# skywoodsz/qm_control

Measured on NVIDIA H100. Metric: mpc_wbc_iters_per_s, higher is better.
Workload: dtype f64

## Files before the change

include/qmb200.h:

```cpp
#ifndef QMB200_H
#define QMB200_H
#include <stdint.h>

#ifdef __cplusplus
extern "C" {
#endif

#define QMB200_NX 30
#define QMB200_NU 30
#define QMB200_RBD 55
#define QMB200_CMD 54
#define QMB200_TARGET 37
#define QMB200_EMAX 32
#define QMB200_KMAX 4

#define QMB200_WBC_HIERARCHICAL 0
#define QMB200_WBC_HIERARCHICAL_MPC 1

#define QMB200_ST_ITER_CAP 1
#define QMB200_ST_OVERFLOW 2
#define QMB200_ST_NAN 4
#define QMB200_ST_NOT_PD 8
#define QMB200_ST_NO_STEP 16
#define QMB200_ST_CONVERGED 32
// ... 15 lines not shown
  int32_t wbc_variant;
} qmb200_config;

int qmb200_create(const qmb200_config* cfg, qmb200_handle** out);
void qmb200_destroy(qmb200_handle* h);
const char* qmb200_last_error(const qmb200_handle* h);

int qmb200_get_dims(const qmb200_handle* h, int32_t* batch, int32_t* nmax, int32_t* emax, int32_t* kmax);
int qmb200_get_model_info(const qmb200_handle* h, double* robot_mass, double* initial_state30, double* default_joint_state18, double* time_horizon, double* dt);
int qmb200_get_joint_name(const qmb200_handle* h, int32_t joint, char* out, int32_t capacity);

int qmb200_wbc_update(qmb200_handle* h, const double* x_des , const double* u_des , const double* rbd ,
                      const int32_t* mode , const double* period , const double* time , double* cmd , int32_t* status );
int qmb200_wbc_update_dev(qmb200_handle* h, const double* x_des, const double* u_des, const double* rbd, const int32_t* mode, const double* period,
                          const double* time, double* cmd, int32_t* status, void* cuda_stream);
int qmb200_wbc_set_input_last(qmb200_handle* h, const double* input_last );
int qmb200_wbc_get_input_last(qmb200_handle* h, double* input_last );

typedef struct {
  double kp_swing, kd_swing, base_height_kp, base_height_kd, kp_base_linear, kd_base_linear, kp_base_angular, kd_base_angular;
  double kp_arm_joint[6], kd_arm_joint[6], kp_ee_linear[3], kd_ee_linear[3], kp_ee_angular[3], kd_ee_angular[3];
} qmb200_wbc_gains;
int qmb200_wbc_get_gains(const qmb200_handle* h, qmb200_wbc_gains* out);
int qmb200_wbc_set_gains(qmb200_handle* h, const qmb200_wbc_gains* gains);
int qmb200_wbc_get_diagnostics(qmb200_handle* h, int32_t* diag );
int qmb200_wbc_set_iteration_caps(qmb200_handle* h, int32_t level0_passes, int32_t active_set_iterations);

int qmb200_mpc_solve(qmb200_handle* h, const double* t0 , const double* x0 ,
                     const int32_t* n_events , const double* event_times , const int32_t* mode_sequence ,
                     const int32_t* n_target , const double* target_times , const double* target_states ,
                     int32_t* n_nodes , double* node_times , int32_t* node_events ,
                     double* x_traj , double* u_traj , int32_t* status , double* step_info );
int qmb200_mpc_solve_dev(qmb200_handle* h, const double* t0, const double* x0, const int32_t* n_events, const double* event_times, const int32_t* mode_sequence,
                         const int32_t* n_target, const double* target_times, const double* target_states, void* cuda_stream);
int qmb200_mpc_set_iterations(qmb200_handle* h, int32_t sqp_iterations, double cost_tol);
int qmb200_mpc_reset(qmb200_handle* h);
int qmb200_mpc_set_solution(qmb200_handle* h, const int32_t* n_nodes, const double* node_times, const int32_t* node_events, const double* x_traj, const double* u_traj);
int qmb200_mpc_get_solution(qmb200_handle* h, int32_t* n_nodes, double* node_times, int32_t* node_events, double* x_traj, double* u_traj, int32_t* status, double* step_info);

int qmb200_policy_eval(qmb200_handle* h, const double* t , double* x_des , double* u_des , int32_t* mode );
int qmb200_policy_eval_dev(qmb200_handle* h, const double* t, double* x_des, double* u_des, int32_t* mode, void* cuda_stream);

int qmb200_tick(qmb200_handle* h, const double* t0, const double* x0, const int32_t* n_events, const double* event_times, const int32_t* mode_sequence,
                const int32_t* n_target, const double* target_times, const double* target_states, const double* t_eval, const double* rbd,
                const double* period, double* cmd , int32_t* status );
int qmb200_tick_dev(qmb200_handle* h, const double* t0, const double* x0, const int32_t* n_events, const double* event_times, const int32_t* mode_sequence,
                    const int32_t* n_target, const double* target_times, const double* target_states, const double* t_eval, const double* rbd,
                    const double* period, double* cmd, int32_t* status, void* cuda_stream);

int qmb200_centroidal_state_from_rbd(const qmb200_handle* h, int32_t n, const double* rbd , double* x );

#define QMB200_SRBD 24
int qmb200_set_model_payload(qmb200_handle* h, const double* payload );
int qmb200_get_model_payload(const qmb200_handle* h, double* payload , int32_t* is_set);

#define QMB200_TUNING 40
int qmb200_set_robot_tuning(qmb200_handle* h, const double* rows );
int qmb200_get_robot_tuning(const qmb200_handle* h, double* rows , int32_t* is_set);
int qmb200_get_handle_tuning(const qmb200_handle* h, double* row );

typedef struct qmb200_payload_est_params {
  double forgetting, p0_mass, p0_first_moment, p0_inertia, trace_max, mass_min, mass_max, offset_max;
} qmb200_payload_est_params;
int qmb200_payload_est_get_params(const qmb200_handle* h, qmb200_payload_est_params* out);
int qmb200_payload_est_set_params(qmb200_handle* h, const qmb200_payload_est_params* p);
int qmb200_payload_est_reset(qmb200_handle* h, const double* prior );
int qmb200_payload_est_step(qmb200_handle* h, double dt, const double* effort , const double* rbd , int32_t* status );
int qmb200_payload_est_step_dev(qmb200_handle* h, double dt, const double* effort, const double* rbd, int32_t* status, void* cuda_stream);
int qmb200_payload_est_commit_dev(qmb200_handle* h, void* cuda_stream);
int qmb200_payload_est_get(qmb200_handle* h, double* theta , double* p_diag , int32_t* samples );
int qmb200_payload_est_stop(qmb200_handle* h);
int qmb200_get_model_payload_dev(const qmb200_handle* h, double* payload , void* cuda_stream);

int qmb200_gait_schedule(const char* gait_file, const char* gait_name, double t_start, double lo, double hi,
                         double* event_times , int32_t* mode_sequence );

typedef struct qmb200_gait qmb200_gait;
int qmb200_gait_create(const char* task_file, const char* reference_file, qmb200_gait** out);
void qmb200_gait_destroy(qmb200_gait* g);
int qmb200_gait_insert_template(qmb200_gait* g, const char* gait_file, const char* gait_name, double start_time, double final_time);
int qmb200_gait_get_mode_schedule(qmb200_gait* g, double lower_bound_time, double upper_bound_time, double* event_times , int32_t* mode_sequence );

#define QMB200_GAIT_CAP 64
#define QMB200_GAIT_MAXM 16
int qmb200_gait_dev_set_templates(qmb200_handle* h, const char* gait_file, const char* const* names, int32_t n);
int qmb200_gait_dev_reset(qmb200_handle* h, const int32_t* tmpl , const double* t_start );
int qmb200_gait_dev_set_commands(qmb200_handle* h, int32_t n_cmd, const double* t , const int32_t* tmpl , const double* cmd_vel );
int qmb200_gait_dev_set_commands_ee(qmb200_handle* h, int32_t n_cmd, const double* t , const int32_t* tmpl , const double* cmd_vel ,
                                    const int32_t* ee_kind , const double* ee_cmd );
int qmb200_gait_dev_step(qmb200_handle* h, const double* t_obs , int32_t* n_events , double* event_times ,
                         int32_t* mode_sequence , double* cmd , int32_t* tmpl , int32_t* mode ,
                         int32_t* status );
int qmb200_gait_dev_step_dev(qmb200_handle* h, const double* t_obs, int32_t* n_events, double* event_times, int32_t* mode_sequence, double* cmd, int32_t* tmpl,
                             int32_t* mode, int32_t* status, void* cuda_stream);
int qmb200_gait_dev_step_ee(qmb200_handle* h, const double* t_obs , int32_t* n_events , double* event_times ,
                            int32_t* mode_sequence , double* cmd , int32_t* tmpl , int32_t* mode ,
                            int32_t* status , int32_t* target_kind );
int qmb200_gait_dev_step_ee_dev(qmb200_handle* h, const double* t_obs, int32_t* n_events, double* event_times, int32_t* mode_sequence, double* cmd, int32_t* tmpl,
                                int32_t* mode, int32_t* status, int32_t* target_kind, void* cuda_stream);
int qmb200_gait_dev_get(qmb200_handle* h, int32_t* n_events , double* event_times , int32_t* mode_sequence ,
                        int32_t* tmpl , int32_t* cursor );
int qmb200_gait_dev_get_commands(qmb200_handle* h, int32_t* n_cmd, double* t , int32_t* tmpl , double* cmd_vel ,
                                 int32_t* ee_kind , double* ee_cmd );
int qmb200_gait_dev_stop(qmb200_handle* h);

#define QMB200_TARGET_CMD_VEL 0
#define QMB200_TARGET_EE_CMD_VEL 1
#define QMB200_TARGET_EE_GOAL 2
#define QMB200_JOINT_CMD 5
#define QMB200_ST_SAFETY 0x10000
#define QMB200_ST_HW_RING_FULL 2

int qmb200_observation_update(qmb200_handle* h, const double* rbd , const double* period , double* t_obs , double* x_obs );
int qmb200_observation_update_dev(qmb200_handle* h, const double* rbd, const double* period, double* t_obs, double* x_obs, void* cuda_stream);

int qmb200_target_trajectories(qmb200_handle* h, int32_t kind, const double* cmd , const double* t_obs , const double* x_obs , const double* ee_state ,
                               double* last_ee_target , int32_t* n_target , double* target_times , double* target_states );
int qmb200_target_trajectories_dev(qmb200_handle* h, int32_t kind, const double* cmd, const double* t_obs, const double* x_obs, const double* ee_state, double* last_ee_target,
                                   int32_t* n_target, double* target_times, double* target_states, void* cuda_stream);
int qmb200_target_trajectories_per_robot(qmb200_handle* h, const int32_t* kind , const double* cmd , const double* t_obs , const double* x_obs ,
                                         const double* ee_state , double* last_ee_target , int32_t* n_target ,
                                         double* target_times , double* target_states );
int qmb200_target_trajectories_per_robot_dev(qmb200_handle* h, const int32_t* kind, const double* cmd, const double* t_obs, const double* x_obs, const double* ee_state,
                                             double* last_ee_target, int32_t* n_target, double* target_times, double* target_states, void* cuda_stream);
void qmb200_initial_ee_target(double* last_ee_target7);

int qmb200_control_law(qmb200_handle* h, const double* x_des , const double* u_des , const double* wbc_cmd , const double* t_obs , const double* x_obs ,
                       double* joint_cmd , double* arm_pos_cmd , double* last_time , int32_t* status );
int qmb200_control_law_dev(qmb200_handle* h, const double* x_des, const double* u_des, const double* wbc_cmd, const double* t_obs, const double* x_obs, double* joint_cmd, double* arm_pos_cmd,
                           double* last_time, int32_t* status, void* cuda_stream);
int qmb200_set_arm_gains(qmb200_handle* h, double kp_arm_wbc, double kd_arm_wbc);

int qmb200_hw_write(qmb200_handle* h, const double* time , const double* period , const double* joint_cmd , const double* joint_pos , const double* joint_vel ,
                    double* effort , int32_t* status );
int qmb200_hw_write_dev(qmb200_handle* h, const double* time, const double* period, const double* joint_cmd, const double* joint_pos, const double* joint_vel, double* effort, int32_t* status, void* cuda_stream);
int qmb200_hw_set_delay(qmb200_handle* h, double delay);

typedef struct {
  double ground_height;
  double foot_radius;
  double stiffness;
  double damping;
  double tangential_damping;
  double friction_mu;
  double joint_damping[18];
  int32_t substeps_per_ms;
} qmb200_sim_params;
int qmb200_sim_get_params(const qmb200_handle* h, qmb200_sim_params* out);
int qmb200_sim_set_params(qmb200_handle* h, const qmb200_sim_params* p);
int qmb200_sim_step(qmb200_handle* h, double duration, const double* effort , double* q , double* v ,
                    double* rbd , int32_t* contact , int32_t* status );
int qmb200_sim_step_dev(qmb200_handle* h, double duration, const double* effort, double* q, double* v, double* rbd, int32_t* contact, int32_t* status, void* cuda_stream);
int qmb200_sim_set_robot_params(qmb200_handle* h, const double* friction_mu , const double* payload );
int qmb200_sim_get_robot_params(const qmb200_handle* h, double* friction_mu , double* payload , int32_t* set_mask);
int qmb200_sim_step_ext(qmb200_handle* h, double duration, const double* effort , const double* wrench , double* q ,
                        double* v , double* rbd , int32_t* contact , int32_t* status );
int qmb200_sim_step_ext_dev(qmb200_handle* h, double duration, const double* effort, const double* wrench, double* q, double* v, double* rbd, int32_t* contact,
                            int32_t* status, void* cuda_stream);
int qmb200_sim_set_terrain(qmb200_handle* h, int32_t n_tiles, int32_t nx, int32_t ny, double cell, const double* heights );
int qmb200_sim_get_terrain(const qmb200_handle* h, int32_t* n_tiles, int32_t* nx, int32_t* ny, double* cell, double* heights );
int qmb200_sim_set_robot_terrain(qmb200_handle* h, const int32_t* tile , const double* origin );
int qmb200_sim_get_robot_terrain(const qmb200_handle* h, int32_t* tile , double* origin , int32_t* is_set);
int qmb200_sim_standing_state(const qmb200_handle* h, int32_t n, const double* xy_yaw , double* q , double* v );

#define QMB200_SENSORS 46
typedef struct qmb200_sensor_params {
  uint64_t seed;
  double sigma_orientation, sigma_gyro, sigma_accel, sigma_joint_pos, sigma_joint_vel;
} qmb200_sensor_params;
int qmb200_sim_get_sensor_params(const qmb200_handle* h, qmb200_sensor_params* out);
int qmb200_sim_set_sensor_params(qmb200_handle* h, const qmb200_sensor_params* p);
int qmb200_sim_read_sensors(qmb200_handle* h, double dt, int64_t sample, const double* q , const double* v , const double* v_prev ,
                            double* sensors );
int qmb200_sim_read_sensors_dev(qmb200_handle* h, double dt, int64_t sample, const double* q, const double* v, const double* v_prev, double* sensors, void* cuda_stream);

typedef struct qmb200_state_est_params {
  double process_base_pos, process_base_vel, process_foot, meas_foot_pos, meas_foot_vel, meas_foot_height, swing_scale, foot_height, p0_base_pos, p0_base_vel, p0_foot;
} qmb200_state_est_params;
int qmb200_state_est_get_params(const qmb200_handle* h, qmb200_state_est_params* out);
int qmb200_state_est_set_params(qmb200_handle* h, const qmb200_state_est_params* p);
int qmb200_state_est_reset(qmb200_handle* h, const double* base_pos );
int qmb200_state_est_step(qmb200_handle* h, double dt, const double* sensors , const int32_t* contact , double* rbd_est , int32_t* status );
int qmb200_state_est_step_dev(qmb200_handle* h, double dt, const double* sensors, const int32_t* contact, double* rbd_est, int32_t* status, void* cuda_stream);
int qmb200_state_est_get(qmb200_handle* h, double* x , double* p_diag , int32_t* samples );
int qmb200_state_est_stop(qmb200_handle* h);
int qmb200_state_est_set_ground(qmb200_handle* h, const int32_t* tile , const double* origin );
int qmb200_state_est_get_ground(const qmb200_handle* h, int32_t* tile , double* origin , int32_t* is_set);

typedef struct qmb200_attitude_params {
  double process_attitude, process_gyro_bias, meas_orientation, p0_attitude, p0_gyro_bias;
} qmb200_attitude_params;
int qmb200_attitude_get_params(const qmb200_handle* h, qmb200_attitude_params* out);
int qmb200_attitude_set_params(qmb200_handle* h, const qmb200_attitude_params* p);
int qmb200_attitude_reset(qmb200_handle* h);
int qmb200_attitude_step(qmb200_handle* h, double dt, double* sensors , int32_t* status );
int qmb200_attitude_step_dev(qmb200_handle* h, double dt, double* sensors, int32_t* status, void* cuda_stream);
int qmb200_attitude_get(qmb200_handle* h, double* quat , double* gyro_bias , double* p_diag , int32_t* samples );
int qmb200_attitude_stop(qmb200_handle* h);

typedef struct qmb200_slip_params {
  double gate, release, meas_slip;
  int32_t hold;
} qmb200_slip_params;
int qmb200_slip_get_params(const qmb200_handle* h, qmb200_slip_params* out);
int qmb200_slip_set_params(qmb200_handle* h, const qmb200_slip_params* p);
int qmb200_slip_reset(qmb200_handle* h);
int qmb200_slip_step(qmb200_handle* h, double dt, const double* sensors , const int32_t* contact_in , int32_t* stance_out ,
                     int32_t* slip_out , int32_t* status );
int qmb200_slip_step_dev(qmb200_handle* h, double dt, const double* sensors, const int32_t* contact_in, int32_t* stance_out, int32_t* slip_out, int32_t* status,
                         void* cuda_stream);
int qmb200_slip_get(qmb200_handle* h, int32_t* mask , int32_t* hold , int32_t* onsets );
int qmb200_slip_stop(qmb200_handle* h);

int qmb200_robot_image_save(qmb200_handle* h);
int qmb200_robot_image_clear(qmb200_handle* h);
int qmb200_robot_image_restore(qmb200_handle* h, const int32_t* mask );
int qmb200_robot_image_restore_dev(qmb200_handle* h, const int32_t* mask , void* cuda_stream);
int qmb200_fall_detect(qmb200_handle* h, const double* rbd , double z_min, double tilt_max, int32_t* count , int32_t* fallen );
int qmb200_fall_detect_dev(qmb200_handle* h, const double* rbd, double z_min, double tilt_max, int32_t* count, int32_t* fallen, void* cuda_stream);

#define QMB200_EPISODE 27
#define QMB200_EPISODE_MODEL_PAYLOAD 1
#define QMB200_EPISODE_MPC_FRICTION 2
#define QMB200_EPISODE_WBC_FRICTION 4
int qmb200_episode_set_ranges(qmb200_handle* h, const double* lo , const double* hi , int64_t seed);
int qmb200_episode_get_ranges(const qmb200_handle* h, double* lo , double* hi , int64_t* seed, int32_t* is_set);
int qmb200_episode_sample(qmb200_handle* h, const int32_t* mask , const int32_t* episode , int32_t link, double* rows );
int qmb200_episode_sample_dev(qmb200_handle* h, const int32_t* mask, const int32_t* episode, int32_t link, double* rows, void* cuda_stream);
int qmb200_episode_draw(const qmb200_handle* h, int32_t n, const int32_t* robot , const int32_t* episode , double* rows );

#define QMB200_SPAWN 4
#define QMB200_SPAWN_GROUND_MAP 1
int qmb200_spawn_set_ranges(qmb200_handle* h, const double* lo , const double* hi , int64_t seed);
int qmb200_spawn_get_ranges(const qmb200_handle* h, double* lo , double* hi , int64_t* seed, int32_t* is_set);
int qmb200_spawn_sample(qmb200_handle* h, const int32_t* mask , const int32_t* episode , int32_t link, double* rows ,
                        double* q , double* v , double* rbd , int32_t* contact ,
                        double* x_obs , double* last_ee , double* rbd_est );
int qmb200_spawn_sample_dev(qmb200_handle* h, const int32_t* mask, const int32_t* episode, int32_t link, double* rows, double* q, double* v, double* rbd, int32_t* contact,
                            double* x_obs, double* last_ee, double* rbd_est, void* cuda_stream);
int qmb200_spawn_draw(const qmb200_handle* h, int32_t n, const int32_t* robot , const int32_t* episode , double* rows );

#define QMB200_METRICS 18
#define QMB200_METRICS_ACC 32
int qmb200_metrics_step(qmb200_handle* h, double dt, const double* rbd , const int32_t* contact , const double* effort ,
                        const double* cmd , const int32_t* kind , const int32_t* n_target , const double* target_times,
                        const double* target_states, const double* time , const int32_t* status , const double* rbd_est ,
                        double* acc );
int qmb200_metrics_step_dev(qmb200_handle* h, double dt, const double* rbd, const int32_t* contact, const double* effort, const double* cmd, const int32_t* kind,
                            const int32_t* n_target, const double* target_times, const double* target_states, const double* time, const int32_t* status,
                            const double* rbd_est, double* acc, void* cuda_stream);
int qmb200_metrics_close(qmb200_handle* h, const int32_t* mask , const int32_t* end , const int32_t* episode , int32_t n_episodes,
                         double* acc , double* out , int32_t* status );
int qmb200_metrics_close_dev(qmb200_handle* h, const int32_t* mask, const int32_t* end, const int32_t* episode, int32_t n_episodes, double* acc, double* out,
                             int32_t* status, void* cuda_stream);

#define QMB200_TIMELINE 22
#define QMB200_TIMELINE_CMD 14
int qmb200_timeline_set_ranges(qmb200_handle* h, int32_t n_cmd, const double* lo , const double* hi ,
                               int64_t seed);
int qmb200_timeline_get_ranges(const qmb200_handle* h, int32_t* n_cmd, double* lo , double* hi , int64_t* seed,
                               int32_t* is_set);
int qmb200_timeline_sample(qmb200_handle* h, const int32_t* mask , const int32_t* episode , double* rows );
int qmb200_timeline_sample_dev(qmb200_handle* h, const int32_t* mask, const int32_t* episode, double* rows, void* cuda_stream);
int qmb200_timeline_draw(const qmb200_handle* h, int32_t n, const int32_t* robot , const int32_t* episode , double* rows );

#define QMB200_CURRICULUM 7
#define QMB200_CURRICULUM_STATE 4
#define QMB200_CURRICULUM_MAX_COND 4
#define QMB200_CURRICULUM_EPISODE 0
#define QMB200_CURRICULUM_SPAWN 1
#define QMB200_CURRICULUM_TIMELINE 2
#define QMB200_CURRICULUM_GE 0
#define QMB200_CURRICULUM_LE 1
#define QMB200_CURRICULUM_PASS 0
#define QMB200_CURRICULUM_FAIL 1
typedef struct qmb200_curriculum_rule {
  int32_t n_levels, n_cond;
  int32_t column[QMB200_CURRICULUM_MAX_COND], op[QMB200_CURRICULUM_MAX_COND], role[QMB200_CURRICULUM_MAX_COND];
} qmb200_curriculum_rule;
int qmb200_curriculum_set(qmb200_handle* h, const qmb200_curriculum_rule* rule, const double* rows );
int qmb200_curriculum_attach(qmb200_handle* h, int32_t kind, const double* lo_top , const double* hi_top );
int qmb200_curriculum_update(qmb200_handle* h, const int32_t* mask , const int32_t* end , const int32_t* episode ,
                             const double* rows , int32_t n_episodes, int32_t* level ,
                             int32_t* status );
int qmb200_curriculum_update_dev(qmb200_handle* h, const int32_t* mask, const int32_t* end, const int32_t* episode, const double* rows, int32_t n_episodes,
                                 int32_t* level, int32_t* status, void* cuda_stream);
int qmb200_curriculum_get(const qmb200_handle* h, int32_t* state , int32_t* is_set);
int qmb200_curriculum_draw(const qmb200_handle* h, int32_t kind, int32_t n, const int32_t* robot , const int32_t* episode ,
                           const int32_t* level , double* rows);

int qmb200_update(qmb200_handle* h, const double* rbd , const double* period , double* t_obs , double* x_obs , double* joint_cmd ,
                  double* arm_pos_cmd , double* last_time , double* cmd , int32_t* status );
int qmb200_update_dev(qmb200_handle* h, const double* rbd, const double* period, double* t_obs, double* x_obs, double* joint_cmd, double* arm_pos_cmd, double* last_time, double* cmd, int32_t* status, void* cuda_stream);

int qmb200_set_pipeline(qmb200_handle* h, int chunks);

int qmb200_set_profiling(qmb200_handle* h, int on);
int qmb200_collect_kernel_times(qmb200_handle* h);
int qmb200_get_kernel_times(qmb200_handle* h, double* ms6);
int qmb200_get_flow_kernel_time(qmb200_handle* h, double* ms);
int qmb200_measure_fp64_peak(qmb200_handle* h, double* tflops);

int qmb200_debug_get_step(qmb200_handle* h, double* dx , double* du , double* robot );
#define QMB200_SOLVER_SQP 0
#define QMB200_SOLVER_IPM 1
#define QMB200_SOLVER_DDP 2
int qmb200_mpc_set_solver(qmb200_handle* h, int32_t solver);
int qmb200_mpc_get_solver(const qmb200_handle* h, int32_t* solver, int32_t* iterations, double* delta_tol, double* g_max, double* g_min);

#define QMB200_COMM_ID_BYTES 128
int qmb200_comm_get_unique_id(void* id128);
int qmb200_comm_init(qmb200_handle* h, int32_t nranks, int32_t rank, const void* id128);
int qmb200_comm_destroy(qmb200_handle* h);
int qmb200_comm_info(const qmb200_handle* h, int32_t* nranks, int32_t* rank, int32_t* nccl_version);
int qmb200_allgather_torque(qmb200_handle* h, void* nccl_comm, const double* cmd_local , const int32_t* perm ,
                            double* torque_all , void* cuda_stream);
int qmb200_gait_bin_permutation(int32_t n, const double* t0, const int32_t* n_events, const double* event_times , const int32_t* modes , int32_t* perm );

int64_t qmb200_debug_model_blob(const qmb200_config* cfg, void* out, int64_t capacity);
int qmb200_debug_srbd_constants(const qmb200_config* cfg, int32_t n, const double* payload , double* out );

int64_t qmb200_launch_count(const qmb200_handle* h);
void* qmb200_stream(const qmb200_handle* h);

#ifdef __cplusplus
}
#endif
#endif
```

qm_control_b200/_lib.py:

```python
import ctypes as C
import os

HERE = os.path.dirname(os.path.abspath(__file__))
ROOT = os.path.dirname(HERE)
LIB_PATH = os.environ.get("QMB200_LIB", os.path.join(HERE, "libqmb200.so"))
ASSETS = os.path.join(ROOT, "assets")

NX, NU, RBD, CMD, TARGET, EMAX, KMAX = 30, 30, 55, 54, 37, 32, 4
GAIT_CAP, GAIT_MAXM = 64, 16
TARGET_CMD_VEL, TARGET_EE_CMD_VEL, TARGET_EE_GOAL = 0, 1, 2

dp = C.POINTER(C.c_double)
ip = C.POINTER(C.c_int32)


class QmbError(RuntimeError):
    pass


class Config(C.Structure):
    _fields_ = [("task_file", C.c_char_p), ("urdf_file", C.c_char_p), ("reference_file", C.c_char_p), ("wbc_gains_file", C.c_char_p),
                ("batch", C.c_int32), ("device", C.c_int32), ("time_horizon", C.c_double), ("dt", C.c_double), ("max_nodes", C.c_int32), ("wbc_variant", C.c_int32)]


class WbcGains(C.Structure):
    _fields_ = [(n, C.c_double) for n in ("kp_swing", "kd_swing", "base_height_kp", "base_height_kd", "kp_base_linear", "kd_base_linear", "kp_base_angular", "kd_base_angular")] + \
               [("kp_arm_joint", C.c_double * 6), ("kd_arm_joint", C.c_double * 6), ("kp_ee_linear", C.c_double * 3), ("kd_ee_linear", C.c_double * 3), ("kp_ee_angular", C.c_double * 3), ("kd_ee_angular", C.c_double * 3)]


class SimParams(C.Structure):
    _fields_ = [(n, C.c_double) for n in ("ground_height", "foot_radius", "stiffness", "damping", "tangential_damping", "friction_mu")] + \
               [("joint_damping", C.c_double * 18), ("substeps_per_ms", C.c_int32)]


class PayloadEstParams(C.Structure):
    _fields_ = [(n, C.c_double) for n in ("forgetting", "p0_mass", "p0_first_moment", "p0_inertia", "trace_max", "mass_min", "mass_max", "offset_max")]


SENSORS = 46


class SensorParams(C.Structure):
    _fields_ = [("seed", C.c_uint64)] + [(n, C.c_double) for n in ("sigma_orientation", "sigma_gyro", "sigma_accel", "sigma_joint_pos", "sigma_joint_vel")]


class StateEstParams(C.Structure):
    _fields_ = [(n, C.c_double) for n in ("process_base_pos", "process_base_vel", "process_foot", "meas_foot_pos", "meas_foot_vel", "meas_foot_height", "swing_scale",
                                          "foot_height", "p0_base_pos", "p0_base_vel", "p0_foot")]


class AttitudeParams(C.Structure):
    _fields_ = [(n, C.c_double) for n in ("process_attitude", "process_gyro_bias", "meas_orientation", "p0_attitude", "p0_gyro_bias")]


class SlipParams(C.Structure):
    _fields_ = [("gate", C.c_double), ("release", C.c_double), ("meas_slip", C.c_double), ("hold", C.c_int32)]


SENSOR_LAYOUT = ("quat_x", "quat_y", "quat_z", "quat_w", "gyro_x", "gyro_y", "gyro_z", "accel_x", "accel_y", "accel_z") + \
                tuple("joint_pos_%d" % j for j in range(18)) + tuple("joint_vel_%d" % j for j in range(18))
STATE_EST_LAYOUT = ("p_x", "p_y", "p_z", "v_x", "v_y", "v_z") + tuple("foot_%s_%s" % (f, a) for f in ("LF", "RF", "LH", "RH") for a in "xyz")
SENSOR_NOISE_REFERENCE = dict(sigma_orientation=0.0012 ** 0.5, sigma_gyro=0.0004 ** 0.5, sigma_accel=0.01 ** 0.5)

THETA_LAYOUT = ("m", "mc_x", "mc_y", "mc_z", "I_xx", "I_xy", "I_xz", "I_yy", "I_yz", "I_zz")

PAYLOAD_LAYOUT = ("m_ee", "o_ee_x", "o_ee_y", "o_ee_z", "m_base", "o_base_x", "o_base_y", "o_base_z")
SRBD_LAYOUT = ("m",) + tuple("I_nom_%d%d" % (i, j) for i in range(3) for j in range(3)) + tuple("I_nom_inv_%d%d" % (i, j) for i in range(3) for j in range(3)) + \
              ("c_nom_x", "c_nom_y", "c_nom_z", "pad0", "pad1")
TUNING_LAYOUT = {}
for _n, _w in [("friction_mu", 1), ("wbc_friction", 1), ("mu_ee_pos", 1), ("mu_ee_ori", 1), ("mu_final_ee_pos", 1), ("mu_final_ee_ori", 1)] + \
              [(_f, getattr(_t, "_length_", 1)) for _f, _t in WbcGains._fields_] + [("kp_arm_wbc", 1), ("kd_arm_wbc", 1)]:
    TUNING_LAYOUT[_n] = (sum(w for _, w in TUNING_LAYOUT.values()), _w)
TUNING = sum(w for _, w in TUNING_LAYOUT.values())
del _n, _w
WRENCH_LAYOUT = ("f_base_x", "f_base_y", "f_base_z", "n_base_x", "n_base_y", "n_base_z", "f_ee_x", "f_ee_y", "f_ee_z", "n_ee_x", "n_ee_y", "n_ee_z")
EPISODE_LAYOUT = ("friction_mu",) + PAYLOAD_LAYOUT + ("push_t_on", "push_duration") + WRENCH_LAYOUT + ("cmd_vel_x", "cmd_vel_y", "cmd_vel_z", "cmd_yaw_rate")
EPISODE = len(EPISODE_LAYOUT)
EPISODE_MODEL_PAYLOAD, EPISODE_MPC_FRICTION, EPISODE_WBC_FRICTION = 1, 2, 4
SPAWN_LAYOUT = ("tile", "dx", "dy", "yaw")
SPAWN = len(SPAWN_LAYOUT)
SPAWN_GROUND_MAP = 1
METRICS_LAYOUT = ("duration", "end", "status", "distance", "path_length", "min_height", "max_tilt", "vel_err_rms", "yaw_rate_err_rms", "ee_pos_err_rms",
                  "ee_pos_err_max", "ee_ori_err_rms", "energy", "torque_rms", "slip", "touchdowns", "est_pos_err_rms", "est_vel_err_rms")
METRICS = len(METRICS_LAYOUT)
METRICS_ACC = 32
TIMELINE_LAYOUT = ("t_first", "gap", "p_gait", "gait_set", "w_none", "w_cmd_vel", "w_ee_cmd_vel", "w_ee_goal", "cmd_vel_x", "cmd_vel_y", "cmd_vel_z", "cmd_yaw_rate",
                   "ee_vx", "ee_vy", "ee_vz", "ee_x", "ee_y", "ee_z", "ee_qx", "ee_qy", "ee_qz", "ee_qw")
TIMELINE = len(TIMELINE_LAYOUT)
TIMELINE_CMD_LAYOUT = ("t", "tmpl", "cmd_vel_x", "cmd_vel_y", "cmd_vel_z", "cmd_yaw_rate", "ee_kind") + tuple("ee_%d" % i for i in range(7))
TIMELINE_CMD = len(TIMELINE_CMD_LAYOUT)
CURRICULUM_LAYOUT = ("start_level", "up_after", "down_after", "threshold_0", "threshold_1", "threshold_2", "threshold_3")
CURRICULUM = len(CURRICULUM_LAYOUT)
CURRICULUM_STATE_LAYOUT = ("level", "pass_run", "fail_run", "n_updates")
CURRICULUM_STATE = len(CURRICULUM_STATE_LAYOUT)
CURRICULUM_MAX_COND = 4
CURRICULUM_KINDS = ("episode", "spawn", "timeline")
CURRICULUM_OPS = (">=", "<=")
CURRICULUM_ROLES = ("pass", "fail")


class CurriculumRule(C.Structure):
    _fields_ = [("n_levels", C.c_int32), ("n_cond", C.c_int32), ("column", C.c_int32 * 4), ("op", C.c_int32 * 4), ("role", C.c_int32 * 4)]


P, I32, I64, D, S, CFG = C.c_void_p, C.c_int32, C.c_int64, C.c_double, C.c_char_p, C.POINTER(Config)
PROTOTYPES = {
    "qmb200_create": (I32, [CFG, P]),
    "qmb200_destroy": (None, [P]),
    "qmb200_last_error": (S, [P]),
    "qmb200_get_dims": (I32, [P] * 5),
    "qmb200_get_model_info": (I32, [P] * 6),
    "qmb200_get_joint_name": (I32, [P, I32, P, I32]),
    "qmb200_wbc_update": (I32, [P] * 9),
    "qmb200_wbc_update_dev": (I32, [P] * 10),
    "qmb200_wbc_set_input_last": (I32, [P] * 2),
    "qmb200_wbc_get_input_last": (I32, [P] * 2),
    "qmb200_wbc_get_gains": (I32, [P] * 2),
    "qmb200_wbc_set_gains": (I32, [P] * 2),
    "qmb200_wbc_get_diagnostics": (I32, [P] * 2),
    "qmb200_wbc_set_iteration_caps": (I32, [P, I32, I32]),
    "qmb200_mpc_solve": (I32, [P] * 16),
    "qmb200_mpc_solve_dev": (I32, [P] * 10),
    "qmb200_mpc_set_iterations": (I32, [P, I32, D]),
    "qmb200_mpc_reset": (I32, [P]),
    "qmb200_mpc_set_solution": (I32, [P] * 6),
    "qmb200_mpc_get_solution": (I32, [P] * 8),
    "qmb200_policy_eval": (I32, [P] * 5),
    "qmb200_policy_eval_dev": (I32, [P] * 6),
    "qmb200_tick": (I32, [P] * 14),
    "qmb200_tick_dev": (I32, [P] * 15),
    "qmb200_centroidal_state_from_rbd": (I32, [P, I32, P, P]),
    "qmb200_set_model_payload": (I32, [P] * 2),
    "qmb200_get_model_payload": (I32, [P] * 3),
    "qmb200_set_robot_tuning": (I32, [P] * 2),
    "qmb200_get_robot_tuning": (I32, [P] * 3),
    "qmb200_get_handle_tuning": (I32, [P] * 2),
    "qmb200_payload_est_get_params": (I32, [P] * 2),
    "qmb200_payload_est_set_params": (I32, [P] * 2),
    "qmb200_payload_est_reset": (I32, [P] * 2),
    "qmb200_payload_est_step": (I32, [P, D] + [P] * 3),
    "qmb200_payload_est_step_dev": (I32, [P, D] + [P] * 4),
    "qmb200_payload_est_commit_dev": (I32, [P] * 2),
    "qmb200_payload_est_get": (I32, [P] * 4),
    "qmb200_payload_est_stop": (I32, [P]),
    "qmb200_get_model_payload_dev": (I32, [P] * 3),
    "qmb200_gait_schedule": (I32, [S, S, D, D, D, P, P]),
    "qmb200_gait_create": (I32, [S, S, P]),
    "qmb200_gait_destroy": (None, [P]),
    "qmb200_gait_insert_template": (I32, [P, S, S, D, D]),
    "qmb200_gait_get_mode_schedule": (I32, [P, D, D, P, P]),
    "qmb200_gait_dev_set_templates": (I32, [P, S, P, I32]),
    "qmb200_gait_dev_reset": (I32, [P] * 3),
    "qmb200_gait_dev_set_commands": (I32, [P, I32] + [P] * 3),
    "qmb200_gait_dev_set_commands_ee": (I32, [P, I32] + [P] * 5),
    "qmb200_gait_dev_step": (I32, [P] * 9),
    "qmb200_gait_dev_step_dev": (I32, [P] * 10),
    "qmb200_gait_dev_step_ee": (I32, [P] * 10),
    "qmb200_gait_dev_step_ee_dev": (I32, [P] * 11),
    "qmb200_gait_dev_get": (I32, [P] * 6),
    "qmb200_gait_dev_get_commands": (I32, [P] * 7),
    "qmb200_gait_dev_stop": (I32, [P]),
    "qmb200_observation_update": (I32, [P] * 5),
    "qmb200_observation_update_dev": (I32, [P] * 6),
    "qmb200_target_trajectories": (I32, [P, I32] + [P] * 8),
    "qmb200_target_trajectories_dev": (I32, [P, I32] + [P] * 9),
    "qmb200_target_trajectories_per_robot": (I32, [P] * 10),
    "qmb200_target_trajectories_per_robot_dev": (I32, [P] * 11),
    "qmb200_initial_ee_target": (None, [P]),
    "qmb200_control_law": (I32, [P] * 10),
    "qmb200_control_law_dev": (I32, [P] * 11),
    "qmb200_set_arm_gains": (I32, [P, D, D]),
    "qmb200_hw_write": (I32, [P] * 8),
    "qmb200_hw_write_dev": (I32, [P] * 9),
    "qmb200_hw_set_delay": (I32, [P, D]),
    "qmb200_sim_get_params": (I32, [P] * 2),
    "qmb200_sim_set_params": (I32, [P] * 2),
    "qmb200_sim_step": (I32, [P, D] + [P] * 6),
    "qmb200_sim_step_dev": (I32, [P, D] + [P] * 7),
    "qmb200_sim_set_robot_params": (I32, [P] * 3),
    "qmb200_sim_get_robot_params": (I32, [P] * 4),
    "qmb200_sim_step_ext": (I32, [P, D] + [P] * 7),
    "qmb200_sim_step_ext_dev": (I32, [P, D] + [P] * 8),
    "qmb200_sim_set_terrain": (I32, [P, I32, I32, I32, D, P]),
    "qmb200_sim_get_terrain": (I32, [P] * 6),
    "qmb200_sim_set_robot_terrain": (I32, [P] * 3),
    "qmb200_sim_get_robot_terrain": (I32, [P] * 4),
    "qmb200_sim_standing_state": (I32, [P, I32, P, P, P]),
    "qmb200_sim_get_sensor_params": (I32, [P] * 2),
    "qmb200_sim_set_sensor_params": (I32, [P] * 2),
    "qmb200_sim_read_sensors": (I32, [P, D, I64] + [P] * 4),
    "qmb200_sim_read_sensors_dev": (I32, [P, D, I64] + [P] * 5),
    "qmb200_state_est_get_params": (I32, [P] * 2),
    "qmb200_state_est_set_params": (I32, [P] * 2),
    "qmb200_state_est_reset": (I32, [P] * 2),
    "qmb200_state_est_step": (I32, [P, D] + [P] * 4),
    "qmb200_state_est_step_dev": (I32, [P, D] + [P] * 5),
    "qmb200_state_est_get": (I32, [P] * 4),
    "qmb200_state_est_stop": (I32, [P]),
    "qmb200_state_est_set_ground": (I32, [P] * 3),
    "qmb200_state_est_get_ground": (I32, [P] * 4),
    "qmb200_attitude_get_params": (I32, [P] * 2),
    "qmb200_attitude_set_params": (I32, [P] * 2),
    "qmb200_attitude_reset": (I32, [P]),
    "qmb200_attitude_step": (I32, [P, D] + [P] * 2),
    "qmb200_attitude_step_dev": (I32, [P, D] + [P] * 3),
    "qmb200_attitude_get": (I32, [P] * 5),
    "qmb200_attitude_stop": (I32, [P]),
    "qmb200_slip_get_params": (I32, [P] * 2),
    "qmb200_slip_set_params": (I32, [P] * 2),
    "qmb200_slip_reset": (I32, [P]),
    "qmb200_slip_step": (I32, [P, D] + [P] * 5),
    "qmb200_slip_step_dev": (I32, [P, D] + [P] * 6),
    "qmb200_slip_get": (I32, [P] * 4),
    "qmb200_slip_stop": (I32, [P]),
    "qmb200_robot_image_save": (I32, [P]),
    "qmb200_robot_image_clear": (I32, [P]),
    "qmb200_robot_image_restore": (I32, [P] * 2),
    "qmb200_robot_image_restore_dev": (I32, [P] * 3),
    "qmb200_fall_detect": (I32, [P, P, D, D, P, P]),
    "qmb200_fall_detect_dev": (I32, [P, P, D, D, P, P, P]),
    "qmb200_episode_set_ranges": (I32, [P, P, P, I64]),
    "qmb200_episode_get_ranges": (I32, [P] * 5),
    "qmb200_episode_sample": (I32, [P, P, P, I32, P]),
    "qmb200_episode_sample_dev": (I32, [P, P, P, I32, P, P]),
    "qmb200_episode_draw": (I32, [P, I32, P, P, P]),
    "qmb200_spawn_set_ranges": (I32, [P, P, P, I64]),
    "qmb200_spawn_get_ranges": (I32, [P] * 5),
    "qmb200_spawn_sample": (I32, [P, P, P, I32] + [P] * 8),
    "qmb200_spawn_sample_dev": (I32, [P, P, P, I32] + [P] * 9),
    "qmb200_spawn_draw": (I32, [P, I32, P, P, P]),
    "qmb200_metrics_step": (I32, [P, D] + [P] * 12),
    "qmb200_metrics_step_dev": (I32, [P, D] + [P] * 13),
    "qmb200_metrics_close": (I32, [P] * 4 + [I32] + [P] * 3),
    "qmb200_metrics_close_dev": (I32, [P] * 4 + [I32] + [P] * 4),
    "qmb200_timeline_set_ranges": (I32, [P, I32, P, P, I64]),
    "qmb200_timeline_get_ranges": (I32, [P] * 6),
    "qmb200_timeline_sample": (I32, [P] * 4),
    "qmb200_timeline_sample_dev": (I32, [P] * 5),
    "qmb200_timeline_draw": (I32, [P, I32, P, P, P]),
    "qmb200_curriculum_set": (I32, [P] * 3),
    "qmb200_curriculum_attach": (I32, [P, I32, P, P]),
    "qmb200_curriculum_update": (I32, [P] * 5 + [I32] + [P] * 2),
    "qmb200_curriculum_update_dev": (I32, [P] * 5 + [I32] + [P] * 3),
    "qmb200_curriculum_get": (I32, [P] * 3),
    "qmb200_curriculum_draw": (I32, [P, I32, I32] + [P] * 4),
    "qmb200_update": (I32, [P] * 10),
    "qmb200_update_dev": (I32, [P] * 11),
    "qmb200_set_pipeline": (I32, [P, I32]),
    "qmb200_set_profiling": (I32, [P, I32]),
    "qmb200_collect_kernel_times": (I32, [P]),
    "qmb200_get_kernel_times": (I32, [P] * 2),
    "qmb200_get_flow_kernel_time": (I32, [P] * 2),
    "qmb200_measure_fp64_peak": (I32, [P] * 2),
    "qmb200_debug_get_step": (I32, [P] * 4),
    "qmb200_mpc_set_solver": (I32, [P, I32]),
    "qmb200_mpc_get_solver": (I32, [P] * 6),
    "qmb200_comm_get_unique_id": (I32, [P]),
    "qmb200_comm_init": (I32, [P, I32, I32, P]),
    "qmb200_comm_destroy": (I32, [P]),
    "qmb200_comm_info": (I32, [P] * 4),
    "qmb200_allgather_torque": (I32, [P] * 6),
    "qmb200_gait_bin_permutation": (I32, [I32] + [P] * 5),
    "qmb200_debug_model_blob": (I64, [CFG, P, I64]),
    "qmb200_debug_srbd_constants": (I32, [CFG, I32, P, P]),
    "qmb200_launch_count": (I64, [P]),
    "qmb200_stream": (P, [P]),
}
SYMBOLS = list(PROTOTYPES)

_lib = None


def load_library():
    global _lib
    if _lib is not None:
        return _lib
    if not os.path.exists(LIB_PATH):
        raise QmbError("libqmb200.so not built (%s): run `python -c 'import __graft_entry__ as g; g.build()'` — there is no CPU fallback" % LIB_PATH)
    lib = C.CDLL(LIB_PATH)
    for name, (restype, argtypes) in PROTOTYPES.items():
        fn = getattr(lib, name)
        fn.restype, fn.argtypes = restype, argtypes
    _lib = lib
    return lib


def asset(name):
    return os.path.join(ASSETS, name)
```

qm_control_b200/csrc/capi_mpc.inc:

```

extern "C" {

int qmb200_centroidal_state_from_rbd(const qmb200_handle* h, int32_t n, const double* rbd, double* x) {
  if (!h || !rbd || !x) return -1; const DevModel& d = h->hm.dev;
  if (int rc = model_rows_sync(h)) return rc;
  const double* srbd = h->srbd.host.empty() ? nullptr : h->srbd.host.data();
  if (srbd && n != h->B) return fail(const_cast<qmb200_handle*>(h), "qmb200_centroidal_state_from_rbd: with a model payload set, n must equal the batch size");
  for (int r = 0; r < n; ++r) centroidal_from_rbd(*srbd_of(&d, srbd, r), rbd + (size_t)r * QMB200_RBD, x + (size_t)r * NX);
  return 0;
}

int qmb200_gait_schedule(const char* gait_file, const char* gait_name, double t_start, double lo, double hi, double* event_times, int32_t* mode_sequence) {
  try {
    InfoFile f(gait_file); ModeTemplate t = read_mode_template(f, gait_name);
    std::vector<double> ev; std::vector<int> md; md.push_back(15); ev.push_back(t_start);
    while (ev.back() < hi) { for (size_t i = 0; i < t.modes.size(); ++i) { md.push_back(t.modes[i]); ev.push_back(ev.back() + (t.switching_times[i + 1] - t.switching_times[i])); } }
    md.push_back(15);
    const size_t idx = std::lower_bound(ev.begin(), ev.end(), lo) - ev.begin();
    if (idx > 0) { ev.erase(ev.begin(), ev.begin() + (idx - 1)); md.erase(md.begin(), md.begin() + (idx - 1)); md.front() = 15; }
    if (ev.size() > QMB200_EMAX) { g_create_error = "qmb200_gait_schedule: more than EMAX events in the window"; return -2; }
    for (size_t i = 0; i < ev.size(); ++i) event_times[i] = ev[i]; for (size_t i = 0; i < md.size(); ++i) mode_sequence[i] = md[i];
    return (int)ev.size();
  } catch (const std::exception& e) { g_create_error = e.what(); return -1; }
}


struct qmb200_gait { std::vector<double> ev; std::vector<int> md; ModeTemplate tmpl; double phase_transition_stance_time = 0.0; };
namespace {
int gait_tile(qmb200_gait* g, double start_time, double final_time) {
  if (g->tmpl.modes.empty()) return 0;
  if (!g->ev.empty() && start_time <= g->ev.back()) { g_create_error = "GaitSchedule: the initial time for template-tiling is not greater than the last event time"; return -2; }
  g->ev.push_back(start_time);
  while (g->ev.back() < final_time) for (size_t i = 0; i < g->tmpl.modes.size(); ++i) { g->md.push_back(g->tmpl.modes[i]); g->ev.push_back(g->ev.back() + (g->tmpl.switching_times[i + 1] - g->tmpl.switching_times[i])); }
  g->md.push_back(15); return 0;
}
}

int qmb200_gait_create(const char* task_file, const char* reference_file, qmb200_gait** out) {
  if (!task_file || !reference_file || !out) { g_create_error = "qmb200_gait_create: null argument"; return -1; }
  try {
    InfoFile task(task_file), ref(reference_file); qmb200_gait* g = new qmb200_gait();
    for (auto& s : ref.list("initialModeSchedule.modeSequence")) g->md.push_back(mode_from_name(s));
    for (auto& s : ref.list("initialModeSchedule.eventTimes")) g->ev.push_back(std::stod(s));
    if (g->md.size() != g->ev.size() + 1) { delete g; g_create_error = "qmb200_gait_create: initialModeSchedule needs one more mode than event times"; return -2; }
    g->tmpl = read_mode_template(ref, "defaultModeSequenceTemplate"); g->phase_transition_stance_time = task.number("model_settings.phaseTransitionStanceTime", 0.4);
    *out = g; return 0;
  } catch (const std::exception& e) { g_create_error = e.what(); return -2; }
}
void qmb200_gait_destroy(qmb200_gait* g) { delete g; }

int qmb200_gait_insert_template(qmb200_gait* g, const char* gait_file, const char* gait_name, double start_time, double final_time) {
  if (!g || !gait_file || !gait_name) return -1;
  try {
    InfoFile f(gait_file); g->tmpl = read_mode_template(f, gait_name);
    const size_t index = std::lower_bound(g->ev.begin(), g->ev.end(), start_time) - g->ev.begin();
    if (index < g->ev.size()) { g->ev.erase(g->ev.begin() + index, g->ev.end()); g->md.erase(g->md.begin() + index + 1, g->md.end()); }
    double stance = g->phase_transition_stance_time; if (!g->md.empty() && g->md.back() == 15) stance = 0.0;
    if (stance > 0.0) { g->ev.push_back(start_time); g->md.push_back(15); }
    return gait_tile(g, start_time + stance, final_time);
  } catch (const std::exception& e) { g_create_error = e.what(); return -2; }
}

int qmb200_gait_get_mode_schedule(qmb200_gait* g, double lower, double upper, double* event_times, int32_t* mode_sequence) {
  if (!g || !event_times || !mode_sequence) return -1;
  const size_t index = std::lower_bound(g->ev.begin(), g->ev.end(), lower) - g->ev.begin();
  if (index > 0) { g->ev.erase(g->ev.begin(), g->ev.begin() + index - 1); g->md.erase(g->md.begin(), g->md.begin() + index - 1); g->md.front() = 15; }
  const double tiling_start = g->ev.empty() ? upper : g->ev.back();
  if (!g->ev.empty()) g->ev.pop_back(); g->md.pop_back();
  if (int rc = gait_tile(g, tiling_start, upper)) return rc;
  if (g->ev.size() > QMB200_EMAX) { g_create_error = "qmb200_gait_get_mode_schedule: more than EMAX events in the window"; return -2; }
  for (size_t i = 0; i < g->ev.size(); ++i) event_times[i] = g->ev[i]; for (size_t i = 0; i < g->md.size(); ++i) mode_sequence[i] = g->md[i];
  return (int)g->ev.size();
}

namespace {
__global__ void combine_status_kernel(int b0, int B, const int32_t* mpc_status, int32_t* status) { const int b = b0 + blockIdx.x * blockDim.x + threadIdx.x; if (b < B) status[b] = status[b] | (mpc_status[b] << 8); }

int stage_problem(qmb200_handle* h, const double* t0, const double* x0, const int32_t* n_events, const double* event_times, const int32_t* modes, const int32_t* n_target, const double* target_times, const double* target_states, cudaMemcpyKind kind, cudaStream_t s) {
  MpcBuffers& m = h->mpc; const size_t B = (size_t)h->B;
  QMB_CUDA(h, cudaMemcpyAsync(m.t0, t0, B * 8, kind, s)); QMB_CUDA(h, cudaMemcpyAsync(m.x0, x0, B * NX * 8, kind, s));
  QMB_CUDA(h, cudaMemcpyAsync(m.n_events, n_events, B * 4, kind, s)); QMB_CUDA(h, cudaMemcpyAsync(m.event_times, event_times, B * EMAX * 8, kind, s));
  QMB_CUDA(h, cudaMemcpyAsync(m.modes, modes, B * (EMAX + 1) * 4, kind, s)); QMB_CUDA(h, cudaMemcpyAsync(m.n_target, n_target, B * 4, kind, s));
  QMB_CUDA(h, cudaMemcpyAsync(m.target_times, target_times, B * KMAX * 8, kind, s)); QMB_CUDA(h, cudaMemcpyAsync(m.target_states, target_states, B * KMAX * TARGET_DIM * 8, kind, s));
  return 0;
}
int launch_solve(qmb200_handle* h, cudaStream_t s) {
  MpcBuffers& m = h->mpc; MpcProblemDev p{m.t0, m.x0, m.n_events, m.event_times, m.modes, m.n_target, m.target_times, m.target_states, h->srbd.dev(), h->tuning.dev()};
  h->launches += mpc_solve_launch(h->d_model, h->hm.dev, m, p, 0, m.B, s, h->profiling ? h->ev : nullptr); m.cur = 1 - m.cur;
  QMB_CUDA(h, cudaGetLastError()); return 0;
}
int launch_tick(qmb200_handle* h, const double* t_eval, const double* rbd, const double* period, double* cmd, int32_t* status, cudaStream_t s) {
  MpcBuffers& m = h->mpc; MpcProblemDev p{m.t0, m.x0, m.n_events, m.event_times, m.modes, m.n_target, m.target_times, m.target_states, h->srbd.dev(), h->tuning.dev()};
  const int B = h->B; const int C = (h->profiling || h->chunks <= 1) ? 1 : h->chunks;
  auto lo = [&](int c) { return (int)((long long)B * c / C); };
  auto stream = [&](int c) { return C == 1 ? s : h->cs[c]; };
  if (C > 1) QMB_CUDA(h, cudaEventRecord(h->fork_ev, s));
  for (int c = 0; c < C; ++c) {
    if (C > 1) QMB_CUDA(h, cudaStreamWaitEvent(h->cs[c], h->fork_ev, 0));
    h->launches += mpc_solve_launch(h->d_model, h->hm.dev, m, p, lo(c), lo(c + 1), stream(c), h->profiling ? h->ev : nullptr);
  }
  m.cur = 1 - m.cur;
  for (int c = 0; c < C; ++c) {
    const int b0 = lo(c), b1 = lo(c + 1); cudaStream_t cs = stream(c);
    h->launches += mpc_policy_eval_launch(m, t_eval, h->d_xdes, h->d_udes, h->d_mode, cs, b0, b1);
    if (h->profiling) cudaEventRecord(h->ev[5], cs);
    wbc_launch(h, h->d_xdes, h->d_udes, rbd, h->d_mode, period, t_eval, cmd, status, cs, b0, b1);
    if (h->profiling) { cudaEventRecord(h->ev[6], cs); h->ev_pending = true; }
    combine_status_kernel<<<(b1 - b0 + 127) / 128, 128, 0, cs>>>(b0, b1, m.status, status); h->launches += 1;
    if (C > 1) { QMB_CUDA(h, cudaEventRecord(h->join_ev[c], cs)); QMB_CUDA(h, cudaStreamWaitEvent(s, h->join_ev[c], 0)); }
  }
  QMB_CUDA(h, cudaGetLastError()); return 0;
}
bool null_problem(const void* a, const void* b, const void* c, const void* d, const void* e, const void* f, const void* g, const void* i) { return !a || !b || !c || !d || !e || !f || !g || !i; }
int check_counts(qmb200_handle* h, const int32_t* n_events, const int32_t* n_target, const char* who) {
  for (int b = 0; b < h->B; ++b) {
    if (n_events[b] < 0 || n_events[b] > EMAX) return fail(h, std::string(who) + ": n_events[" + std::to_string(b) + "] = " + std::to_string(n_events[b]) + " outside [0, QMB200_EMAX]");
    if (n_target[b] < 1 || n_target[b] > KMAX) return fail(h, std::string(who) + ": n_target[" + std::to_string(b) + "] = " + std::to_string(n_target[b]) + " outside [1, QMB200_KMAX]");
  }
  return 0;
}
}

int qmb200_mpc_solve_dev(qmb200_handle* h, const double* t0, const double* x0, const int32_t* n_events, const double* event_times, const int32_t* modes, const int32_t* n_target, const double* target_times, const double* target_states, void* cuda_stream) {
  if (!h) return -1; if (null_problem(t0, x0, n_events, event_times, modes, n_target, target_times, target_states)) return fail(h, "qmb200_mpc_solve_dev: null buffer");
  QMB_CUDA(h, cudaSetDevice(h->device)); cudaStream_t s = cuda_stream ? (cudaStream_t)cuda_stream : h->stream;
  if (int rc = stage_problem(h, t0, x0, n_events, event_times, modes, n_target, target_times, target_states, cudaMemcpyDeviceToDevice, s)) return rc;
  return launch_solve(h, s);
}

int qmb200_mpc_get_solution(qmb200_handle* h, int32_t* n_nodes, double* node_times, int32_t* node_events, double* x_traj, double* u_traj, int32_t* status, double* step_info) {
  if (!h) return -1; QMB_CUDA(h, cudaSetDevice(h->device)); MpcBuffers& m = h->mpc; const MpcSolutionDev& sol = m.sol[m.cur]; const size_t B = (size_t)h->B, Bn = B * h->nmax; cudaStream_t s = h->stream;
  if (n_nodes) QMB_CUDA(h, cudaMemcpyAsync(n_nodes, sol.n_nodes, B * 4, cudaMemcpyDeviceToHost, s)); if (node_times) QMB_CUDA(h, cudaMemcpyAsync(node_times, sol.t, Bn * 8, cudaMemcpyDeviceToHost, s));
  if (node_events) QMB_CUDA(h, cudaMemcpyAsync(node_events, sol.event, Bn * 4, cudaMemcpyDeviceToHost, s)); if (x_traj) QMB_CUDA(h, cudaMemcpyAsync(x_traj, sol.x, Bn * NX * 8, cudaMemcpyDeviceToHost, s));
  if (u_traj) QMB_CUDA(h, cudaMemcpyAsync(u_traj, sol.u, Bn * NU * 8, cudaMemcpyDeviceToHost, s)); if (status) QMB_CUDA(h, cudaMemcpyAsync(status, m.status, B * 4, cudaMemcpyDeviceToHost, s));
  if (step_info) QMB_CUDA(h, cudaMemcpyAsync(step_info, m.step_info, B * 4 * 8, cudaMemcpyDeviceToHost, s));
  QMB_CUDA(h, cudaStreamSynchronize(s)); return 0;
}

int qmb200_mpc_solve(qmb200_handle* h, const double* t0, const double* x0, const int32_t* n_events, const double* event_times, const int32_t* modes, const int32_t* n_target, const double* target_times, const double* target_states,
                     int32_t* n_nodes, double* node_times, int32_t* node_events, double* x_traj, double* u_traj, int32_t* status, double* step_info) {
  if (!h) return -1; if (null_problem(t0, x0, n_events, event_times, modes, n_target, target_times, target_states)) return fail(h, "qmb200_mpc_solve: null buffer");
  if (int rc = check_counts(h, n_events, n_target, "qmb200_mpc_solve")) return rc;
  QMB_CUDA(h, cudaSetDevice(h->device));
  if (int rc = stage_problem(h, t0, x0, n_events, event_times, modes, n_target, target_times, target_states, cudaMemcpyHostToDevice, h->stream)) return rc;
  if (int rc = launch_solve(h, h->stream)) return rc;
  return qmb200_mpc_get_solution(h, n_nodes, node_times, node_events, x_traj, u_traj, status, step_info);
}

int qmb200_mpc_set_solver(qmb200_handle* h, int32_t solver) {
  if (!h) return -1; if (solver < QMB200_SOLVER_SQP || solver > QMB200_SOLVER_DDP) return fail(h, "qmb200_mpc_set_solver: unknown solver");
  QMB_CUDA(h, cudaSetDevice(h->device)); DevModel& d = h->hm.dev;
  try {
    InfoFile task(h->task_file);
    if (solver == QMB200_SOLVER_SQP) { d.sqp_iterations = std::max(1, (int)task.number("sqp.sqpIteration", 1.0)); d.delta_tol = task.number("sqp.deltaTol", 1e-4); d.g_max = task.number("sqp.g_max", 1e-2); d.g_min = task.number("sqp.g_min", 1e-6); }
    else if (solver == QMB200_SOLVER_IPM) {
      d.sqp_iterations = std::max(1, (int)task.number("ipm.ipmIteration", 1.0)); d.delta_tol = task.number("ipm.deltaTol", 1e-4); d.g_max = task.number("ipm.g_max", 1e-2); d.g_min = task.number("ipm.g_min", 1e-6); }
    else { d.sqp_iterations = std::max(1, (int)task.number("ddp.maxNumIterations", 1.0)); d.ddp_penalty = task.number("ddp.constraintPenaltyInitialValue", 20.0);
      d.ddp_min_step = task.number("ddp.lineSearch.minStepLength", 1e-2); d.ddp_max_step = task.number("ddp.lineSearch.maxStepLength", 1.0);
      d.ddp_armijo = 1e-4; d.ddp_contraction = 0.5; }
  } catch (const std::exception& e) { return fail(h, std::string("qmb200_mpc_set_solver: ") + e.what()); }
  d.solver = solver;
  return push_model(h);
}
int qmb200_mpc_get_solver(const qmb200_handle* h, int32_t* solver, int32_t* iterations, double* delta_tol, double* g_max, double* g_min) {
  if (!h) return -1; const DevModel& d = h->hm.dev; if (solver) *solver = d.solver; if (iterations) *iterations = d.sqp_iterations; if (delta_tol) *delta_tol = d.delta_tol; if (g_max) *g_max = d.g_max; if (g_min) *g_min = d.g_min; return 0;
}

int qmb200_mpc_set_iterations(qmb200_handle* h, int32_t sqp_iterations, double cost_tol) {
  if (!h) return -1; QMB_CUDA(h, cudaSetDevice(h->device));
  if (sqp_iterations > 0) h->hm.dev.sqp_iterations = sqp_iterations; if (cost_tol > 0.0) h->hm.dev.cost_tol = cost_tol;
  return push_model(h);
}

int qmb200_mpc_reset(qmb200_handle* h) {
  if (!h) return -1; QMB_CUDA(h, cudaSetDevice(h->device));
  for (int s = 0; s < 2; ++s) QMB_CUDA(h, cudaMemsetAsync(h->mpc.sol[s].n_nodes, 0, (size_t)h->B * 4, h->stream));
  QMB_CUDA(h, cudaStreamSynchronize(h->stream)); return 0;
}

int qmb200_mpc_set_solution(qmb200_handle* h, const int32_t* n_nodes, const double* node_times, const int32_t* node_events, const double* x_traj, const double* u_traj) {
  if (!h) return -1; if (!n_nodes || !node_times || !node_events || !x_traj || !u_traj) return fail(h, "qmb200_mpc_set_solution: null buffer");
  QMB_CUDA(h, cudaSetDevice(h->device)); MpcBuffers& m = h->mpc; const MpcSolutionDev& sol = m.sol[m.cur]; const size_t B = (size_t)h->B, Bn = B * h->nmax; cudaStream_t s = h->stream;
  QMB_CUDA(h, cudaMemcpyAsync(sol.n_nodes, n_nodes, B * 4, cudaMemcpyHostToDevice, s)); QMB_CUDA(h, cudaMemcpyAsync(sol.t, node_times, Bn * 8, cudaMemcpyHostToDevice, s));
  QMB_CUDA(h, cudaMemcpyAsync(sol.event, node_events, Bn * 4, cudaMemcpyHostToDevice, s)); QMB_CUDA(h, cudaMemcpyAsync(sol.x, x_traj, Bn * NX * 8, cudaMemcpyHostToDevice, s));
  QMB_CUDA(h, cudaMemcpyAsync(sol.u, u_traj, Bn * NU * 8, cudaMemcpyHostToDevice, s));
  h->launches += mpc_fixup_launch(m, s); QMB_CUDA(h, cudaGetLastError()); QMB_CUDA(h, cudaStreamSynchronize(s)); return 0;
}

int qmb200_policy_eval_dev(qmb200_handle* h, const double* t, double* x_des, double* u_des, int32_t* mode, void* cuda_stream) {
  if (!h) return -1; if (!t || !x_des || !u_des || !mode) return fail(h, "qmb200_policy_eval_dev: null buffer");
  QMB_CUDA(h, cudaSetDevice(h->device));
  h->launches += mpc_policy_eval_launch(h->mpc, t, x_des, u_des, mode, cuda_stream ? (cudaStream_t)cuda_stream : h->stream); QMB_CUDA(h, cudaGetLastError()); return 0;
}
int qmb200_policy_eval(qmb200_handle* h, const double* t, double* x_des, double* u_des, int32_t* mode) {
  if (!h) return -1; if (!t || !x_des || !u_des || !mode) return fail(h, "qmb200_policy_eval: null buffer");
  Staging st(h); if (int rc = st.open()) return rc; const size_t B = (size_t)h->B;
  return st.done(qmb200_policy_eval_dev(h, st.in(t, B), st.out(x_des, B * NX), st.out(u_des, B * NU), st.out(mode, B), h->stream));
}

int qmb200_tick_dev(qmb200_handle* h, const double* t0, const double* x0, const int32_t* n_events, const double* event_times, const int32_t* modes, const int32_t* n_target, const double* target_times, const double* target_states,
                    const double* t_eval, const double* rbd, const double* period, double* cmd, int32_t* status, void* cuda_stream) {
  if (!h) return -1; if (!t_eval || !rbd || !period || !cmd || !status) return fail(h, "qmb200_tick_dev: null buffer");
  cudaStream_t s = cuda_stream ? (cudaStream_t)cuda_stream : h->stream;
  if (null_problem(t0, x0, n_events, event_times, modes, n_target, target_times, target_states)) return fail(h, "qmb200_tick_dev: null buffer");
  QMB_CUDA(h, cudaSetDevice(h->device));
  if (int rc = stage_problem(h, t0, x0, n_events, event_times, modes, n_target, target_times, target_states, cudaMemcpyDeviceToDevice, s)) return rc;
  return launch_tick(h, t_eval, rbd, period, cmd, status, s);
}
int qmb200_tick(qmb200_handle* h, const double* t0, const double* x0, const int32_t* n_events, const double* event_times, const int32_t* modes, const int32_t* n_target, const double* target_times, const double* target_states,
                const double* t_eval, const double* rbd, const double* period, double* cmd, int32_t* status) {
  if (!h) return -1; if (null_problem(t0, x0, n_events, event_times, modes, n_target, target_times, target_states) || !t_eval || !rbd || !period || !cmd || !status) return fail(h, "qmb200_tick: null buffer");
  if (int rc = check_counts(h, n_events, n_target, "qmb200_tick")) return rc;
  Staging st(h); if (int rc = st.open()) return rc; const size_t B = (size_t)h->B;
  if (int rc = stage_problem(h, t0, x0, n_events, event_times, modes, n_target, target_times, target_states, cudaMemcpyHostToDevice, h->stream)) return rc;
  return st.done(launch_tick(h, st.in(t_eval, B), st.in(rbd, B * QMB200_RBD), st.in(period, B), st.out(cmd, B * QMB200_CMD), st.out(status, B), h->stream));
}

int qmb200_set_pipeline(qmb200_handle* h, int chunks) {
  if (!h) return -1; QMB_CUDA(h, cudaSetDevice(h->device));
  if (chunks < 1 || chunks > qmb200_handle::MAX_CHUNKS) return fail(h, "qmb200_set_pipeline: chunks must be in [1, 8]");
  if (chunks > h->B) chunks = h->B;
  if (!h->fork_ev) QMB_CUDA(h, cudaEventCreateWithFlags(&h->fork_ev, cudaEventDisableTiming));
  for (int c = 0; c < chunks; ++c) { if (!h->cs[c]) QMB_CUDA(h, cudaStreamCreateWithFlags(&h->cs[c], cudaStreamNonBlocking)); if (!h->join_ev[c]) QMB_CUDA(h, cudaEventCreateWithFlags(&h->join_ev[c], cudaEventDisableTiming)); }
  h->chunks = chunks; return 0;
}
int qmb200_set_profiling(qmb200_handle* h, int on) {
  if (!h) return -1; QMB_CUDA(h, cudaSetDevice(h->device));
  if (on && !h->ev[0]) for (int i = 0; i < 8; ++i) QMB_CUDA(h, cudaEventCreate(&h->ev[i]));
  h->profiling = on != 0; for (double& v : h->kernel_ms) v = 0.0; h->kernel_calls = 0; h->ev_pending = false; return 0;
}
int qmb200_collect_kernel_times(qmb200_handle* h) {
  if (!h || !h->profiling || !h->ev_pending) return -1; QMB_CUDA(h, cudaSetDevice(h->device)); QMB_CUDA(h, cudaEventSynchronize(h->ev[6]));
  const int a[6] = {0, 1, 2, 3, 4, 5}, b[6] = {1, 2, 3, 4, 5, 6};
  for (int i = 0; i < 6; ++i) { float ms = 0; QMB_CUDA(h, cudaEventElapsedTime(&ms, h->ev[a[i]], h->ev[b[i]])); h->kernel_ms[i] += ms; }
  { float ms = 0; QMB_CUDA(h, cudaEventElapsedTime(&ms, h->ev[1], h->ev[7])); h->kernel_ms[6] += ms; }
  h->kernel_calls += 1; h->ev_pending = false; return 0;
}
int qmb200_get_kernel_times(qmb200_handle* h, double* ms6) { if (!h || !ms6) return -1; for (int i = 0; i < 6; ++i) ms6[i] = h->kernel_calls ? h->kernel_ms[i] / h->kernel_calls : 0.0; return 0; }
int qmb200_get_flow_kernel_time(qmb200_handle* h, double* ms) { if (!h || !ms) return -1; *ms = h->kernel_calls ? h->kernel_ms[6] / h->kernel_calls : 0.0; return 0; }
int qmb200_measure_fp64_peak(qmb200_handle* h, double* tflops) { if (!h || !tflops) return -1; QMB_CUDA(h, cudaSetDevice(h->device)); *tflops = measure_fp64_peak(h->stream); QMB_CUDA(h, cudaGetLastError()); return 0; }

int qmb200_debug_get_step(qmb200_handle* h, double* dx , double* du , double* robot ) {
  if (!h) return -1; QMB_CUDA(h, cudaSetDevice(h->device)); const size_t Bn = (size_t)h->B * h->nmax;
  if (dx) QMB_CUDA(h, cudaMemcpy(dx, h->mpc.dx, Bn * NX * 8, cudaMemcpyDeviceToHost)); if (du) QMB_CUDA(h, cudaMemcpy(du, h->mpc.du, Bn * NU * 8, cudaMemcpyDeviceToHost));
  if (robot) QMB_CUDA(h, cudaMemcpy(robot, h->mpc.robot, (size_t)h->B * ROBOT_DBL * 8, cudaMemcpyDeviceToHost)); return 0;
}

}
```

qm_control_b200/csrc/kernels/mpc_api.cuh:

```cuda
#pragma once
#include <cuda_runtime.h>

#include <string>
#include <vector>

#include "dev_common.cuh"

namespace qmb {

constexpr int EMAX = 32, KMAX = 4, TARGET_DIM = 37;
constexpr int LDX = 36, LDB = 28, LDG = 34, LDH = 24;
constexpr int ST_AR = 0;
constexpr int ST_BR = ST_AR + 9 * LDX;
constexpr int ST_Q = ST_BR + 9 * LDB;
constexpr int Q_PACKED = 480;
__host__ __device__ constexpr int q_row_offset(int r) { return (r & 1) ? 2 * ((r >> 1) + 1) * ((r >> 1) + 1) : 2 * (r >> 1) * ((r >> 1) + 1); }
__host__ __device__ constexpr int q_row_padded(int r) { return (r + 2) & ~1; }
static_assert(q_row_offset(29) + q_row_padded(29) == Q_PACKED && q_row_offset(1) == 2 && q_row_offset(2) == 4 && q_row_offset(3) == 8, "packed lower triangle with even rows");
constexpr int ST_TAIL = ST_Q + Q_PACKED;
constexpr int T_PXJ = 0;
constexpr int T_b = 144, T_q = 174, T_r = 204;
constexpr int T_RT = 222;
constexpr int T_SJ = 276;
constexpr int T_PU2 = 372, T_PED = 380;
constexpr int T_MISC = 396;
constexpr int T_INT = 400;
constexpr int TAIL_DBL = 428, STAGE_DBL = ST_TAIL + TAIL_DBL;
constexpr int SI_TYPE = 0, SI_M = 1, SI_NDEP = 2, SI_DEP = 3, SI_FREE = 19, SI_PIV = 37, SI_PCOL = 41;
static_assert(STAGE_DBL == 1484 && (ST_BR % 2 == 0) && (ST_Q % 2 == 0) && (ST_TAIL % 2 == 0) && (TAIL_DBL % 2 == 0), "16-byte aligned pieces");
constexpr int GAIN_DBL = 18 * LDG;
constexpr int ROBOT_DBL = 8;

struct MpcSolutionDev { int32_t* n_nodes = nullptr; double* t = nullptr; int32_t* event = nullptr; double* x = nullptr; double* u = nullptr; };

struct MpcBuffers {
  int B = 0, nmax = 0, cur = 0;
  double *t0 = nullptr, *x0 = nullptr, *event_times = nullptr, *target_times = nullptr, *target_states = nullptr;
  int32_t *n_events = nullptr, *modes = nullptr, *n_target = nullptr;
  MpcSolutionDev sol[2];
  double *ddp_trial = nullptr;
  double *node_rec = nullptr;
  double *stage = nullptr, *gains = nullptr, *dx = nullptr, *du = nullptr, *robot = nullptr, *step_info = nullptr;
  int32_t *stage_i = nullptr, *status = nullptr;
};
bool mpc_alloc(MpcBuffers& m, int B, int nmax, std::string& err, std::vector<void*>& allocs, cudaStream_t stream);
int mpc_configure_device();

struct MpcProblemDev { const double* t0; const double* x0; const int32_t* n_events; const double* event_times; const int32_t* modes; const int32_t* n_target; const double* target_times; const double* target_states;
                       const double* srbd; const double* tuning; };

int mpc_solve_launch(const DevModel* mdl, const DevModel& host_mdl, MpcBuffers& m, const MpcProblemDev& p, int b0, int b1, cudaStream_t stream, cudaEvent_t* ev = nullptr);
double measure_fp64_peak(cudaStream_t stream);
int mpc_policy_eval_launch(const MpcBuffers& m, const double* t, double* x_des, double* u_des, int32_t* mode, cudaStream_t stream, int b0 = 0, int b1 = -1);
int mpc_fixup_launch(const MpcBuffers& m, cudaStream_t stream);

}
```

qm_control_b200/csrc/kernels/mpc_kernels.cu:

```cuda
#include <cstdlib>
#include "mpc_api.cuh"
#include "mpc_device.cuh"
#include "node_eval.cuh"
#include "wlinalg.cuh"

namespace qmb {

#ifndef QMB_LQ_WARPS
#define QMB_LQ_WARPS 4
#endif
#ifndef QMB_LQ_MINB
#define QMB_LQ_MINB 4
#endif
constexpr int LQ_WARPS = QMB_LQ_WARPS, LS_WARPS = 4, SETUP_WARPS = 4;
enum { MST_ITER_CAP = 1, MST_OVERFLOW = 2, MST_NAN = 4, MST_NOT_PD = 8, MST_NO_STEP = 16, MST_CONVERGED = 32, MST_NEG_DT = 64 };

__device__ __forceinline__ double interval_start(double t, int ev) { return ev == 2 ? t + WEAK_EPS : t; }
__device__ __forceinline__ double interval_end(double t, int ev) { return ev == 1 ? t - WEAK_EPS : t; }
__device__ __forceinline__ int clamp_events(int ne) { return ne < 0 ? 0 : (ne > EMAX ? EMAX : ne); }
__device__ __forceinline__ int clamp_targets(int nk) { return nk < 1 ? 1 : (nk > KMAX ? KMAX : nk); }
__device__ __forceinline__ int flag_mask(int mode) { int m = 0; for (int i = 0; i < 4; ++i) if (contact_flag(mode, i)) m |= 1 << i; return m; }

struct SetupIdx { int iu, ix; double au, ax; };
__host__ __device__ inline size_t setup_smem_per_warp(int nmax) { return (size_t)nmax * (8 + 8 + 4 + sizeof(SetupIdx) + 4) + 8 * EMAX + 64; }
// ... 114 lines not shown
  double f1[12];
  if (work) { ne::FlowBlk* fl = reinterpret_cast<ne::FlowBlk*>(row); ne::flow_finish<true>(mdl, x, bk, acc, fl->f, fl, sc);
#pragma unroll
    for (int i = 0; i < 12; ++i) f1[i] = fl->f[i]; }
  flush(4 * ne::FOOT_DBL, ne::FLOW_DBL);
  if (work) { ne::EeRec* ee = reinterpret_cast<ne::EeRec*>(row);
    const int nk = clamp_targets(p.n_target[b]); const ne::TargetSeg sg = ne::target_segment(p.target_times + (size_t)b * KMAX, p.target_states + (size_t)b * KMAX * TARGET_DIM, nk, t);
    double pref[3], qref[4]; ne::target_pose(sg, nk, pref, qref); ne::ee_eval<true>(mdl, x, bk, pref, qref, ee->e, ee->Je); }
  flush(4 * ne::FOOT_DBL + ne::FLOW_DBL, ne::EE_DBL);
  const bool stage2 = work && !terminal;
  if (stage2) {
    const double cdt = mdl->rk_c * dt;
#pragma unroll
    for (int i = 0; i < NX; ++i) x[i] += cdt * (i < 12 ? f1[i < 12 ? i : 0] : u[i]);
    ne::base_eval<true>(mdl, x, bk, sc); ne::flow_acc_init(acc);
#pragma unroll 1
    for (int i = 0; i < 4; ++i) { ne::Foot2Blk* f2 = reinterpret_cast<ne::Foot2Blk*>(row) + i; ne::foot_eval<true>(mdl, x, u, bk, i, acc, f2->d, nullptr, nullptr, nullptr, f2->JxF, sc); }
  }
  flush(4 * ne::FOOT_DBL + ne::FLOW_DBL + ne::EE_DBL, 4 * ne::FOOT2_DBL);
  if (stage2) { ne::FlowBlk* fl = reinterpret_cast<ne::FlowBlk*>(row); ne::flow_finish<true>(mdl, x, bk, acc, fl->f, fl, sc); }
  flush(4 * ne::FOOT_DBL + ne::FLOW_DBL + ne::EE_DBL + 4 * ne::FOOT2_DBL, ne::FLOW_DBL);
}

__device__ __forceinline__ void flow_column(const ne::FlowBlk& fb, const double* jxf0, int fstride , int lfp, int col, double (&a)[9]) {
#pragma unroll
  for (int q = 0; q < 9; ++q) a[q] = (q >= 3 && q < 6 && col == q - 3) ? 1.0 : 0.0;
  if (col >= 3 && col < 6) {
#pragma unroll
    for (int r = 0; r < 3; ++r) { a[3 + r] = fb.Mpc[3 * r + col - 3]; a[6 + r] = fb.Mtw[3 * r + col - 3]; } }
  else if (col >= 9 && col < 12) {
#pragma unroll
    for (int r = 0; r < 3; ++r) { a[r] = fb.hth[col - 9][r]; a[3 + r] = fb.vp[col - 9][r]; a[6 + r] = fb.vt[col - 9][r]; } }
  else if (col >= 12 && col < 24) { const int j12 = col - 12; const double* jf = jxf0 + foot_of_leg_joint(lfp, j12) * fstride + 3 * (j12 % 3);
#pragma unroll
    for (int r = 0; r < 3; ++r) a[r] = jf[r]; }
}
__device__ __forceinline__ double flow_inner(const ne::FlowBlk& fb, int r, int q) {
  if (q < 3) return r < 3 ? 0.0 : (r < 6 ? fb.Mpc[3 * (r - 3) + q] : fb.Mtw[3 * (r - 6) + q]);
  if (q < 6) return 0.0;
  return r < 3 ? fb.hth[q - 6][r] : (r < 6 ? fb.vp[q - 6][r - 3] : fb.vt[q - 6][r - 6]);
}
template <bool TUNED>
__global__ void __launch_bounds__(32 * LQ_WARPS, QMB_LQ_MINB) mpc_lq_kernel(const DevModel* __restrict__ mdl, int b0, int B, int nmax, MpcProblemDev p, MpcSolutionDev sol, const double* __restrict__ rec, double* __restrict__ stage, int32_t* __restrict__ status) {
  extern __shared__ __align__(16) unsigned char smem_raw[];
  const int warp = threadIdx.x >> 5, lane = threadIdx.x & 31; const long long gid = (long long)blockIdx.x * LQ_WARPS + warp;
  const int b = b0 + (int)(gid / nmax), k = (int)(gid % nmax);
  if (b >= B) return;
  LqSmem& sm = reinterpret_cast<LqSmem*>(smem_raw)[warp]; LqLate& lt = *reinterpret_cast<LqLate*>(&sm.rec.foot[0]);
  const size_t node = (size_t)b * nmax + k; const bool has_next = k + 1 < nmax;
  const double2* rg = reinterpret_cast<const double2*>(rec + node * ne::NODE_REC_DBL); double2 rr[(ne::NODE_REC_DBL / 2 + 31) / 32];
#pragma unroll
  for (int q = 0; q < (ne::NODE_REC_DBL / 2 + 31) / 32; ++q) { const int e = lane + 32 * q; rr[q] = (e < ne::NODE_REC_DBL / 2) ? __ldg(rg + e) : make_double2(0.0, 0.0); }
  const double* xk = sol.x + node * NX; const double* uk = sol.u + node * NU;
  const double xv = (lane < NX) ? xk[lane] : 0.0, uv = (lane < NU) ? uk[lane] : 0.0, xnv = (lane < NX && has_next) ? xk[NX + lane] : 0.0;
  const double* gt = sol.t + (size_t)b * nmax; const int32_t* ge = sol.event + (size_t)b * nmax;
  const double tk = gt[k], tk1 = has_next ? gt[k + 1] : 0.0; const int ek = ge[k], ek1 = has_next ? ge[k + 1] : 0;
  const int ne = clamp_events(p.n_events[b]); double* s_ev = sm.ev; unsigned char* s_modes = sm.modes; const double* ev = s_ev; const unsigned char* modes = s_modes;
  { const double* gev = p.event_times + (size_t)b * EMAX; const int32_t* gmodes = p.modes + (size_t)b * (EMAX + 1); s_ev[lane] = (lane < ne) ? gev[lane] : 0.0; s_modes[lane] = (unsigned char)((lane <= ne) ? gmodes[lane] : 15); if (lane == 0) s_modes[EMAX] = (unsigned char)((EMAX <= ne) ? gmodes[EMAX] : 15); }
  const int n = sol.n_nodes[b];
  const bool work = k < n && !(status[b] & MST_CONVERGED);
  if (!work) return;
  double* sg = stage + node * STAGE_DBL;
  const bool terminal = (k == n - 1);
  const SrbdConst* sc = srbd_of(mdl, p.srbd, b);
  if (lane < NX) { sm.x[lane] = xv; sm.u[lane] = terminal ? 0.0 : uv; }
  __syncwarp();
  if (!terminal && ek == 1) {
    double* tl = sg + ST_TAIL; int32_t* si = reinterpret_cast<int32_t*>(tl + T_INT);
    double d = 0.0; if (lane < NX) { d = xv - xnv; tl[T_b + lane] = d; }
    const double ss = warp_sum(d * d);
    if (lane == 0) { si[SI_TYPE] = 1; si[SI_M] = 0; si[SI_NDEP] = 0; tl[T_MISC] = 0.0; tl[T_MISC + 1] = 0.0; tl[T_MISC + 2] = ss; tl[T_MISC + 3] = 0.0; }
    return;
  }
  { double2* rs = reinterpret_cast<double2*>(&sm.rec);
#pragma unroll
    for (int q = 0; q < (ne::NODE_REC_DBL / 2 + 31) / 32; ++q) { const int e = lane + 32 * q; if (e < ne::NODE_REC_DBL / 2) rs[e] = rr[q]; } }
  __syncwarp();
  const int lfp = pack_leg_foot(mdl);
  const int nk = clamp_targets(p.n_target[b]); const double* tt = p.target_times + (size_t)b * KMAX; const double* ts = p.target_states + (size_t)b * KMAX * TARGET_DIM;
  const double t = interval_start(tk, ek);
  const double dt = terminal ? 0.0 : interval_end(tk1, ek1) - t;
  const int mode = mode_at_time(ev, modes, ne, t); const int fm = terminal ? 0 : flag_mask(mode);
  if (!terminal && !(dt > 0.0) && lane == 0) atomicOr(&status[b], MST_NEG_DT);
  double cost_val = 0.0, eq_ss = 0.0; int ndep = 0, m = 0; double b1v[3] = {0.0, 0.0, 0.0}, b2v[3] = {0.0, 0.0, 0.0}, a1[9], a2[9];
  {
  struct XU { double x[NX], u[NU]; }; static_assert(offsetof(LqSmem, u) == offsetof(LqSmem, x) + NX * 8, "x then u");
  cost_val = stage_cost_quad(mdl, sc, tuning_of(mdl, TUNED ? p.tuning : nullptr, b), reinterpret_cast<const XU*>(sm.x), &sm.rec.ee, &sm.quad, target_xnom(tt, ts, nk, t, lane), fm, terminal, lane);
  if (terminal) {
    double* tl = sg + ST_TAIL; int32_t* si = reinterpret_cast<int32_t*>(tl + T_INT);
    for (int r = 0; r < NX; ++r) { const int a = ee_pos(r); if (lane < q_row_padded(r)) { const int cc = (lane <= r) ? ee_pos(lane) : -1; sg[ST_Q + q_row_offset(r) + lane] = (a >= 0 && cc >= 0) ? sm.quad.E[a * 12 + cc] : 0.0; } }
    if (lane < NX) tl[T_q + lane] = sm.quad.qf[lane];
    if (lane == 0) { si[SI_TYPE] = 2; si[SI_M] = 0; si[SI_NDEP] = 0; tl[T_MISC] = 0.0; tl[T_MISC + 1] = cost_val; tl[T_MISC + 2] = 0.0; tl[T_MISC + 3] = 0.0; }
    return;
  }
  int nd_before = 0; for (int i = 0; i < 4; ++i) if (i < lane) nd_before += ((fm >> i) & 1) ? 3 : 4;
  ndep = 0; for (int i = 0; i < 4; ++i) ndep += ((fm >> i) & 1) ? 3 : 4;
  m = NU - ndep;
  for (int e = lane; e < NU * 3; e += 32) { const int i = e / 3, c = e - 3 * i; sm.Rw[i][c] = (i < 24) ? quad_R(mdl, &sm.quad, i, 3 * (i / 3) + c) : (c == 0 ? quad_R(mdl, &sm.quad, i, i) : 0.0); }
  bool swing_ok = true; int pivot = -1;
  if (lane < 4) {
    const int i = lane; const int first = mdl->foot_leg[i]; LegWs& L = sm.leg[i]; L.first = first; L.stance = (fm >> i) & 1;
    if (L.stance) { for (int j = 0; j < 3; ++j) { sm.dep_idx[nd_before + j] = 12 + first + j; L.dep[j] = 1; } L.pivot = -1; for (int a = 0; a < 3; ++a) eq_ss += sm.rec.foot[i].e[a] * sm.rec.foot[i].e[a]; }
    else {
      double zp, zv; swing_ok = swing_reference(mdl, ev, modes, ne, i, t, zp, zv);
      double ez = sm.rec.foot[i].e[2] - zv; if (mdl->position_error_gain != 0.0) ez += mdl->position_error_gain * (sm.rec.foot[i].pf[2] - zp);
      sm.rec.foot[i].e[2] = ez;
      for (int a = 0; a < 3; ++a) { sm.dep_idx[nd_before + a] = 3 * i + a; eq_ss += sm.u[3 * i + a] * sm.u[3 * i + a]; }
      eq_ss += ez * ez;
      double best = -1.0; for (int j = 0; j < 3; ++j) { const double a = fabs(sm.rec.foot[i].Jl[3 * j + 2]); if (a > best) { best = a; pivot = j; } }
      sm.dep_idx[nd_before + 3] = 12 + first + pivot; L.pivot = pivot; for (int j = 0; j < 3; ++j) L.dep[j] = (j == pivot);
    }
  }
  eq_ss = warp_sum(eq_ss);
  if (!__all_sync(FULL, swing_ok)) { if (lane == 0) atomicOr(&status[b], MST_OVERFLOW); }
  __syncwarp();
  bool is_dep = false; if (lane < NU) for (int d = 0; d < ndep; ++d) is_dep |= (sm.dep_idx[d] == lane);
  const unsigned free_mask = __ballot_sync(FULL, lane < NU && !is_dep);
  if (lane < NU) { const int rank = __popc(free_mask & ((1u << lane) - 1u)); sm.col_of_input[lane] = is_dep ? -1 : rank; if (!is_dep) sm.free_idx[rank] = lane; }
  if (lane < 4) {
    const int i = lane; LegWs& L = sm.leg[i]; const ne::FootBlk& fb = sm.rec.foot[i];
    L.Pu2[0] = L.Pu2[1] = 0.0;
    if (L.stance) {
      double Jm[9], Ji[9]; for (int a = 0; a < 3; ++a) for (int j = 0; j < 3; ++j) Jm[3 * a + j] = fb.Jl[3 * j + a]; inv3(Jm, Ji);
      for (int e = 0; e < 9; ++e) L.G[e] = -Ji[e];
    } else {
      const double nip = -1.0 / fb.Jl[3 * pivot + 2];
      for (int e = 0; e < 9; ++e) L.G[e] = (e == 3 * pivot + 2) ? nip : 0.0;
      int nf = 0; for (int j = 0; j < 3; ++j) if (j != pivot) L.Pu2[nf++] = fb.Jl[3 * j + 2] * nip;
    }
  }
  __syncwarp();
  if (lane < 16) { const int i = lane >> 2, j = lane & 3; if (j < 3) sm.leg[i].free_col[j] = sm.col_of_input[12 + sm.leg[i].first + j]; }
  for (int e = lane; e < 144; e += 32) {
    const int i = e / 36, jc = e - 36 * i, j = jc / 12, c = jc - 12 * j; LegWs& L = sm.leg[i]; const ne::FootBlk& fb = sm.rec.foot[i];
    double sv = 0.0;
#pragma unroll
    for (int a = 0; a < 3; ++a) sv = fma(L.G[3 * j + a], fb.C[a][c], sv);
    L.Px[j][c] = sv;
  }
  if (lane < NU) {
    double pe = 0.0;
    if (lane < 12) { if (!sm.leg[lane / 3].stance) pe = -sm.u[lane]; }
    else if (lane < 24) { const int jl = lane - 12; const int i = foot_of_leg_joint(lfp, jl), j = jl % 3; const LegWs& L = sm.leg[i]; const double* e = sm.rec.foot[i].e;
#pragma unroll
      for (int a = 0; a < 3; ++a) pe = fma(L.G[3 * j + a], e[a], pe); }
    sm.Pe_full[lane] = pe;
  }
  __syncwarp();
  if (lane < NU) {
    double sv = sm.quad.rf[lane];
    if (lane < 24) { const int f = lane / 3; for (int a = 0; a < 3; ++a) sv += sm.Rw[lane][a] * sm.Pe_full[3 * f + a]; }
    sm.rs[lane] = sv;
  }
  const double imr = 1.0 / sc->m;
  if (lane < 12) { const int i = lane / 3, a = lane - 3 * i; const double* d1 = sm.rec.foot[i].d; const double* d2 = sm.rec.foot2[i].d;
#pragma unroll
    for (int r = 0; r < 3; ++r) if (r != a) { const double sgn = ((a - r + 3) % 3 == 1) ? -imr : imr; b1v[r] = sgn * d1[3 - r - a]; b2v[r] = sgn * d2[3 - r - a]; } }
  if (lane < NX) { flow_column(sm.rec.s1, sm.rec.foot[0].JxF, ne::FOOT_DBL, lfp, lane, a1); flow_column(sm.rec.s2, sm.rec.foot2[0].JxF, ne::FOOT2_DBL, lfp, lane, a2); }
  __syncwarp();
  }
  const double w1 = mdl->rk_w1, w2 = mdl->rk_w2, cdt = mdl->rk_c * dt, mass = sc->m, dtw = dt * (w1 + w2), imass = 1.0 / mass;
  double bb = 0.0; if (lane < NX) { const double fa = lane < 12 ? sm.rec.s1.f[lane < 12 ? lane : 0] : sm.u[lane], fb = lane < 12 ? sm.rec.s2.f[lane < 12 ? lane : 0] : sm.u[lane];
    bb = xv + dt * (w1 * fa + w2 * fb) - xnv; lt.bvec[lane] = bb; }
  const double dyn_ss = warp_sum(bb * bb);
  double out[9];
  if (lane < NX) {
    const int c = lane; const ne::FlowBlk& f2 = sm.rec.s2;
#pragma unroll
    for (int r = 0; r < 9; ++r) { double aa = 0.0;
#pragma unroll
      for (int q = 0; q < 9; ++q) if (!(q >= 3 && q < 6) && !(q < 3 && r < 3)) aa = fma(flow_inner(f2, r, q), a1[q], aa);
      out[r] = dt * (w1 * a1[r] + w2 * (a2[r] + cdt * aa));
      if (c < 12) { double b1 = 0.0, b2 = 0.0; if (r < 3) { b1 = b1v[r < 3 ? r : 0]; b2 = b2v[r < 3 ? r : 0]; } double ab = (r == 3 + c % 3) ? imass : 0.0;
        if (r >= 3) {
#pragma unroll
          for (int q = 0; q < 3; ++q) ab += flow_inner(f2, r, q) * b1v[q]; }
        lt.BrdF[r * 12 + c] = dt * (w1 * b1 + w2 * (b2 + cdt * ab)); }
      else if (r < 3) lt.BrdJ[r * NJ + c - 12] = dt * w2 * cdt * a2[r]; }
  }
  __syncwarp();
  double* tl = sg + ST_TAIL; int32_t* si = reinterpret_cast<int32_t*>(tl + T_INT);
  if (lane < NX) {
    const int r = lane; double bt = lt.bvec[r];
    if (r >= 3 && r < 6) for (int i = 0; i < 4; ++i) { const LegWs& L = sm.leg[i]; for (int j = 0; j < 3; ++j) if (L.dep[j]) bt += lt.BrdJ[(r - 3) * NJ + L.first + j] * sm.Pe_full[12 + L.first + j]; }
    if (r >= 12 && r < 24) {
      const LegWs& L = sm.leg[foot_of_leg_joint(lfp, r - 12)];
      if (L.dep[(r - 12) % 3]) bt += dtw * sm.Pe_full[r];
    }
    if (r < 3) for (int f = 0; f < 4; ++f) bt += (dtw * imass) * sm.Pe_full[3 * f + r];
    if (r >= 3 && r < 12) for (int f = 0; f < 4; ++f) if (!sm.leg[f].stance) for (int a = 0; a < 3; ++a) bt += lt.BrdF[(r - 3) * 12 + 3 * f + a] * sm.Pe_full[3 * f + a];
    tl[T_b + r] = bt;
    if (r >= 3 && r < 12) sg[ST_AR + (r - 3) * LDX + NX] = bt;
    const int c = lane; const int pos_all = c < 6 ? c : ((c >= 9 && c < 12) ? c - 3 : -1);
#pragma unroll
    for (int rr = 0; rr < 3; ++rr) {
      double v = out[rr];
#pragma unroll
      for (int i = 0; i < 4; ++i) { const LegWs& L = sm.leg[i]; const int first = L.first;
        const int pos = pos_all >= 0 ? pos_all : ((c >= 12 + first && c < 15 + first) ? 9 + c - 12 - first : -1);
        if (pos >= 0) { double acc = 0.0;
          for (int j = 0; j < 3; ++j) if (L.dep[j]) acc = fma(lt.BrdJ[rr * NJ + first + j], L.Px[j][pos], acc);
          v += acc; } }
      out[rr] = v;
    }
#pragma unroll
    for (int rr = 0; rr < 9; ++rr) { if (c == rr + 3) out[rr] += 1.0; sg[ST_AR + rr * LDX + c] = out[rr]; }
  } else if (lane == 31) {
#pragma unroll
    for (int rr = 0; rr < 9; ++rr) sg[ST_AR + rr * LDX + 31] = 0.0;
  }
  for (int e = lane; e < 36; e += 32) sg[ST_AR + (e >> 2) * LDX + 32 + (e & 3)] = 0.0;
  for (int e = lane; e < 144; e += 32) { const int j12 = e / 12, c = e - 12 * j12; const LegWs& L = sm.leg[foot_of_leg_joint(lfp, j12)]; const int j = j12 % 3; tl[T_PXJ + e] = L.dep[j] ? L.Px[j][c] : 0.0; }
  for (int e = lane; e < 9 * LDB; e += 32) {
    const int rr = e / LDB, a = e - rr * LDB; const int r = 3 + rr; double v = 0.0;
    if (a < m) { const int fa = sm.free_idx[a];
      if (fa < 12) v = lt.BrdF[rr * 12 + fa];
      else if (r < 6) { v = lt.BrdJ[rr * NJ + fa - 12];
        if (fa < 24) { const LegWs& L = sm.leg[foot_of_leg_joint(lfp, fa - 12)]; if (!L.stance) { const int jf = (fa - 12) % 3; v += lt.BrdJ[rr * NJ + L.first + L.pivot] * L.Pu2[jf > L.pivot ? jf - 1 : jf]; } } }
    }
    sg[ST_BR + e] = v;
  }
  if (lane < NX) {
    const int r = lane; double acc[NX];
    if (mdl->q_is_diag) { const double qrr = mdl->Qdiag[r];
#pragma unroll
      for (int c = 0; c < NX; ++c) acc[c] = (c == r) ? qrr : 0.0; }
    else {
#pragma unroll
      for (int c = 0; c < NX; ++c) acc[c] = mdl->Q[r * NX + c]; }
    double qv = sm.quad.qf[r];
    const int ea = ee_pos(r);
    if (ea >= 0) {
#pragma unroll
      for (int c = 0; c < 6; ++c) { acc[6 + c] += sm.quad.E[ea * 12 + c]; acc[24 + c] += sm.quad.E[ea * 12 + 6 + c]; }
    }
#pragma unroll
    for (int i = 0; i < 4; ++i) {
      const LegWs& L = sm.leg[i]; const int first = L.first;
      const int pr = (r < 6) ? r : ((r >= 9 && r < 12) ? r - 3 : ((r >= 12 + first && r < 15 + first) ? 9 + r - 12 - first : -1));
      if (pr >= 0) {
        double blk[12];
#pragma unroll
        for (int c = 0; c < 12; ++c) blk[c] = 0.0;
        double w3[3] = {0.0, 0.0, 0.0};
        for (int j = 0; j < 3; ++j) if (L.dep[j]) { const double pj = L.Px[j][pr]; qv = fma(pj, sm.rs[12 + first + j], qv);
#pragma unroll
          for (int a = 0; a < 3; ++a) w3[a] = fma(pj, sm.Rw[12 + first + j][a], w3[a]); }
        for (int a = 0; a < 3; ++a) if (L.dep[a]) { const double wa = w3[a];
#pragma unroll
          for (int c = 0; c < 12; ++c) blk[c] = fma(wa, L.Px[a][c], blk[c]); }
#pragma unroll
        for (int c = 0; c < 6; ++c) acc[c] += blk[c];
#pragma unroll
        for (int c = 0; c < 3; ++c) acc[9 + c] += blk[6 + c];
#pragma unroll
        for (int l = 0; l < 4; ++l) if (first == 3 * l) {
#pragma unroll
          for (int c = 0; c < 3; ++c) acc[12 + 3 * l + c] += blk[9 + c]; }
      }
    }
    const double dq = sm.quad.qdiag[r];
#pragma unroll
    for (int c = 0; c < NX; ++c) if (r <= c) sg[ST_Q + q_row_offset(c) + r] = dt * (acc[c] + ((c == r) ? dq : 0.0));
    if (!(r & 1)) sg[ST_Q + q_row_offset(r) + r + 1] = 0.0;
    tl[T_q + r] = dt * qv;
  }
  for (int e = lane; e < 8 * 12; e += 32) tl[T_SJ + e] = 0.0;
  __syncwarp();
  if (lane < MU) {
    const int a = lane; double rt[3] = {0.0, 0.0, 0.0}; double rtil = 0.0;
    if (a < m) {
      const int fa = sm.free_idx[a]; double rv = sm.rs[fa]; int li = -1, jf = -1;
      if (fa >= 12 && fa < 24) { li = foot_of_leg_joint(lfp, fa - 12); jf = (fa - 12) % 3; }
      const bool swing_joint = li >= 0 && !sm.leg[li].stance;
      const double* Rl = sm.Rw[jf >= 0 ? fa - jf : 0];
      if (swing_joint) {
        const LegWs& L = sm.leg[li]; const int pv = L.pivot; const int jfi = jf > pv ? jf - 1 : jf; const double pu = L.Pu2[jfi];
        rv += pu * sm.rs[fa - jf + pv];
        const double coef = Rl[3 * jf + pv]; double* Srow = tl + T_SJ + (2 * li + jfi) * 12;
        const double cf = dt * (coef + pu * Rl[3 * pv + pv]);
        for (int c = 0; c < 12; ++c) Srow[c] = cf * L.Px[pv][c];
      }
      rtil = dt * rv;
      if (fa >= 24) rt[0] = dt * sm.Rw[fa][0];
      else { const int bi = fa / 3;
        for (int jc = 0; jc < 3; ++jc) { const int fc = 3 * bi + jc; if (sm.col_of_input[fc] < 0) continue;
          double v = sm.Rw[fa][jc];
          if (swing_joint) { const LegWs& L = sm.leg[li]; const int pv = L.pivot; const double pa = L.Pu2[jf > pv ? jf - 1 : jf], pc = L.Pu2[jc > pv ? jc - 1 : jc];
            v += pa * Rl[3 * pv + jc] + Rl[3 * jf + pv] * pc + pa * Rl[3 * pv + pv] * pc; }
          rt[jc] = dt * v; } }
    }
    tl[T_r + a] = rtil; tl[T_RT + 3 * a] = rt[0]; tl[T_RT + 3 * a + 1] = rt[1]; tl[T_RT + 3 * a + 2] = rt[2];
  }
  if (lane < 4) { const LegWs& L = sm.leg[lane]; tl[T_PU2 + 2 * lane] = L.Pu2[0]; tl[T_PU2 + 2 * lane + 1] = L.Pu2[1]; si[SI_PIV + lane] = L.stance ? -1 : L.pivot;
    int nf = 0; for (int jj = 0; jj < 3; ++jj) if (!L.stance && jj != L.pivot) si[SI_PCOL + 2 * lane + nf++] = L.free_col[jj]; if (L.stance) { si[SI_PCOL + 2 * lane] = -1; si[SI_PCOL + 2 * lane + 1] = -1; } }
  if (lane < MAXDEP) { const int d = lane; double pe = 0.0; int di = -1; if (d < ndep) { di = sm.dep_idx[d]; pe = sm.Pe_full[di]; } tl[T_PED + d] = pe; si[SI_DEP + d] = di; }
  if (lane < MU) si[SI_FREE + lane] = (lane < m) ? sm.free_idx[lane] : -1;
  if (lane == 0) { si[SI_TYPE] = 0; si[SI_M] = m; si[SI_NDEP] = ndep; tl[T_MISC] = dtw; tl[T_MISC + 1] = dt * cost_val; tl[T_MISC + 2] = dt * dyn_ss; tl[T_MISC + 3] = dt * eq_ss; }
}

#ifndef QMB_TMA
#define QMB_TMA 1
#endif
constexpr int RIC_THREADS = 128, RIC_NTYPE = 512;
struct RicSmem {
  double P[NX * LDX];
  double A[NX * LDX];
  double W[NX * LDX];
  double Bm[NX * LDB], PB[NX * LDB];
  double G[MU * LDG];
  double H[MU * LDH];
  double Lt[MU * MU];
  alignas(16) double tail[TAIL_DBL];
  double dx[32], dut[32], tmp[32];
  double red[RIC_THREADS / 32][4];
  alignas(8) unsigned long long bar[4];
  int flag; int pad_;
  signed char srow[MU + 2], sfirst[MU + 2];
  unsigned char ntype[RIC_NTYPE];
};
static_assert(sizeof(RicSmem) <= 57344 - 64, "Riccati kernel must keep four CTAs per SM");

__device__ __forceinline__ unsigned smem_u32(const void* p) { return (unsigned)__cvta_generic_to_shared(p); }
__device__ __forceinline__ void mbar_init(unsigned long long* b, unsigned count) { asm volatile("mbarrier.init.shared::cta.b64 [%0], %1;\n" ::"r"(smem_u32(b)), "r"(count) : "memory"); }
__device__ __forceinline__ void mbar_expect_tx(unsigned long long* b, unsigned bytes) { asm volatile("mbarrier.arrive.expect_tx.shared::cta.b64 _, [%0], %1;\n" ::"r"(smem_u32(b)), "r"(bytes) : "memory"); }
__device__ __forceinline__ void mbar_wait(unsigned long long* b, unsigned parity) {
  asm volatile("{\n .reg .pred p;\n WAIT_LOOP:\n mbarrier.try_wait.parity.shared::cta.b64 p, [%0], %1;\n @p bra WAIT_DONE;\n bra WAIT_LOOP;\n WAIT_DONE:\n}\n" ::"r"(smem_u32(b)), "r"(parity) : "memory");
}
__device__ __forceinline__ void bulk_g2s(void* dst, const void* src, unsigned bytes, unsigned long long* bar) {
  asm volatile("cp.async.bulk.shared::cluster.global.mbarrier::complete_tx::bytes [%0], [%1], %2, [%3];\n" ::"r"(smem_u32(dst)), "l"(src), "r"(bytes), "r"(smem_u32(bar)) : "memory");
}
__device__ __forceinline__ int fresh_tid() { int t; asm volatile("mov.u32 %0, %%tid.x;" : "=r"(t)); return t; }
__device__ __forceinline__ void cp_async16(void* smem_dst, const void* gmem_src) { asm volatile("cp.async.cg.shared.global [%0], [%1], 16;\n" ::"r"(smem_u32(smem_dst)), "l"(gmem_src) : "memory"); }
__device__ __forceinline__ void cp_async_wait_all() { asm volatile("cp.async.wait_all;\n" ::: "memory"); }
struct CopyGroup {
  unsigned long long* bar; unsigned phase;
  __device__ __forceinline__ void begin(unsigned bytes, int tid) { if (QMB_TMA && tid == 0) mbar_expect_tx(bar, bytes); }
  __device__ __forceinline__ void copy(void* dst, const void* src, unsigned bytes, int tid, int nthr = RIC_THREADS, int t0 = 0) {
    if (QMB_TMA) { if (tid == 0) bulk_g2s(dst, src, bytes, bar); }
    else { const int me = tid - t0; if (me >= 0 && me < nthr) for (unsigned o = 16u * me; o < bytes; o += 16u * nthr) cp_async16((char*)dst + o, (const char*)src + o); }
  }
  __device__ __forceinline__ void wait() { if (QMB_TMA) mbar_wait(bar, phase & 1u); else { cp_async_wait_all(); __syncthreads(); } ++phase; }
  __device__ __forceinline__ void skip() { ++phase; }
};

__device__ __forceinline__ void dmma884(double (&c)[2], double a, double b) {
  asm("mma.sync.aligned.m8n8k4.row.col.f64.f64.f64.f64 {%0,%1}, {%2}, {%3}, {%0,%1};\n" : "+d"(c[0]), "+d"(c[1]) : "d"(a), "d"(b));
}
template <int K, int MT, int NT, bool NEG>
__device__ __forceinline__ void warp_mma(const double* __restrict__ X, int ldx, int i0, const double* __restrict__ Y, int ldy, int j0, double (&c)[MT][NT][2], int g, int t) {
#pragma unroll
  for (int ks = 0; ks < (K + 3) / 4; ++ks) {
    const int kr = 4 * ks + t; const bool ok = (4 * ks + 3 < K) || (kr < K);
    double a[MT], bf[NT];
#pragma unroll
    for (int m = 0; m < MT; ++m) { const double v = ok ? X[kr * ldx + i0 + 8 * m + g] : 0.0; a[m] = NEG ? -v : v; }
#pragma unroll
    for (int n = 0; n < NT; ++n) bf[n] = ok ? Y[kr * ldy + j0 + 8 * n + g] : 0.0;
#pragma unroll
    for (int m = 0; m < MT; ++m)
#pragma unroll
      for (int n = 0; n < NT; ++n) dmma884(c[m][n], a[m], bf[n]);
  }
}
template <int MT, int NT>
__device__ __forceinline__ void cfrag_load(const double* M, int ld, int i0, int j0, int rows, double (&c)[MT][NT][2], int g, int t) {
#pragma unroll
  for (int m = 0; m < MT; ++m)
#pragma unroll
    for (int n = 0; n < NT; ++n) { const int ri = i0 + 8 * m + g;
      if (ri < rows) { const double2 v = *reinterpret_cast<const double2*>(M + ri * ld + j0 + 8 * n + 2 * t); c[m][n][0] = v.x; c[m][n][1] = v.y; } else { c[m][n][0] = 0.0; c[m][n][1] = 0.0; } }
}
template <int MT, int NT>
__device__ __forceinline__ void cfrag_store(double* M, int ld, int i0, int j0, int rows, const double (&c)[MT][NT][2], int g, int t) {
#pragma unroll
  for (int m = 0; m < MT; ++m)
#pragma unroll
    for (int n = 0; n < NT; ++n) { const int ri = i0 + 8 * m + g; if (ri < rows) *reinterpret_cast<double2*>(M + ri * ld + j0 + 8 * n + 2 * t) = make_double2(c[m][n][0], c[m][n][1]); }
}
__device__ __forceinline__ int sup_pos(int j, int first) { return j < 6 ? j : ((j >= 9 && j < 12) ? j - 3 : (((unsigned)(j - 12 - first) < 3u) ? 9 + j - 12 - first : -1)); }

__global__ void __launch_bounds__(RIC_THREADS, 4) mpc_riccati_kernel(const DevModel* __restrict__ mdl, int b0, int B, int nmax, MpcProblemDev p, MpcSolutionDev sol, const double* __restrict__ stage,
                                                                  double* __restrict__ gains, double* __restrict__ dxo, double* __restrict__ duo, double* __restrict__ robot, int32_t* __restrict__ status) {
  extern __shared__ __align__(16) unsigned char smem_raw[];
  RicSmem& sm = *reinterpret_cast<RicSmem*>(smem_raw);
  const int tid = threadIdx.x, warp = tid >> 5, lane = tid & 31, ti = tid >> 2, jb = tid & 3; const int b = b0 + blockIdx.x;
  if (status[b] & MST_CONVERGED) return;
  const int n = sol.n_nodes[b]; const int N = n - 1;
  const double* sgb = stage + (size_t)b * nmax * STAGE_DBL; double* gb = gains + (size_t)b * nmax * GAIN_DBL;
  const int lfp = pack_leg_foot(mdl); const double imass = 1.0 / srbd_of(mdl, p.srbd, b)->m;
  for (int e = tid; e < (int)(sizeof(RicSmem) / 8); e += RIC_THREADS) reinterpret_cast<double*>(&sm)[e] = 0.0;
  __syncthreads();
  if (tid < NX && (tid < 3 || tid >= 24)) sm.A[tid * LDX + tid] = 1.0;
  if (tid == 0) { for (int i = 0; i < 4; ++i) mbar_init(&sm.bar[i], 1); asm volatile("fence.mbarrier_init.release.cluster;\n" ::: "memory"); }
  asm volatile("fence.proxy.async.shared::cta;\n" ::: "memory");
  const bool types_in_smem = n <= RIC_NTYPE;
  auto rec_type = [&](int k) -> int { return reinterpret_cast<const int32_t*>(sgb + (size_t)k * STAGE_DBL + ST_TAIL + T_INT)[SI_TYPE]; };
  if (types_in_smem) for (int k = tid; k < n; k += RIC_THREADS) sm.ntype[k] = (unsigned char)rec_type(k);
  auto node_type = [&](int k) -> int { return types_in_smem ? (int)sm.ntype[k] : rec_type(k); };
  CopyGroup gAB{&sm.bar[0], 0u}, gT{&sm.bar[1], 0u}, gQ{&sm.bar[2], 0u}, gF1{&sm.bar[3], 0u};
  auto issue_ab = [&](int k) { const double* sg = sgb + (size_t)k * STAGE_DBL; gAB.begin((9 * LDX + 9 * LDB) * 8, tid);
    gAB.copy(sm.A + 3 * LDX, sg + ST_AR, 9 * LDX * 8, tid); gAB.copy(sm.Bm + 3 * LDB, sg + ST_BR, 9 * LDB * 8, tid); };
  auto issue_tail = [&](int k) { gT.begin(TAIL_DBL * 8, tid); gT.copy(sm.tail, sgb + (size_t)k * STAGE_DBL + ST_TAIL, TAIL_DBL * 8, tid); };
  auto issue_q = [&](int k) { gQ.begin(Q_PACKED * 8, tid); gQ.copy(sm.Bm, sgb + (size_t)k * STAGE_DBL + ST_Q, Q_PACKED * 8, tid); };
  auto expand = [&]() { const int tid = fresh_tid();
    const double* tl = sm.tail; const int32_t* si = reinterpret_cast<const int32_t*>(tl + T_INT); const double dtw = tl[T_MISC];
    for (int e = tid; e < 144; e += RIC_THREADS) { const int j12 = e / 12, c = e - 12 * j12; const int col = sup_col(c, 3 * (j12 / 3));
      sm.A[(12 + j12) * LDX + col] = ((col == 12 + j12) ? 1.0 : 0.0) + dtw * tl[T_PXJ + e]; }
    if (tid < NX && (tid < 3 || tid >= 12)) sm.A[tid * LDX + NX] = tl[T_b + tid];
    for (int e = tid; e < 21 * MU; e += RIC_THREADS) {
      const int rr = e / MU, a = e - rr * MU; const int r = rr < 3 ? rr : rr + 9; const int fa = si[SI_FREE + a]; double v = 0.0;
      if (fa >= 0) {
        if (r < 3) { if (fa < 12 && fa - 3 * (fa / 3) == r) v = dtw * imass; }
        else if (fa == r) v = dtw;
        else if (fa >= 12 && fa < 24) { const int j = fa - 12, lg = j / 3, foot = (lfp >> (2 * lg)) & 3; const int pv = si[SI_PIV + foot];
          if (pv >= 0 && r == 12 + 3 * lg + pv) { const int jf = j - 3 * lg; v = dtw * tl[T_PU2 + 2 * foot + (jf > pv ? jf - 1 : jf)]; } }
      }
      sm.Bm[r * LDB + a] = v;
    }
    if (tid < MU) { const int fa = si[SI_FREE + tid]; int slot = -1, first = 0;
      if (fa >= 12 && fa < 24) { const int j = fa - 12, lg = j / 3, foot = (lfp >> (2 * lg)) & 3; const int pv = si[SI_PIV + foot]; if (pv >= 0) { const int jf = j - 3 * lg; slot = 2 * foot + (jf > pv ? jf - 1 : jf); first = 3 * lg; } }
      sm.srow[tid] = (signed char)slot; sm.sfirst[tid] = (signed char)first; }
  };
  for (int e = tid; e < NX * NX; e += RIC_THREADS) { const int r = e / NX, c = e - r * NX; sm.P[r * LDX + c] = sgb[(size_t)N * STAGE_DBL + ST_Q + q_row_offset(r > c ? r : c) + (r > c ? c : r)]; }
  if (tid < NX) sm.P[tid * LDX + NX] = sgb[(size_t)N * STAGE_DBL + ST_TAIL + T_q + tid];
  double perf0 = 0, perf1 = 0, perf2 = 0;
  for (int k = tid; k < n; k += RIC_THREADS) { const double* pf = sgb + (size_t)k * STAGE_DBL + ST_TAIL + T_MISC + 1; perf0 += pf[0]; perf1 += pf[1]; perf2 += pf[2]; }
  if (tid < NX) { const double d = p.x0[(size_t)b * NX + tid] - sol.x[(size_t)b * nmax * NX + tid]; sm.dx[tid] = d; perf1 += d * d; }
  perf0 = warp_sum(perf0); perf1 = warp_sum(perf1); perf2 = warp_sum(perf2);
  if (lane == 0) { sm.red[warp][0] = perf0; sm.red[warp][1] = perf1; sm.red[warp][2] = perf2; }
  __syncthreads();
  double perf[3]; for (int i = 0; i < 3; ++i) perf[i] = sm.red[0][i] + sm.red[1][i] + sm.red[2][i] + sm.red[3][i];
  if (N >= 1) { issue_tail(N - 1); if (node_type(N - 1) != 1) issue_ab(N - 1); gT.wait(); if (node_type(N - 1) != 1) expand(); }
  int st = 0;
  const int g = lane >> 2, t = lane & 3;
  for (int k = N - 1; k >= 0; --k) {
    const int type = node_type(k); const int tnext = k > 0 ? node_type(k - 1) : 1;
    if (type == 1) {
      __syncthreads();
      if (tid < NX) { double sv = sm.P[tid * LDX + NX]; for (int j = 0; j < NX; ++j) sv = fma(sm.P[tid * LDX + j], sm.tail[T_b + j], sv); sm.tmp[tid] = sv; }
      __syncthreads();
      if (tid < NX) sm.P[tid * LDX + NX] = sm.tmp[tid];
      if (k > 0) { issue_tail(k - 1); if (tnext != 1) issue_ab(k - 1); gT.wait(); if (tnext != 1) expand(); }
      continue;
    }
    gAB.wait(); if (QMB_TMA) __syncthreads();
    const double dtw_k = sm.tail[T_MISC]; const int acol0 = reinterpret_cast<const int32_t*>(sm.tail + T_INT)[SI_M] - 6;
    { const int i0 = 16 * (warp >> 1), j0 = 16 * (warp & 1);
      double c[2][2][2] = {};
      if (warp & 1) {
#pragma unroll
        for (int m = 0; m < 2; ++m) { const int ri = i0 + 8 * m + g; if (ri < NX) {
            if (t < 3) { c[m][1][0] = sm.P[(24 + 2 * t) * LDX + ri]; c[m][1][1] = sm.P[(25 + 2 * t) * LDX + ri]; }
            else { double sv = sm.P[ri * LDX + NX];
#pragma unroll
              for (int kk = 24; kk < NX; ++kk) sv = fma(sm.P[kk * LDX + ri], sm.A[kk * LDX + NX], sv);
              c[m][1][0] = sv; } } } }
      warp_mma<24, 2, 2, false>(sm.P, LDX, i0, sm.A, LDX, j0, c, g, t);
      cfrag_store<2, 2>(sm.W, LDX, i0, j0, NX, c, g, t);
      double d[1][3][2];
#pragma unroll
      for (int nn = 0; nn < 3; ++nn)
#pragma unroll
        for (int e = 0; e < 2; ++e) { const int a = 8 * nn + 2 * t + e - acol0, ri = 8 * warp + g; d[0][nn][e] = ((unsigned)a < 6u && ri < NX) ? dtw_k * sm.P[(24 + a) * LDX + ri] : 0.0; }
      warp_mma<24, 1, 3, false>(sm.P, LDX, 8 * warp, sm.Bm, LDB, 0, d, g, t);
      cfrag_store<1, 3>(sm.PB, LDB, 8 * warp, 0, NX, d, g, t); }
    __syncthreads();
    if (tid < NX) sm.P[tid * LDX + NX] = sm.tail[T_q + tid];
    { const double* tl = sm.tail; const int32_t* si = reinterpret_cast<const int32_t*>(tl + T_INT); const int mm = si[SI_M];
      double c[3][1][2];
#pragma unroll
      for (int mt = 0; mt < 3; ++mt) { const int a = 8 * mt + g; const bool rowok = a < MU; const int slot = rowok ? sm.srow[a] : -1, first = rowok ? sm.sfirst[a] : 0;
#pragma unroll
        for (int e = 0; e < 2; ++e) { const int j = 8 * warp + 2 * t + e; double v = 0.0;
          if (rowok) { if (j == NX) v = tl[T_r + a]; else if (slot >= 0 && j < NX) { const int ps = sup_pos(j, first); if (ps >= 0) v = tl[T_SJ + slot * 12 + ps]; }
            if ((unsigned)(a - acol0) < 6u) v = fma(dtw_k, sm.W[(24 + a - acol0) * LDX + j], v); }
          c[mt][0][e] = v; } }
      warp_mma<24, 3, 1, false>(sm.Bm, LDB, 0, sm.W, LDX, 8 * warp, c, g, t); cfrag_store<3, 1>(sm.G, LDG, 0, 8 * warp, MU, c, g, t);
      if (warp < 3) { double d[3][1][2];
#pragma unroll
        for (int mt = 0; mt < 3; ++mt) { const int a = 8 * mt + g; const int fa = (a < MU) ? si[SI_FREE + a] : -1;
#pragma unroll
          for (int e = 0; e < 2; ++e) { const int cc = 8 * warp + 2 * t + e; double v = 0.0;
            if (a < MU && cc < MU) { if (a >= mm) v = (a == cc) ? 1.0 : 0.0;
              else if (fa >= 24) v = (a == cc) ? tl[T_RT + 3 * a] : 0.0;
              else { const int fc = si[SI_FREE + cc]; if (fc >= 0 && fc / 3 == fa / 3) v = tl[T_RT + 3 * a + fc - 3 * (fc / 3)]; }
              if ((unsigned)(a - acol0) < 6u) v = fma(dtw_k, sm.PB[(24 + a - acol0) * LDB + cc], v); }
            d[mt][0][e] = v; } }
        warp_mma<24, 3, 1, false>(sm.Bm, LDB, 0, sm.PB, LDB, 8 * warp, d, g, t); cfrag_store<3, 1>(sm.H, LDH, 0, 8 * warp, MU, d, g, t); } }
    __syncthreads();
    issue_q(k);
    if (k > 0) issue_tail(k - 1);
    const int sw = (k + b) & 3;
    if (!QMB_TMA) gQ.wait();
    if (warp == sw) {
      if (QMB_TMA) gQ.skip();
      double hr[MU], y[MU]; double dinv = 0.0; bool ok = true; double* Yb = sm.PB;
#pragma unroll
      for (int c = 0; c < MU; ++c) { hr[c] = (lane < MU) ? sm.H[c * LDH + lane] : 0.0; y[c] = sm.G[c * LDG + lane]; }
#pragma unroll
      for (int j = 0; j < MU; ++j) {
        const double djj = __shfl_sync(FULL, hr[j], j); if (!(djj > 0.0)) ok = false;
        const double inv = rsqrt(djj); const double lij = hr[j] * inv;
        if (lane == j) dinv = inv;
        if (lane < MU) sm.Lt[j * MU + lane] = lij;
        y[j] *= inv; Yb[j * LDX + lane] = y[j];
#pragma unroll
        for (int c = j + 1; c < MU; ++c) { const double lcj = __shfl_sync(FULL, lij, c); hr[c] = fma(-lij, lcj, hr[c]); y[c] = fma(-lcj, y[j], y[c]); }
      }
      if (lane < MU) sm.dut[lane] = dinv;
      if (!ok && lane == 0) sm.flag = 1;
      __syncwarp();
      double* gk = gb + (size_t)k * GAIN_DBL;
#pragma unroll
      for (int a = MU - 1; a >= 0; --a) {
        asm volatile("" ::: "memory");
        y[a] *= sm.dut[a];
        gk[a * LDG + lane] = -y[a];
#pragma unroll
        for (int c = 0; c < a; ++c) y[c] = fma(-sm.Lt[c * MU + a], y[a], y[c]);
      }
    } else {
      if (QMB_TMA) gQ.wait();
      const int hi = (warp - sw - 1) & 3;
      for (int tile = hi; tile < 16; tile += 3) { const int i0 = 8 * (tile >> 2), j0 = 8 * (tile & 3);
        double c[1][1][2]; const int ri = i0 + g;
#pragma unroll
        for (int e = 0; e < 2; ++e) { const int cj = j0 + 2 * t + e; double v = (ri < NX && cj <= NX) ? (cj == NX ? sm.P[ri * LDX + NX] : (cj <= ri ? sm.Bm[q_row_offset(ri) + cj] : sm.Bm[q_row_offset(cj) + ri])) : 0.0;
          if (ri >= 24 && ri < NX && cj <= NX) v += sm.W[ri * LDX + cj];
          c[0][0][e] = v; }
        warp_mma<24, 1, 1, false>(sm.A, LDX, i0, sm.W, LDX, j0, c, g, t); cfrag_store<1, 1>(sm.P, LDX, i0, j0, NX, c, g, t); }
    }
    __syncthreads();
    if (sm.flag) { st |= MST_NOT_PD; if (k > 0) gT.wait(); break; }
    if (k > 0) { if (tnext != 1) issue_ab(k - 1); gT.wait(); if (tnext != 1) expand(); }
    { const double* Yb = sm.PB; const int i0 = 16 * (warp >> 1), j0 = 16 * (warp & 1);
      double c[2][2][2]; cfrag_load<2, 2>(sm.P, LDX, i0, j0, NX, c, g, t); warp_mma<MU, 2, 2, true>(Yb, LDX, i0, Yb, LDX, j0, c, g, t); cfrag_store<2, 2>(sm.P, LDX, i0, j0, NX, c, g, t); }
  }
  __syncthreads();
  double armijo = 0.0, dxn2 = 0.0, dun2 = 0.0;
  if (!(st & MST_NOT_PD)) {
    auto issue_fwd = [&](int k) {
      if (k >= N) return; const double* sg = sgb + (size_t)k * STAGE_DBL; const bool ev = node_type(k) == 1;
      auto issue = [&](CopyGroup& cg, double* kb, double* ab, double* bb) {
        cg.begin((ev ? 0 : (GAIN_DBL + 9 * LDX + 9 * LDB) * 8) + TAIL_DBL * 8, tid);
        cg.copy(ab + 9 * LDX, sg + ST_TAIL, TAIL_DBL * 8, tid);
        if (!ev) { cg.copy(kb, gb + (size_t)k * GAIN_DBL, GAIN_DBL * 8, tid); cg.copy(ab, sg + ST_AR, 9 * LDX * 8, tid); cg.copy(bb, sg + ST_BR, 9 * LDB * 8, tid); } };
      if (k & 1) issue(gF1, sm.W, sm.P, sm.PB); else issue(gAB, sm.G, sm.A, sm.Bm); };
    issue_fwd(0);
    for (int k = 0; k < N; ++k) {
      const int o = k & 1; const double* Kb = o ? sm.W : sm.G; const double* ARb = o ? sm.P : sm.A; const double* BRb = o ? sm.PB : sm.Bm; const double* tl = (o ? sm.P : sm.A) + 9 * LDX;
      double* dxk = dxo + ((size_t)b * nmax + k) * NX; double* duk = duo + ((size_t)b * nmax + k) * NU;
      const double* dxc = (k & 1) ? sm.tmp : sm.dx; double* dxn = (k & 1) ? sm.dx : sm.tmp;
      if (o) gF1.wait(); else gAB.wait();
      if (QMB_TMA) __syncthreads();
      issue_fwd(k + 1);
      const int32_t* si = reinterpret_cast<const int32_t*>(tl + T_INT); const int type = si[SI_TYPE], ndep = si[SI_NDEP], mm = si[SI_M]; const double dtw = tl[T_MISC];
      if (tid < NX) { const double dxi = dxc[tid]; dxk[tid] = dxi; dxn2 += dxi * dxi; }
      if (type == 1) { if (tid < NX) { duk[tid] = 0.0; dxn[tid] = dxc[tid] + tl[T_b + tid]; } continue; }
      { double s = 0.0;
        if (ti < MU) { const double* kr = Kb + ti * LDG + jb * 8; const double* dx = dxc + jb * 8;
#pragma unroll
          for (int v = 0; v < 8; ++v) s = fma(kr[v], dx[v], s); }
        s += __shfl_xor_sync(FULL, s, 1); s += __shfl_xor_sync(FULL, s, 2); if (ti < MU && jb == 0) sm.dut[ti] = s + Kb[ti * LDG + NX]; }
      __syncthreads();
      {
        static_assert(MAXDEP * 8 == RIC_THREADS, "one 8-thread group per dependent input");
        const int d = tid >> 3, q8 = tid & 7; double s = 0.0; const int di = (d < ndep) ? si[SI_DEP + d] : -1;
        if (di >= 12) { const int j = di - 12, lg = j / 3, first = 3 * lg; const double* px = tl + T_PXJ + j * 12;
          s = px[q8] * dxc[sup_col(q8, first)]; if (q8 < 4) s = fma(px[q8 + 8], dxc[sup_col(q8 + 8, first)], s);
          if (q8 >= 4 && q8 < 6) { const int foot = (lfp >> (2 * lg)) & 3; const int col = si[SI_PCOL + 2 * foot + q8 - 4]; if (si[SI_PIV + foot] >= 0 && col >= 0) s = fma(tl[T_PU2 + 2 * foot + q8 - 4], sm.dut[col], s); } }
        s += __shfl_xor_sync(FULL, s, 1); s += __shfl_xor_sync(FULL, s, 2); s += __shfl_xor_sync(FULL, s, 4);
        if (di >= 0 && q8 == 0) { const double full = s + tl[T_PED + d]; duk[di] = full; dun2 += full * full; if (di >= 12) dxn[di] = dxc[di] + dtw * s + tl[T_b + di]; } }
      if (tid < NX) armijo += tl[T_q + tid] * dxc[tid];
      if (tid < MU) { const double dut = sm.dut[tid]; armijo += tl[T_r + tid] * dut; const int fi = si[SI_FREE + tid];
        if (fi >= 0) { duk[fi] = dut; dun2 += dut * dut; if (fi >= 12) dxn[fi] = dxc[fi] + dtw * dut + tl[T_b + fi]; } }
      if (warp == 1 && lane < 3) { double acc = 0.0; for (int a = 0; a < mm; ++a) { const int fa = si[SI_FREE + a]; if (fa < 12 && fa - 3 * (fa / 3) == lane) acc += sm.dut[a]; }
        dxn[lane] = dxc[lane] + dtw * imass * acc + tl[T_b + lane]; }
      if (warp >= 2) { const int rr = (tid - 64) >> 2; double s = 0.0;
        if (rr < 9) { const double* ar = ARb + rr * LDX + jb * 8; const double* dx = dxc + jb * 8;
#pragma unroll
          for (int v = 0; v < 8; ++v) s = fma(ar[v], dx[v], s);
          if (jb < 3) { const double* br = BRb + rr * LDB + jb * 8; const double* du = sm.dut + jb * 8;
#pragma unroll
            for (int v = 0; v < 8; ++v) s = fma(br[v], du[v], s); } }
        s += __shfl_xor_sync(FULL, s, 1); s += __shfl_xor_sync(FULL, s, 2); if (rr < 9 && jb == 0) dxn[3 + rr] = s + tl[T_b + 3 + rr]; }
    }
    __syncthreads();
    if (tid < NX) { const double dxi = ((N & 1) ? sm.tmp : sm.dx)[tid]; dxo[((size_t)b * nmax + N) * NX + tid] = dxi; duo[((size_t)b * nmax + N) * NU + tid] = 0.0; dxn2 += dxi * dxi; armijo += sgb[(size_t)N * STAGE_DBL + ST_TAIL + T_q + tid] * dxi; }
  }
  armijo = warp_sum(armijo); dxn2 = warp_sum(dxn2); dun2 = warp_sum(dun2);
  __syncthreads();
  if (lane == 0) { sm.red[warp][0] = armijo; sm.red[warp][1] = dxn2; sm.red[warp][2] = dun2; }
  __syncthreads();
  if (tid == 0) { double a = 0, x2 = 0, u2 = 0; for (int w = 0; w < RIC_THREADS / 32; ++w) { a += sm.red[w][0]; x2 += sm.red[w][1]; u2 += sm.red[w][2]; }
    double* rb = robot + (size_t)b * ROBOT_DBL; rb[0] = a; rb[1] = perf[0]; rb[2] = perf[1]; rb[3] = perf[2]; rb[4] = sqrt(x2); rb[5] = sqrt(u2); if (st) atomicOr(&status[b], st); }
}

__device__ __forceinline__ void fixup_inputs(MpcSolutionDev sol, int b, int nmax, int n, int tid, int nthreads) {
  const int32_t* ge = sol.event + (size_t)b * nmax; double* gu = sol.u + (size_t)b * nmax * NU;
  for (int i = tid; i < NU; i += nthreads) for (int k = 1; k < n; ++k) if ((k == n - 1) || (ge[k] == 1)) gu[(size_t)k * NU + i] = gu[(size_t)(k - 1) * NU + i];
}

#ifndef QMB_LS_MINB
#define QMB_LS_MINB 2
#endif
constexpr int LS_ROW = NX + NU + 12 + 1, LS_SMEM = 32 * LS_WARPS * LS_ROW * 8;
__global__ void __launch_bounds__(32 * LS_WARPS, QMB_LS_MINB) mpc_linesearch_kernel(const DevModel* __restrict__ mdl, int b0, int B, int nmax, MpcProblemDev p, MpcSolutionDev sol, const double* __restrict__ dxo, const double* __restrict__ duo,
                                                                     const double* __restrict__ robot, int32_t* __restrict__ status, double* __restrict__ step_info, int iteration) {
  __shared__ double red[LS_WARPS][3]; __shared__ int decision; __shared__ double s_ev[EMAX]; __shared__ unsigned char s_modes[EMAX + 8];
  extern __shared__ double s_tp[];
  const int tid = threadIdx.x, warp = tid >> 5, lane = tid & 31; const int b = b0 + blockIdx.x; if (b >= B) return;
  if (status[b] & MST_CONVERGED) return;
  const int n = sol.n_nodes[b]; const int N = n - 1;
  const double* gt = sol.t + (size_t)b * nmax; const int32_t* ge = sol.event + (size_t)b * nmax;
  double* gx = sol.x + (size_t)b * nmax * NX; double* gu = sol.u + (size_t)b * nmax * NU; const double* gdx = dxo + (size_t)b * nmax * NX; const double* gdu = duo + (size_t)b * nmax * NU;
  const int ne = clamp_events(p.n_events[b]); const double* ev = s_ev; const unsigned char* modes = s_modes;
  if (tid < 32) { const double* gev = p.event_times + (size_t)b * EMAX; const int32_t* gmodes = p.modes + (size_t)b * (EMAX + 1); s_ev[lane] = (lane < ne) ? gev[lane] : 0.0; s_modes[lane] = (unsigned char)((lane <= ne) ? gmodes[lane] : 15); if (lane == 0) s_modes[EMAX] = (unsigned char)((EMAX <= ne) ? gmodes[EMAX] : 15); }
  __syncthreads();
  const int nk = clamp_targets(p.n_target[b]); const double* tt = p.target_times + (size_t)b * KMAX; const double* ts = p.target_states + (size_t)b * KMAX * TARGET_DIM;
  const double* rb = robot + (size_t)b * ROBOT_DBL; const double armijo = rb[0], base_cost = rb[1], base_viol = sqrt(rb[2] + rb[3]), dxn = rb[4], dun = rb[5];
  const bool failed = (status[b] & MST_NOT_PD) != 0;
  double alpha = 1.0; bool accepted = false; double sc = base_cost, sd = rb[2], se = rb[3];
  const double w1 = mdl->rk_w1, w2 = mdl->rk_w2; const SrbdConst* srb = srbd_of(mdl, p.srbd, b);
  while (!failed) {
    double cost = 0.0, dyn = 0.0, eq = 0.0;
    for (int k = tid; k <= N; k += 32 * LS_WARPS) {
      double* xa = s_tp + tid * LS_ROW; double* ua = xa + NX; const bool terminal = (k == N);
#pragma unroll 6
      for (int i = 0; i < NX; ++i) { xa[i] = gx[(size_t)k * NX + i] + alpha * gdx[(size_t)k * NX + i]; ua[i] = terminal ? 0.0 : gu[(size_t)k * NU + i] + alpha * gdu[(size_t)k * NU + i]; }
      asm volatile("" ::: "memory");
      if (k == 0) { double s = 0.0; for (int i = 0; i < NX; ++i) { const double d = p.x0[(size_t)b * NX + i] - xa[i]; s = fma(d, d, s); } dyn += s; }
      if (!terminal && ge[k] == 1) { double s = 0.0; for (int i = 0; i < NX; ++i) { const double d = xa[i] - (gx[(size_t)(k + 1) * NX + i] + alpha * gdx[(size_t)(k + 1) * NX + i]); s = fma(d, d, s); } dyn += s; continue; }
      const double t = interval_start(gt[k], ge[k]);
      const double dt = terminal ? 1.0 : interval_end(gt[k + 1], ge[k + 1]) - t; const int mode = mode_at_time(ev, modes, ne, t); const int fm = terminal ? 0 : flag_mask(mode);
      ne::BaseKin bk; ne::FlowAcc acc; double* f1 = ua + NU;
      ne::base_eval<false>(mdl, xa, bk, srb); ne::flow_acc_init(acc);
      { double es = 0.0; bool ok = true;
#pragma unroll 1
        for (int i = 0; i < 4; ++i) { double d[3], Jl[9], pf[3]; ne::foot_eval<false>(mdl, xa, ua, bk, i, acc, d, pf, Jl, nullptr, nullptr, srb);
          if (!terminal) { double fe[3]; ne::foot_velocity_1<false>(mdl, xa, ua, bk, i, d, Jl, nullptr, fe, nullptr); ne::equality_add(mdl, ua, fe, pf, fm, ev, modes, ne, t, i, es, ok); } }
        if (!terminal) eq += dt * es; }
      ne::flow_finish<false>(mdl, xa, bk, acc, f1, nullptr, srb);
      asm volatile("" ::: "memory");
      { const ne::TargetSeg sg = ne::target_segment(tt, ts, nk, t); double pref[3], qref[4], ee[6]; ne::target_pose(sg, nk, pref, qref); ne::ee_eval<false>(mdl, xa, bk, pref, qref, ee, nullptr);
        cost += dt * ne::cost_value(mdl, xa, ua, sg, ee, fm, terminal, srb, tuning_of(mdl, p.tuning, b)); }
      if (terminal) continue;
      const double cdt = mdl->rk_c * dt;
#pragma unroll
      for (int i = 0; i < 12; ++i) xa[i] += cdt * f1[i];
#pragma unroll 6
      for (int i = 12; i < NX; ++i) xa[i] += cdt * ua[i];
      double f2[12]; ne::base_eval<false>(mdl, xa, bk, srb); ne::flow_acc_init(acc);
#pragma unroll 1
      for (int i = 0; i < 4; ++i) { double d[3]; ne::foot_eval<false>(mdl, xa, ua, bk, i, acc, d, nullptr, nullptr, nullptr, nullptr, srb); }
      ne::flow_finish<false>(mdl, xa, bk, acc, f2, nullptr, srb);
      double s = 0.0;
      auto defect = [&](int i, double fa, double fb) { const double x0i = gx[(size_t)k * NX + i] + alpha * gdx[(size_t)k * NX + i];
        const double d = x0i + dt * (w1 * fa + w2 * fb) - (gx[(size_t)(k + 1) * NX + i] + alpha * gdx[(size_t)(k + 1) * NX + i]); s = fma(d, d, s); };
#pragma unroll
      for (int i = 0; i < 12; ++i) defect(i, f1[i], f2[i]);
#pragma unroll 6
      for (int i = 12; i < NX; ++i) defect(i, ua[i], ua[i]);
      dyn += dt * s;
    }
    cost = warp_sum(cost); dyn = warp_sum(dyn); eq = warp_sum(eq);
    if (lane == 0) { red[warp][0] = cost; red[warp][1] = dyn; red[warp][2] = eq; }
    __syncthreads();
    if (threadIdx.x == 0) {
      double c = 0, dd = 0, e = 0; for (int w = 0; w < LS_WARPS; ++w) { c += red[w][0]; dd += red[w][1]; e += red[w][2]; }
      const double sv = sqrt(dd + e), am = alpha * armijo; bool acc;
      if (sv > mdl->g_max) acc = sv < (1.0 - mdl->gamma_c) * base_viol;
      else if (sv < mdl->g_min && base_viol < mdl->g_min && am < 0.0) acc = c < base_cost + mdl->armijo_factor * am;
      else acc = (c < base_cost - mdl->gamma_c * base_viol) || (sv < (1.0 - mdl->gamma_c) * base_viol);
      red[0][0] = c; red[0][1] = dd; red[0][2] = e;
      int dec = 0; if (acc) dec = 1; else { const double an = alpha * mdl->alpha_decay; if ((an * dxn < mdl->delta_tol && an * dun < mdl->delta_tol) || an < mdl->alpha_min) dec = 2; }
      decision = dec;
    }
    __syncthreads();
    const int dec = decision; sc = red[0][0]; sd = red[0][1]; se = red[0][2];
    __syncthreads();
    if (dec == 1) { accepted = true; break; }
    if (dec == 2) break;
    alpha *= mdl->alpha_decay;
  }
  if (accepted) {
    const int tot = n * NX, totu = N * NU, nt = blockDim.x;
    for (int e0 = threadIdx.x; e0 < tot; e0 += 4 * nt) {
      double vx[4], vu[4];
#pragma unroll
      for (int q = 0; q < 4; ++q) { const int e = e0 + q * nt; vx[q] = (e < tot) ? gx[e] + alpha * gdx[e] : 0.0; vu[q] = (e < totu) ? gu[e] + alpha * gdu[e] : 0.0; }
#pragma unroll
      for (int q = 0; q < 4; ++q) { const int e = e0 + q * nt; if (e < tot) gx[e] = vx[q]; if (e < totu) gu[e] = vu[q]; }
    }
  } else { alpha = 0.0; sc = base_cost; sd = rb[2]; se = rb[3]; }
  __syncthreads();
  fixup_inputs(sol, b, nmax, n, threadIdx.x, blockDim.x);
  if (threadIdx.x == 0) {
    int flags = accepted ? 0 : MST_NO_STEP;
    if (iteration + 1 < mdl->sqp_iterations) {
      const bool stepsize = alpha < mdl->alpha_min;
      const bool metrics = fabs(sc - base_cost) < mdl->cost_tol && sqrt(sd + se) < mdl->g_min;
      const bool primal = alpha * dxn < mdl->delta_tol && alpha * dun < mdl->delta_tol;
      if (stepsize || metrics || primal) flags |= MST_CONVERGED;
    }
    if (flags) atomicOr(&status[b], flags);
    double* si = step_info + (size_t)b * 4; si[0] = alpha; si[1] = sc; si[2] = sd; si[3] = se; }
}

constexpr int RO_THREADS = 128, RO_MAXTRIALS = 32;
template <bool PERF, class MT>
__device__ __forceinline__ void rollout_step(const DevModel* __restrict__ mdl, const SrbdConst* sc, const Tuning* tn, double* x, const double* u, double t, double dt, int fm, const double* ev, const MT* modes, int ne, const double* tt, const double* ts, int nk, double& cost, double& eq) {
  ne::BaseKin bk; ne::FlowAcc acc; double f1[12], x2[NX]; ne::base_eval<false>(mdl, x, bk, sc); ne::flow_acc_init(acc);
  if (PERF) { double es = 0.0; bool ok = true;
#pragma unroll 1
    for (int i = 0; i < 4; ++i) { double d[3], Jl[9], pf[3], fe[3]; ne::foot_eval<false>(mdl, x, u, bk, i, acc, d, pf, Jl, nullptr, nullptr, sc); ne::foot_velocity_1<false>(mdl, x, u, bk, i, d, Jl, nullptr, fe, nullptr);
      ne::equality_add(mdl, u, fe, pf, fm, ev, modes, ne, t, i, es, ok); }
    eq += dt * es;
    const ne::TargetSeg sg = ne::target_segment(tt, ts, nk, t); double pref[3], qref[4], ee[6]; ne::target_pose(sg, nk, pref, qref); ne::ee_eval<false>(mdl, x, bk, pref, qref, ee, nullptr);
    cost += dt * ne::cost_value(mdl, x, u, sg, ee, fm, false, sc, tn);
  } else {
#pragma unroll 1
    for (int i = 0; i < 4; ++i) { double d[3]; ne::foot_eval<false>(mdl, x, u, bk, i, acc, d, nullptr, nullptr, nullptr, nullptr, sc); } }
  ne::flow_finish<false>(mdl, x, bk, acc, f1, nullptr, sc);
  const double cdt = mdl->rk_c * dt, w1 = mdl->rk_w1, w2 = mdl->rk_w2;
#pragma unroll
  for (int i = 0; i < NX; ++i) x2[i] = x[i] + cdt * (i < 12 ? f1[i < 12 ? i : 0] : u[i]);
  double f2[12]; ne::base_eval<false>(mdl, x2, bk, sc); ne::flow_acc_init(acc);
#pragma unroll 1
  for (int i = 0; i < 4; ++i) { double d[3]; ne::foot_eval<false>(mdl, x2, u, bk, i, acc, d, nullptr, nullptr, nullptr, nullptr, sc); }
  ne::flow_finish<false>(mdl, x2, bk, acc, f2, nullptr, sc);
#pragma unroll
  for (int i = 0; i < NX; ++i) x[i] += dt * (w1 * (i < 12 ? f1[i < 12 ? i : 0] : u[i]) + w2 * (i < 12 ? f2[i < 12 ? i : 0] : u[i]));
}
__device__ __forceinline__ void rollout_input(const double* __restrict__ tl, const double* __restrict__ Kg, const double* __restrict__ unom, const double* dxv, double alpha, int lfp, double* un) {
  const int32_t* si = reinterpret_cast<const int32_t*>(tl + T_INT); const int ndep = si[SI_NDEP]; double dut[MU];
  for (int a = 0; a < MU; ++a) { const double* kr = Kg + a * LDG; double s0 = 0.0, s1 = 0.0;
#pragma unroll 5
    for (int j = 0; j < NX; j += 2) { s0 = fma(kr[j], dxv[j], s0); s1 = fma(kr[j + 1], dxv[j + 1], s1); }
    dut[a] = s0 + s1 + alpha * kr[NX]; }
  for (int c = 0; c < NU; ++c) un[c] = unom[c];
  for (int a = 0; a < MU; ++a) { const int fa = si[SI_FREE + a]; if (fa >= 0) un[fa] += dut[a]; }
  for (int d = 0; d < ndep; ++d) { const int di = si[SI_DEP + d]; double du = alpha * tl[T_PED + d];
    if (di >= 12) { const int j = di - 12, lg = j / 3, first = 3 * lg; const double* px = tl + T_PXJ + j * 12;
      for (int c = 0; c < 12; ++c) du = fma(px[c], dxv[sup_col(c, first)], du);
      const int foot = (lfp >> (2 * lg)) & 3; if (si[SI_PIV + foot] >= 0) for (int q2 = 0; q2 < 2; ++q2) { const int col = si[SI_PCOL + 2 * foot + q2]; if (col >= 0) du = fma(tl[T_PU2 + 2 * foot + q2], dut[col], du); } }
    un[di] += du; }
}
#ifndef QMB_RO_MINB
#define QMB_RO_MINB 2
#endif
__global__ void __launch_bounds__(RO_THREADS, QMB_RO_MINB) mpc_rollout_kernel(const DevModel* __restrict__ mdl, int b0, int B, int nmax, MpcProblemDev p, MpcSolutionDev sol, const double* __restrict__ stage, const double* __restrict__ gains,
                                                                   double* __restrict__ trial, const double* __restrict__ robot, int32_t* __restrict__ status, double* __restrict__ step_info, int mode_ls, int n_trials, int tr_pitch, int iteration) {
  const long long gid = (long long)blockIdx.x * RO_THREADS + threadIdx.x;
  const int b = b0 + (int)gid; if (b >= B) return;
  if (status[b] & MST_CONVERGED) return;
  const int n = sol.n_nodes[b]; const int N = n - 1;
  const double* gt = sol.t + (size_t)b * nmax; const int32_t* ge = sol.event + (size_t)b * nmax;
  double* gx = sol.x + (size_t)b * nmax * NX; double* gu = sol.u + (size_t)b * nmax * NU;
  const int ne = clamp_events(p.n_events[b]); const double* ev = p.event_times + (size_t)b * EMAX; const int32_t* modes = p.modes + (size_t)b * (EMAX + 1);
  const int lfp = pack_leg_foot(mdl);
  const int nk = clamp_targets(p.n_target[b]); const double* tt = p.target_times + (size_t)b * KMAX; const double* ts = p.target_states + (size_t)b * KMAX * TARGET_DIM;
  double xa[NX], cost = 0.0, eq = 0.0;
  if (mode_ls == 0) {
#pragma unroll
    for (int i = 0; i < NX; ++i) { xa[i] = p.x0[(size_t)b * NX + i]; gx[i] = xa[i]; }
    for (int k = 0; k < N; ++k) {
      if (ge[k] != 1) { const double t = interval_start(gt[k], ge[k]); const double dt = interval_end(gt[k + 1], ge[k + 1]) - t; double u[NU];
#pragma unroll
        for (int i = 0; i < NU; ++i) u[i] = gu[(size_t)k * NU + i];
        rollout_step<false>(mdl, srbd_of(mdl, p.srbd, b), tuning_of(mdl, p.tuning, b), xa, u, t, dt, 0, ev, modes, ne, tt, ts, nk, cost, eq); }
#pragma unroll
      for (int i = 0; i < NX; ++i) gx[(size_t)(k + 1) * NX + i] = xa[i];
    }
    return;
  }
  const double* rb = robot + (size_t)b * ROBOT_DBL; const double base_cost = rb[1], base_eq = rb[3]; const double pen = mdl->ddp_penalty;
  const double merit0 = base_cost + pen * sqrt(base_eq); const bool failed = (status[b] & MST_NOT_PD) != 0;
  double* tb = trial + (size_t)b * RO_MAXTRIALS * 2;
  double alpha = mdl->ddp_max_step; bool accepted = false; double sc = base_cost, se = base_eq;
  {
    if (!failed) for (int j = 0; j < n_trials; ++j) { const double c = tb[2 * j], e = tb[2 * j + 1], merit = c + pen * sqrt(e);
        if (merit < merit0 - mdl->ddp_armijo * alpha * fabs(merit0)) { accepted = true; sc = c; se = e; break; } alpha *= mdl->ddp_contraction; }
  }
  if (accepted) {
    const double* sgb = stage + (size_t)b * nmax * STAGE_DBL; const double* gb = gains + (size_t)b * nmax * GAIN_DBL;
    double xnom[NX];
#pragma unroll
    for (int i = 0; i < NX; ++i) { xa[i] = p.x0[(size_t)b * NX + i]; xnom[i] = gx[i]; }
#pragma unroll
    for (int i = 0; i < NX; ++i) gx[i] = xa[i];
    for (int k = 0; k < N; ++k) {
      if (ge[k] == 1) {
        for (int i = 0; i < NU; ++i) gu[(size_t)k * NU + i] = 0.0;
      } else {
        const double* tl = sgb + (size_t)k * STAGE_DBL + ST_TAIL; double dxv[NX], un[NU];
#pragma unroll
        for (int i = 0; i < NX; ++i) dxv[i] = xa[i] - xnom[i];
        rollout_input(tl, gb + (size_t)k * GAIN_DBL, gu + (size_t)k * NU, dxv, alpha, lfp, un);
        for (int i = 0; i < NU; ++i) gu[(size_t)k * NU + i] = un[i];
        const double t = interval_start(gt[k], ge[k]); const double dt = interval_end(gt[k + 1], ge[k + 1]) - t; const int fm = flag_mask(mode_at_time(ev, modes, ne, t));
        rollout_step<false>(mdl, srbd_of(mdl, p.srbd, b), tuning_of(mdl, p.tuning, b), xa, un, t, dt, fm, ev, modes, ne, tt, ts, nk, cost, eq);
      }
#pragma unroll
      for (int i = 0; i < NX; ++i) { xnom[i] = gx[(size_t)(k + 1) * NX + i]; gx[(size_t)(k + 1) * NX + i] = xa[i]; }
    }
  }
  if (!accepted) { alpha = 0.0; sc = base_cost; se = base_eq; }
  for (int k = 1; k < n; ++k) { if ((k == n - 1) || (ge[k] == 1)) for (int i = 0; i < NU; ++i) gu[(size_t)k * NU + i] = gu[(size_t)(k - 1) * NU + i]; }
  { int flags = accepted ? 0 : MST_NO_STEP; if (!accepted && iteration + 1 < mdl->sqp_iterations) flags |= MST_CONVERGED; if (flags) atomicOr(&status[b], flags);
    double* si = step_info + (size_t)b * 4; si[0] = alpha; si[1] = sc; si[2] = 0.0; si[3] = se; }
}

constexpr int RO_RPC_MAX = 16;
__global__ void __launch_bounds__(RO_THREADS, QMB_RO_MINB) mpc_rollout_trials_kernel(const DevModel* __restrict__ mdl, int b0, int B, int nmax, MpcProblemDev p, MpcSolutionDev sol, const double* __restrict__ stage, const double* __restrict__ gains,
                                                                          double* __restrict__ trial, const double* __restrict__ robot, const int32_t* __restrict__ status, int n_trials, int tr_pitch, int rpc) {
  extern __shared__ __align__(16) unsigned char smem_raw[]; double* sK = reinterpret_cast<double*>(smem_raw);
  __shared__ int s_kmax;
  const int tid = threadIdx.x, nthr = blockDim.x, r = tid / tr_pitch, tr = tid - r * tr_pitch; const int bfirst = b0 + blockIdx.x * rpc, b = bfirst + r;
  const bool active = b < B && tr < n_trials && !(status[b] & (MST_CONVERGED | MST_NOT_PD));
  const int N = active ? sol.n_nodes[b] - 1 : 0;
  if (tid == 0) s_kmax = 0;
  __syncthreads();
  if (active) atomicMax(&s_kmax, N);
  __syncthreads();
  const int kmax = s_kmax; if (kmax <= 0) return;
  const size_t bb = active ? (size_t)b : 0;
  const double* gt = sol.t + bb * nmax; const int32_t* ge = sol.event + bb * nmax; const double* gx = sol.x + bb * nmax * NX; const double* gu = sol.u + bb * nmax * NU;
  const int ne = clamp_events(p.n_events[bb]); const double* ev = p.event_times + bb * EMAX; const int32_t* modes = p.modes + bb * (EMAX + 1);
  const int lfp = pack_leg_foot(mdl);
  const int nk = clamp_targets(p.n_target[bb]); const double* tt = p.target_times + bb * KMAX; const double* ts = p.target_states + bb * KMAX * TARGET_DIM;
  const double* sgb = stage + bb * nmax * STAGE_DBL;
  double alpha = mdl->ddp_max_step; for (int j = 0; j < tr; ++j) alpha *= mdl->ddp_contraction;
  double xa[NX], xnom[NX], cost = 0.0, eq = 0.0;
#pragma unroll
  for (int i = 0; i < NX; ++i) { xa[i] = p.x0[bb * NX + i]; xnom[i] = gx[i]; }
  for (int k = 0; k < kmax; ++k) {
    __syncthreads();
    for (int e = tid; e < rpc * GAIN_DBL; e += nthr) { const int rr = e / GAIN_DBL; const int br = bfirst + rr; sK[e] = (br < B) ? gains[((size_t)br * nmax + k) * GAIN_DBL + (e - rr * GAIN_DBL)] : 0.0; }
    __syncthreads();
    if (active && k < N) {
      if (ge[k] != 1) {
        const double* tl = sgb + (size_t)k * STAGE_DBL + ST_TAIL; double dxv[NX], un[NU];
#pragma unroll
        for (int i = 0; i < NX; ++i) dxv[i] = xa[i] - xnom[i];
        rollout_input(tl, sK + r * GAIN_DBL, gu + (size_t)k * NU, dxv, alpha, lfp, un);
        const double t = interval_start(gt[k], ge[k]); const double dt = interval_end(gt[k + 1], ge[k + 1]) - t; const int fm = flag_mask(mode_at_time(ev, modes, ne, t));
        rollout_step<true>(mdl, srbd_of(mdl, p.srbd, (int)bb), tuning_of(mdl, p.tuning, (int)bb), xa, un, t, dt, fm, ev, modes, ne, tt, ts, nk, cost, eq);
      }
#pragma unroll
      for (int i = 0; i < NX; ++i) xnom[i] = gx[(size_t)(k + 1) * NX + i];
    }
  }
  if (active) {
    const double t = interval_start(gt[N], ge[N]); ne::BaseKin bk; ne::base_eval<false>(mdl, xa, bk, srbd_of(mdl, p.srbd, b)); double u0[NU]; for (int i = 0; i < NU; ++i) u0[i] = 0.0;
    const ne::TargetSeg sg = ne::target_segment(tt, ts, nk, t); double pref[3], qref[4], ee[6]; ne::target_pose(sg, nk, pref, qref); ne::ee_eval<false>(mdl, xa, bk, pref, qref, ee, nullptr);
    cost += ne::cost_value(mdl, xa, u0, sg, ee, 0, true, srbd_of(mdl, p.srbd, b), tuning_of(mdl, p.tuning, b));
    double* tb = trial + (size_t)b * RO_MAXTRIALS * 2; tb[2 * tr] = cost; tb[2 * tr + 1] = eq; }
}

__global__ void mpc_fixup_kernel(int B, int nmax, MpcSolutionDev sol) { const int b = blockIdx.x; if (b >= B) return; const int n = sol.n_nodes[b]; if (n >= 2) fixup_inputs(sol, b, nmax, n, threadIdx.x, blockDim.x); }

__global__ void mpc_policy_eval_kernel(int b0, int B, int nmax, MpcSolutionDev sol, const int32_t* __restrict__ n_events, const double* __restrict__ event_times, const int32_t* __restrict__ modes,
                                       const double* __restrict__ tq, double* __restrict__ x_des, double* __restrict__ u_des, int32_t* __restrict__ mode_out) {
  const int warp = threadIdx.x >> 5, lane = threadIdx.x & 31; const int b = b0 + blockIdx.x * (blockDim.x >> 5) + warp; if (b >= B) return;
  const int n = sol.n_nodes[b]; const double* gt = sol.t + (size_t)b * nmax; const double t = tq[b];
  int idx; double a; time_segment(gt, n, t, idx, a); const int i2 = (idx + 1 < n) ? idx + 1 : idx;
  const double* gx = sol.x + (size_t)b * nmax * NX; const double* gu = sol.u + (size_t)b * nmax * NU;
  if (lane < NX) { x_des[(size_t)b * NX + lane] = a * gx[(size_t)idx * NX + lane] + (1.0 - a) * gx[(size_t)i2 * NX + lane]; u_des[(size_t)b * NU + lane] = a * gu[(size_t)idx * NU + lane] + (1.0 - a) * gu[(size_t)i2 * NU + lane]; }
  if (lane == 0) mode_out[b] = mode_at_time(event_times + (size_t)b * EMAX, modes + (size_t)b * (EMAX + 1), clamp_events(n_events[b]), t);
}

bool mpc_alloc(MpcBuffers& m, int B, int nmax, std::string& err, std::vector<void*>& allocs, cudaStream_t stream) {
  m.B = B; m.nmax = nmax; m.cur = 0;
  if (SETUP_WARPS * ((setup_smem_per_warp(nmax) + 15) & ~(size_t)15) > 200 * 1024) { err = "max_nodes too large for the grid staging of the setup kernel (limit ~1000 nodes)"; return false; }
  auto A = [&](auto** p, size_t count) { void* q = nullptr; const size_t bytes = count * sizeof(**p); cudaError_t e = cudaMalloc(&q, bytes); if (e != cudaSuccess) { err = std::string("cudaMalloc (MPC buffers) failed: ") + cudaGetErrorString(e); return false; } cudaMemsetAsync(q, 0, bytes, stream); allocs.push_back(q); *p = static_cast<std::remove_reference_t<decltype(**p)>*>(q); return true; };
  const size_t Bn = (size_t)B * nmax;
  bool ok = A(&m.t0, B) && A(&m.x0, (size_t)B * NX) && A(&m.n_events, B) && A(&m.event_times, (size_t)B * EMAX) && A(&m.modes, (size_t)B * (EMAX + 1)) && A(&m.n_target, B) && A(&m.target_times, (size_t)B * KMAX) && A(&m.target_states, (size_t)B * KMAX * TARGET_DIM);
  for (int s = 0; s < 2 && ok; ++s) ok = A(&m.sol[s].n_nodes, B) && A(&m.sol[s].t, Bn) && A(&m.sol[s].event, Bn) && A(&m.sol[s].x, Bn * NX) && A(&m.sol[s].u, Bn * NU);
  ok = ok && A(&m.stage, Bn * STAGE_DBL) && A(&m.gains, Bn * GAIN_DBL) && A(&m.dx, Bn * NX) && A(&m.du, Bn * NU) && A(&m.node_rec, Bn * ne::NODE_REC_DBL) && A(&m.ddp_trial, (size_t)B * RO_MAXTRIALS * 2) && A(&m.robot, (size_t)B * ROBOT_DBL) && A(&m.status, B) && A(&m.step_info, (size_t)B * 4);
  return ok;
}

int mpc_configure_device() {
  cudaError_t e = cudaFuncSetAttribute(mpc_setup_kernel, cudaFuncAttributeMaxDynamicSharedMemorySize, 200 * 1024);
  if (e == cudaSuccess) e = cudaFuncSetAttribute(mpc_flow_kernel, cudaFuncAttributeMaxDynamicSharedMemorySize, FL_SMEM);
  if (e == cudaSuccess) e = cudaFuncSetAttribute(mpc_linesearch_kernel, cudaFuncAttributeMaxDynamicSharedMemorySize, LS_SMEM);
  if (e == cudaSuccess) e = cudaFuncSetAttribute(mpc_rollout_trials_kernel, cudaFuncAttributeMaxDynamicSharedMemorySize, RO_RPC_MAX * GAIN_DBL * 8);
  if (e == cudaSuccess) e = cudaFuncSetAttribute(mpc_lq_kernel<false>, cudaFuncAttributeMaxDynamicSharedMemorySize, (int)(sizeof(LqSmem) * LQ_WARPS));
  if (e == cudaSuccess) e = cudaFuncSetAttribute(mpc_lq_kernel<true>, cudaFuncAttributeMaxDynamicSharedMemorySize, (int)(sizeof(LqSmem) * LQ_WARPS));
  if (e == cudaSuccess) e = cudaFuncSetAttribute(mpc_riccati_kernel, cudaFuncAttributeMaxDynamicSharedMemorySize, (int)sizeof(RicSmem));
  return (int)e;
}

int mpc_solve_launch(const DevModel* mdl, const DevModel& hm, MpcBuffers& m, const MpcProblemDev& p, int b0, int b1, cudaStream_t stream, cudaEvent_t* ev) {
  const int nb = b1 - b0, nmax = m.nmax; if (nb <= 0) return 0;
  MpcSolutionDev prev = m.sol[m.cur], next = m.sol[1 - m.cur];
  if (ev) cudaEventRecord(ev[0], stream);
  mpc_setup_kernel<<<(nb + SETUP_WARPS - 1) / SETUP_WARPS, 32 * SETUP_WARPS, SETUP_WARPS * ((setup_smem_per_warp(nmax) + 15) & ~(size_t)15), stream>>>(mdl, b0, b1, nmax, p, prev, next, m.status);
  if (ev) cudaEventRecord(ev[1], stream);
  const long long nodes = (long long)nb * nmax; const int iters = hm.sqp_iterations < 1 ? 1 : hm.sqp_iterations; int launched = 1;
  const bool ddp = hm.solver == 2; int n_trials = 0, tr_pitch = 1;
  if (ddp) { for (double a = hm.ddp_max_step; a >= hm.ddp_min_step && n_trials < RO_MAXTRIALS; a *= hm.ddp_contraction) ++n_trials; while (tr_pitch < n_trials) tr_pitch *= 2; }
  const int ro_grid = (nb + RO_THREADS - 1) / RO_THREADS; const int ro_rpc = (RO_THREADS / tr_pitch < RO_RPC_MAX) ? RO_THREADS / tr_pitch : RO_RPC_MAX;
  if (ddp) { mpc_rollout_kernel<<<ro_grid, RO_THREADS, 0, stream>>>(mdl, b0, b1, nmax, p, next, m.stage, m.gains, m.ddp_trial, m.robot, m.status, m.step_info, 0, 1, 1, 0); ++launched; }
  for (int it = 0; it < iters; ++it) {
    mpc_flow_kernel<<<(unsigned)((nodes + 32 * FL_WARPS - 1) / (32 * FL_WARPS)), 32 * FL_WARPS, FL_SMEM, stream>>>(mdl, b0, b1, nmax, p, next, m.node_rec, m.status);
    if (ev && it == iters - 1) cudaEventRecord(ev[7], stream);
    (p.tuning ? mpc_lq_kernel<true> : mpc_lq_kernel<false>)<<<(unsigned)((nodes + LQ_WARPS - 1) / LQ_WARPS), 32 * LQ_WARPS, sizeof(LqSmem) * LQ_WARPS, stream>>>(mdl, b0, b1, nmax, p, next, m.node_rec, m.stage, m.status);
    if (ev && it == iters - 1) cudaEventRecord(ev[2], stream);
    mpc_riccati_kernel<<<nb, RIC_THREADS, sizeof(RicSmem), stream>>>(mdl, b0, b1, nmax, p, next, m.stage, m.gains, m.dx, m.du, m.robot, m.status);
    if (ev && it == iters - 1) cudaEventRecord(ev[3], stream);
    if (ddp) { mpc_rollout_trials_kernel<<<(nb + ro_rpc - 1) / ro_rpc, ro_rpc * tr_pitch, (size_t)ro_rpc * GAIN_DBL * 8, stream>>>(mdl, b0, b1, nmax, p, next, m.stage, m.gains, m.ddp_trial, m.robot, m.status, n_trials, tr_pitch, ro_rpc);
      mpc_rollout_kernel<<<ro_grid, RO_THREADS, 0, stream>>>(mdl, b0, b1, nmax, p, next, m.stage, m.gains, m.ddp_trial, m.robot, m.status, m.step_info, 2, n_trials, tr_pitch, it); ++launched; }
    else mpc_linesearch_kernel<<<nb, 32 * LS_WARPS, LS_SMEM, stream>>>(mdl, b0, b1, nmax, p, next, m.dx, m.du, m.robot, m.status, m.step_info, it);
    launched += 4;
  }
  if (ev) cudaEventRecord(ev[4], stream);
  return launched;
}

int mpc_policy_eval_launch(const MpcBuffers& m, const double* t, double* x_des, double* u_des, int32_t* mode, cudaStream_t stream, int b0, int b1) {
  if (b1 < 0) b1 = m.B; if (b1 <= b0) return 0;
  mpc_policy_eval_kernel<<<(b1 - b0 + 3) / 4, 128, 0, stream>>>(b0, b1, m.nmax, m.sol[m.cur], m.n_events, m.event_times, m.modes, t, x_des, u_des, mode);
  return 1;
}
int mpc_fixup_launch(const MpcBuffers& m, cudaStream_t stream) { mpc_fixup_kernel<<<m.B, 32, 0, stream>>>(m.B, m.nmax, m.sol[m.cur]); return 1; }

__global__ void __launch_bounds__(256) fp64_peak_kernel(double* out, int iters, double a, double b) {
  double x0 = threadIdx.x, x1 = x0 + 1, x2 = x0 + 2, x3 = x0 + 3, x4 = x0 + 4, x5 = x0 + 5, x6 = x0 + 6, x7 = x0 + 7;
  for (int i = 0; i < iters; ++i) { x0 = fma(x0, a, b); x1 = fma(x1, a, b); x2 = fma(x2, a, b); x3 = fma(x3, a, b); x4 = fma(x4, a, b); x5 = fma(x5, a, b); x6 = fma(x6, a, b); x7 = fma(x7, a, b); }
  if (x0 + x1 + x2 + x3 + x4 + x5 + x6 + x7 == 12345.678) out[0] = x0;
}
double measure_fp64_peak(cudaStream_t stream) {
  double* d = nullptr; cudaMalloc(&d, 8); cudaEvent_t e0, e1; cudaEventCreate(&e0); cudaEventCreate(&e1);
  int dev = 0, sms = 132; cudaGetDevice(&dev); cudaDeviceGetAttribute(&sms, cudaDevAttrMultiProcessorCount, dev);
  const int blocks = sms * 8, iters = 1 << 15; double best = 0.0;
  fp64_peak_kernel<<<blocks, 256, 0, stream>>>(d, 1024, 0.999999, 1e-9);
  for (int rep = 0; rep < 3; ++rep) {
    cudaEventRecord(e0, stream); fp64_peak_kernel<<<blocks, 256, 0, stream>>>(d, iters, 0.999999, 1e-9); cudaEventRecord(e1, stream); cudaEventSynchronize(e1);
    float ms = 0; cudaEventElapsedTime(&ms, e0, e1); const double tf = 2.0 * 8.0 * iters * 256.0 * blocks / (ms * 1e-3) / 1e12; if (tf > best) best = tf;
  }
  cudaEventDestroy(e0); cudaEventDestroy(e1); cudaFree(d); return best;
}

}
```

qm_control_b200/interface.py:

```python
import ctypes as C
import os

import numpy as np

from . import _lib
from ._lib import NX, NU, RBD, CMD, TARGET, EMAX, KMAX, Config, QmbError


class QMInterface:
    def __init__(self, taskFile=None, urdfFile=None, referenceFile=None, wbcGainsFile=None):
        self.taskFile = taskFile or _lib.asset("qm_task.info")
        self.urdfFile = urdfFile or _lib.asset("qm_robot.urdf")
        self.referenceFile = referenceFile or _lib.asset("qm_reference.info")
        self.gaitFile = _lib.asset("qm_gait.info")
        self.wbcGainsFile = wbcGainsFile
        for what, path in (("Task file", self.taskFile), ("URDF file", self.urdfFile), ("targetCommand file", self.referenceFile)):
            if not os.path.exists(path):
                raise ValueError("[QMInterface] %s not found: %s" % (what, path))


def _f64(a, shape=None):
    a = np.ascontiguousarray(a, dtype=np.float64)
    if shape is not None and tuple(a.shape) != tuple(shape):
        raise ValueError("expected shape %s, got %s" % (shape, a.shape))
    return a


def _i32(a, shape=None):
    a = np.ascontiguousarray(a, dtype=np.int32)
    if shape is not None and tuple(a.shape) != tuple(shape):
        raise ValueError("expected shape %s, got %s" % (shape, a.shape))
    return a


def _p(a):
    if a is None:
        return None
    if isinstance(a, np.ndarray):
        return C.c_void_p(a.ctypes.data)
    return C.c_void_p(a.data_ptr())


class Solver:

    def __init__(self, interface=None, batch=1, device=0, time_horizon=0.0, dt=0.0, max_nodes=0, wbc_variant=0):
        self.lib = _lib.load_library()
        self.interface = interface or QMInterface()
        cfg = Config(self.interface.taskFile.encode(), self.interface.urdfFile.encode(), self.interface.referenceFile.encode(),
                     self.interface.wbcGainsFile.encode() if self.interface.wbcGainsFile else None, batch, device, time_horizon, dt, max_nodes, wbc_variant)
        self._cfg = cfg
        h = C.c_void_p()
        rc = self.lib.qmb200_create(C.byref(cfg), C.byref(h))
        if rc != 0:
            raise QmbError("qmb200_create failed (%d): %s" % (rc, self.lib.qmb200_last_error(None).decode()))
        self.h = h
        b, n, e, k = C.c_int32(), C.c_int32(), C.c_int32(), C.c_int32()
        self.lib.qmb200_get_dims(self.h, C.byref(b), C.byref(n), C.byref(e), C.byref(k))
        self.batch, self.nmax, self.emax, self.kmax = b.value, n.value, e.value, k.value
        mass, hor, dtt = C.c_double(), C.c_double(), C.c_double()
        self.initial_state = np.zeros(NX); self.default_joint_state = np.zeros(18)
        self.lib.qmb200_get_model_info(self.h, C.byref(mass), _p(self.initial_state), _p(self.default_joint_state), C.byref(hor), C.byref(dtt))
        self.robot_mass, self.time_horizon, self.dt = mass.value, hor.value, dtt.value

    def close(self):
        if getattr(self, "h", None):
            self.lib.qmb200_destroy(self.h)
            self.h = None

    def __del__(self):
        try:
            self.close()
        except Exception:
            pass

    def _call(self, name, *args):
        rc = getattr(self.lib, "qmb200_" + name)(self.h, *args)
        if rc != 0:
            raise QmbError("qmb200_%s failed (%d): %s" % (name, rc, self.lib.qmb200_last_error(self.h).decode()))

    @property
    def launch_count(self):
        return int(self.lib.qmb200_launch_count(self.h))

    @property
    def stream(self):
        return self.lib.qmb200_stream(self.h)

    def joint_names(self):
        out = []
        for j in range(18):
            buf = C.create_string_buffer(64); self.lib.qmb200_get_joint_name(self.h, j, buf, 64); out.append(buf.value.decode())
        return out

    def wbc_update(self, x_des, u_des, rbd, mode, period, time):
        B = self.batch
        x_des = _f64(x_des, (B, NX)); u_des = _f64(u_des, (B, NU)); rbd = _f64(rbd, (B, RBD)); mode = _i32(mode, (B,)); period = _f64(period, (B,)); time = _f64(time, (B,))
        cmd = np.empty((B, CMD)); status = np.empty(B, dtype=np.int32)
        self._call("wbc_update", _p(x_des), _p(u_des), _p(rbd), _p(mode), _p(period), _p(time), _p(cmd), _p(status))
        return cmd, status

    def wbc_update_dev(self, x_des, u_des, rbd, mode, period, time, cmd, status, stream=None):
        self._call("wbc_update_dev", _p(x_des), _p(u_des), _p(rbd), _p(mode), _p(period), _p(time), _p(cmd), _p(status), stream)

    def wbc_get_gains(self):
        g = _lib.WbcGains(); self._call("wbc_get_gains", C.byref(g))
        return {n: (list(getattr(g, n)) if hasattr(getattr(g, n), "__len__") else getattr(g, n)) for n, _ in _lib.WbcGains._fields_}

    def wbc_set_gains(self, **gains):
        g = _lib.WbcGains(); self._call("wbc_get_gains", C.byref(g))
        for k, v in gains.items():
            cur = getattr(g, k)
            if hasattr(cur, "__len__"):
                for i, x in enumerate(v):
                    cur[i] = float(x)
            else:
                setattr(g, k, float(v))
        self._call("wbc_set_gains", C.byref(g))

    def wbc_set_input_last(self, input_last=None):
        self._call("wbc_set_input_last", _p(_f64(input_last, (self.batch, NU))) if input_last is not None else None)

    def wbc_get_diagnostics(self):
        d = np.zeros(self.batch, dtype=np.int32); self._call("wbc_get_diagnostics", _p(d))
        return dict(level0_passes=d & 0xFF, level1_iterations=(d >> 8) & 0xFF, level2_iterations=(d >> 16) & 0xFF, working_set=(d >> 24) & 0xFF)

    def wbc_set_iteration_caps(self, level0_passes=0, active_set_iterations=0):
        self._call("wbc_set_iteration_caps", int(level0_passes), int(active_set_iterations))

    def wbc_get_input_last(self):
        out = np.empty((self.batch, NU)); self._call("wbc_get_input_last", _p(out)); return out

    def _prob(self, prob):
        B = self.batch
        return [_f64(prob["t0"], (B,)), _f64(prob["x0"], (B, NX)), _i32(prob["n_events"], (B,)), _f64(prob["event_times"], (B, EMAX)), _i32(prob["modes"], (B, EMAX + 1)),
                _i32(prob["n_target"], (B,)), _f64(prob["target_times"], (B, KMAX)), _f64(prob["target_states"], (B, KMAX, TARGET))]

    def mpc_solve(self, prob):
        B, N = self.batch, self.nmax; a = self._prob(prob)
        out = dict(n_nodes=np.zeros(B, dtype=np.int32), t=np.zeros((B, N)), event=np.zeros((B, N), dtype=np.int32), x=np.zeros((B, N, NX)), u=np.zeros((B, N, NU)),
                   status=np.zeros(B, dtype=np.int32), step_info=np.zeros((B, 4)))
        self._call("mpc_solve", *[_p(v) for v in a], _p(out["n_nodes"]), _p(out["t"]), _p(out["event"]), _p(out["x"]), _p(out["u"]), _p(out["status"]), _p(out["step_info"]))
        return out

    def mpc_solve_dev(self, prob_dev, stream=None):
        keys = ("t0", "x0", "n_events", "event_times", "modes", "n_target", "target_times", "target_states")
        self._call("mpc_solve_dev", *[_p(prob_dev[k]) for k in keys], stream)

    SOLVERS = {"sqp": 0, "ipm": 1, "ddp": 2}

    def mpc_set_solver(self, solver):
        self._call("mpc_set_solver", self.SOLVERS[solver] if isinstance(solver, str) else int(solver))

    def mpc_get_solver(self):
        s, it = C.c_int32(), C.c_int32(); dt, gx, gn = C.c_double(), C.c_double(), C.c_double()
        self.lib.qmb200_mpc_get_solver(self.h, C.byref(s), C.byref(it), C.byref(dt), C.byref(gx), C.byref(gn))
        return dict(solver=s.value, iterations=it.value, delta_tol=dt.value, g_max=gx.value, g_min=gn.value)

    def mpc_set_iterations(self, sqp_iterations=0, cost_tol=0.0):
        self._call("mpc_set_iterations", int(sqp_iterations), float(cost_tol))

    def mpc_reset(self):
        self._call("mpc_reset")

    def mpc_set_solution(self, sol):
        B, N = self.batch, self.nmax
        self._call("mpc_set_solution", _p(_i32(sol["n_nodes"], (B,))), _p(_f64(sol["t"], (B, N))), _p(_i32(sol["event"], (B, N))), _p(_f64(sol["x"], (B, N, NX))), _p(_f64(sol["u"], (B, N, NU))))

    def mpc_get_solution(self):
        B, N = self.batch, self.nmax
        out = dict(n_nodes=np.zeros(B, dtype=np.int32), t=np.zeros((B, N)), event=np.zeros((B, N), dtype=np.int32), x=np.zeros((B, N, NX)), u=np.zeros((B, N, NU)),
                   status=np.zeros(B, dtype=np.int32), step_info=np.zeros((B, 4)))
        self._call("mpc_get_solution", _p(out["n_nodes"]), _p(out["t"]), _p(out["event"]), _p(out["x"]), _p(out["u"]), _p(out["status"]), _p(out["step_info"]))
        return out

    def policy_eval(self, t):
        B = self.batch; t = _f64(t, (B,)); xd = np.empty((B, NX)); ud = np.empty((B, NU)); mode = np.empty(B, dtype=np.int32)
        self._call("policy_eval", _p(t), _p(xd), _p(ud), _p(mode))
        return xd, ud, mode

    def tick(self, prob, t_eval, rbd, period):
        B = self.batch; a = self._prob(prob); t_eval = _f64(t_eval, (B,)); rbd = _f64(rbd, (B, RBD)); period = _f64(period, (B,))
        cmd = np.empty((B, CMD)); status = np.empty(B, dtype=np.int32)
        self._call("tick", *[_p(v) for v in a], _p(t_eval), _p(rbd), _p(period), _p(cmd), _p(status))
        return cmd, status

    def tick_dev(self, prob_dev, t_eval, rbd, period, cmd, status, stream=None):
        keys = ("t0", "x0", "n_events", "event_times", "modes", "n_target", "target_times", "target_states")
        self._call("tick_dev", *[_p(prob_dev[k]) for k in keys], _p(t_eval), _p(rbd), _p(period), _p(cmd), _p(status), stream)

    def comm_unique_id(self):
        buf = C.create_string_buffer(128)
        if self.lib.qmb200_comm_get_unique_id(buf) != 0:
            raise QmbError("qmb200_comm_get_unique_id: %s" % self.lib.qmb200_last_error(None).decode())
        return buf.raw

    def comm_init(self, nranks, rank, unique_id):
        self._call("comm_init", int(nranks), int(rank), C.c_char_p(bytes(unique_id)))

    def comm_info(self):
        n, r, v = C.c_int32(), C.c_int32(), C.c_int32(); self.lib.qmb200_comm_info(self.h, C.byref(n), C.byref(r), C.byref(v)); return n.value, r.value, v.value

    def allgather_torque(self, cmd_dev, torque_all_dev, perm_dev=None, stream=None):
        self._call("allgather_torque", None, _p(cmd_dev), _p(perm_dev), _p(torque_all_dev), stream)

    def gait_bin_permutation(self, prob):
        n = len(prob["t0"]); perm = np.zeros(n, dtype=np.int32)
        rc = self.lib.qmb200_gait_bin_permutation(n, _p(_f64(prob["t0"])), _p(_i32(prob["n_events"])), _p(_f64(prob["event_times"])), _p(_i32(prob["modes"])), _p(perm))
        if rc != 0:
            raise QmbError("qmb200_gait_bin_permutation failed")
        return perm

    def set_pipeline(self, chunks):
        self._call("set_pipeline", int(chunks))

    def set_profiling(self, on=True):
        self._call("set_profiling", 1 if on else 0)

    def collect_kernel_times(self):
        self.lib.qmb200_collect_kernel_times(self.h)

    def kernel_times(self):
        ms = np.zeros(6); self._call("get_kernel_times", _p(ms))
        d = dict(zip(("setup", "lq", "riccati", "linesearch", "policy_eval", "wbc"), ms.tolist()))
        v = C.c_double(); self._call("get_flow_kernel_time", C.byref(v)); d["lq_flow"] = v.value
        return d

    def measure_fp64_peak(self):
        v = C.c_double(); self._call("measure_fp64_peak", C.byref(v)); return v.value

    def debug_get_step(self):
        B, N = self.batch, self.nmax; dx = np.zeros((B, N, NX)); du = np.zeros((B, N, NU)); robot = np.zeros((B, 8))
        self._call("debug_get_step", _p(dx), _p(du), _p(robot)); return dx, du, robot

    def observation_update(self, rbd, period, t_obs, x_obs):
        B = self.batch; rbd = _f64(rbd, (B, RBD)); period = _f64(period, (B,)); t = _f64(t_obs, (B,)).copy(); x = _f64(x_obs, (B, NX)).copy()
        self._call("observation_update", _p(rbd), _p(period), _p(t), _p(x)); return t, x

    def target_trajectories(self, kind, cmd, t_obs, x_obs, ee_state, last_ee_target, target=None):
        B = self.batch; c = np.zeros((B, 7)); cmd = np.asarray(cmd, dtype=np.float64).reshape(B, -1); c[:, :cmd.shape[1]] = cmd
        t = _f64(t_obs, (B,)); x = _f64(x_obs, (B, NX)); ee = _f64(ee_state, (B, 7)); le = _f64(last_ee_target, (B, 7)).copy()
        nt = np.zeros(B, dtype=np.int32); tt = np.zeros((B, KMAX)); ts = np.zeros((B, KMAX, TARGET))
        if np.ndim(kind) == 0:
            self._call("target_trajectories", int(kind), _p(c), _p(t), _p(x), _p(ee), _p(le), _p(nt), _p(tt), _p(ts)); return nt, tt, ts, le
        if target is not None:
            nt, tt, ts = _i32(target[0], (B,)).copy(), _f64(target[1], (B, KMAX)).copy(), _f64(target[2], (B, KMAX, TARGET)).copy()
        self._call("target_trajectories_per_robot", _p(_i32(kind, (B,))), _p(c), _p(t), _p(x), _p(ee), _p(le), _p(nt), _p(tt), _p(ts)); return nt, tt, ts, le

    def initial_ee_target(self):
        v = np.zeros(7); self.lib.qmb200_initial_ee_target(_p(v)); return np.tile(v, (self.batch, 1))

    def set_arm_gains(self, kp, kd):
        self._call("set_arm_gains", float(kp), float(kd))

    def control_law(self, x_des, u_des, wbc_cmd, t_obs, x_obs, joint_cmd, arm_pos_cmd, last_time):
        B = self.batch; jc = _f64(joint_cmd, (B, 18, 5)).copy(); ap = _f64(arm_pos_cmd, (B, 6)).copy(); lt = _f64(last_time, (B,)).copy(); st = np.zeros(B, dtype=np.int32)
        self._call("control_law", _p(_f64(x_des, (B, NX))), _p(_f64(u_des, (B, NU))), _p(_f64(wbc_cmd, (B, CMD))), _p(_f64(t_obs, (B,))), _p(_f64(x_obs, (B, NX))),
                   _p(jc), _p(ap), _p(lt), _p(st)); return jc, ap, lt, st

    def hw_set_delay(self, delay):
        self._call("hw_set_delay", float(delay))

    def hw_write(self, time, period, joint_cmd, joint_pos, joint_vel):
        B = self.batch; eff = np.zeros((B, 18)); st = np.zeros(B, dtype=np.int32)
        self._call("hw_write", _p(_f64(time, (B,))), _p(_f64(period, (B,))), _p(_f64(joint_cmd, (B, 18, 5))), _p(_f64(joint_pos, (B, 18))), _p(_f64(joint_vel, (B, 18))), _p(eff), _p(st))
        return eff, st

    def update(self, rbd, period, t_obs, x_obs, joint_cmd, arm_pos_cmd, last_time):
        B = self.batch; t = _f64(t_obs, (B,)).copy(); x = _f64(x_obs, (B, NX)).copy(); jc = _f64(joint_cmd, (B, 18, 5)).copy(); ap = _f64(arm_pos_cmd, (B, 6)).copy(); lt = _f64(last_time, (B,)).copy()
        cmd = np.zeros((B, CMD)); st = np.zeros(B, dtype=np.int32)
        self._call("update", _p(_f64(rbd, (B, RBD))), _p(_f64(period, (B,))), _p(t), _p(x), _p(jc), _p(ap), _p(lt), _p(cmd), _p(st))
        return t, x, jc, ap, lt, cmd, st

    def target_trajectories_dev(self, kind, cmd, t_obs, x_obs, ee_state, last_ee_target, n_target, target_times, target_states, stream=None):
        if not hasattr(kind, "data_ptr"):
            self._call("target_trajectories_dev", int(kind), _p(cmd), _p(t_obs), _p(x_obs), _p(ee_state), _p(last_ee_target), _p(n_target), _p(target_times), _p(target_states), stream)
        else:
            self._call("target_trajectories_per_robot_dev", _p(kind), _p(cmd), _p(t_obs), _p(x_obs), _p(ee_state), _p(last_ee_target), _p(n_target), _p(target_times),
                       _p(target_states), stream)

    def update_dev(self, rbd, period, t_obs, x_obs, joint_cmd, arm_pos_cmd, last_time, cmd, status, stream=None):
        self._call("update_dev", _p(rbd), _p(period), _p(t_obs), _p(x_obs), _p(joint_cmd), _p(arm_pos_cmd), _p(last_time), _p(cmd), _p(status), stream)

    def hw_write_dev(self, time, period, joint_cmd, joint_pos, joint_vel, effort, status, stream=None):
        self._call("hw_write_dev", _p(time), _p(period), _p(joint_cmd), _p(joint_pos), _p(joint_vel), _p(effort), _p(status), stream)

    def sim_get_params(self):
        p = _lib.SimParams(); self._call("sim_get_params", C.byref(p))
        return {n: (list(getattr(p, n)) if n == "joint_damping" else getattr(p, n)) for n, _ in _lib.SimParams._fields_}

    def sim_set_params(self, **params):
        p = _lib.SimParams(); self._call("sim_get_params", C.byref(p))
        for k, v in params.items():
            if k == "joint_damping":
                for i, x in enumerate(v):
                    p.joint_damping[i] = float(x)
            elif k == "substeps_per_ms":
                p.substeps_per_ms = int(v)
            else:
                setattr(p, k, float(v))
        self._call("sim_set_params", C.byref(p))

    def sim_step(self, duration, effort, q, v, wrench=None):
        B = self.batch; q = _f64(q, (B, 24)).copy(); v = _f64(v, (B, 24)).copy(); rbd = np.zeros((B, RBD)); contact = np.zeros(B, dtype=np.int32); st = np.zeros(B, dtype=np.int32)
        if wrench is None:
            self._call("sim_step", float(duration), _p(_f64(effort, (B, 18))), _p(q), _p(v), _p(rbd), _p(contact), _p(st))
        else:
            self._call("sim_step_ext", float(duration), _p(_f64(effort, (B, 18))), _p(_f64(wrench, (B, 12))), _p(q), _p(v), _p(rbd), _p(contact), _p(st))
        return q, v, rbd, contact, st

    def sim_step_dev(self, duration, effort, q, v, rbd, contact, status, stream=None, wrench=None):
        if wrench is None:
            self._call("sim_step_dev", float(duration), _p(effort), _p(q), _p(v), _p(rbd), _p(contact), _p(status), stream)
        else:
            self._call("sim_step_ext_dev", float(duration), _p(effort), _p(wrench), _p(q), _p(v), _p(rbd), _p(contact), _p(status), stream)

    def sim_set_robot_params(self, friction_mu=None, payload=None):
        B = self.batch
        mu = None if friction_mu is None else _f64(np.broadcast_to(np.asarray(friction_mu, dtype=np.float64), (B,)), (B,))
        pl = None if payload is None else _f64(payload, (B, 8))
        self._call("sim_set_robot_params", _p(mu), _p(pl))

    def sim_get_robot_params(self):
        B = self.batch; mu = np.zeros(B); pl = np.zeros((B, 8)); mask = C.c_int32()
        self._call("sim_get_robot_params", _p(mu), _p(pl), C.byref(mask))
        return dict(friction_mu=mu if mask.value & 1 else None, payload=pl if mask.value & 2 else None)

    def set_model_payload(self, payload=None):
        pl = None if payload is None else _f64(payload, (self.batch, 8))
        self._call("set_model_payload", _p(pl))

    def get_model_payload(self):
        pl = np.zeros((self.batch, 8)); is_set = C.c_int32()
        self._call("get_model_payload", _p(pl), C.byref(is_set))
        return pl if is_set.value else None

    def set_robot_tuning(self, tuning=None):
        rows = None if tuning is None else self.robot_tuning_rows(tuning)
        self._call("set_robot_tuning", _p(rows))

    def robot_tuning_rows(self, tuning):
        B = self.batch; rows = np.repeat(self.get_handle_tuning()[None, :], B, axis=0)
        for k, v in tuning.items():
            if k not in _lib.TUNING_LAYOUT:
                raise ValueError("robot tuning: unknown field %r (one of %s)" % (k, ", ".join(_lib.TUNING_LAYOUT)))
            off, w = _lib.TUNING_LAYOUT[k]; a = np.asarray(v, dtype=np.float64)
            ok = a.shape in ((), (B, w)) or a.shape == ((B,) if w == 1 else (w,))
            if not ok:
                raise ValueError("robot tuning: %s must be a scalar, %s, got shape %s" % (k, "[%d]" % B if w == 1 else "[%d] or [%d, %d]" % (w, B, w), a.shape))
            rows[:, off:off + w] = a.reshape(B, 1) if w == 1 and a.shape == (B,) else a
        return rows

    def get_handle_tuning(self):
        row = np.zeros(_lib.TUNING); self._call("get_handle_tuning", _p(row)); return row

    def get_robot_tuning(self):
        rows = np.zeros((self.batch, _lib.TUNING)); is_set = C.c_int32()
        self._call("get_robot_tuning", _p(rows), C.byref(is_set))
        if not is_set.value:
            return None
        return {k: rows[:, off] if w == 1 else rows[:, off:off + w] for k, (off, w) in _lib.TUNING_LAYOUT.items()}

    def payload_est_get_params(self):
        p = _lib.PayloadEstParams(); self._call("payload_est_get_params", C.byref(p))
        return {n: getattr(p, n) for n, _ in _lib.PayloadEstParams._fields_}

    def payload_est_set_params(self, **params):
        p = _lib.PayloadEstParams(); self._call("payload_est_get_params", C.byref(p))
        names = [n for n, _ in _lib.PayloadEstParams._fields_]
        for k, v in params.items():
            if k not in names:
                raise ValueError("payload_est_set_params: unknown parameter %r (one of %s)" % (k, ", ".join(names)))
            setattr(p, k, float(v))
        self._call("payload_est_set_params", C.byref(p))

    def payload_est_reset(self, prior=None):
        pl = None if prior is None else _f64(prior, (self.batch, 8))
        self._call("payload_est_reset", _p(pl))

    def payload_est_step(self, dt, effort, rbd):
        B = self.batch; st = np.zeros(B, dtype=np.int32)
        self._call("payload_est_step", float(dt), _p(_f64(effort, (B, 18))), _p(_f64(rbd, (B, RBD))), _p(st))
        return st

    def payload_est_step_dev(self, dt, effort, rbd, status, stream=None):
        self._call("payload_est_step_dev", float(dt), _p(effort), _p(rbd), _p(status), stream)

    def payload_est_commit_dev(self, stream=None):
        self._call("payload_est_commit_dev", stream)

    def payload_est_get(self):
        B = self.batch; th = np.zeros((B, 10)); pd = np.zeros((B, 10)); n = np.zeros(B, dtype=np.int32)
        self._call("payload_est_get", _p(th), _p(pd), _p(n))
        return dict(theta=th, p_diag=pd, samples=n)

    def payload_est_stop(self):
        self._call("payload_est_stop")

    def get_model_payload_dev(self, out, stream=None):
        self._call("get_model_payload_dev", _p(out), stream)

    def sim_set_terrain(self, tiles=None, cell=None):
        if tiles is None:
            self._call("sim_set_terrain", 0, 0, 0, 0.0, None); return
        t = _f64(tiles)
        if t.ndim != 3:
            raise ValueError("expected tiles of shape [T, ny, nx], got %s" % (t.shape,))
        self._call("sim_set_terrain", t.shape[0], t.shape[2], t.shape[1], float(cell), _p(t))

    def sim_get_terrain(self):
        n, nx, ny, cell = C.c_int32(), C.c_int32(), C.c_int32(), C.c_double()
        self._call("sim_get_terrain", C.byref(n), C.byref(nx), C.byref(ny), C.byref(cell), None)
        if n.value == 0:
            return None
        t = np.zeros((n.value, ny.value, nx.value))
        self._call("sim_get_terrain", None, None, None, None, _p(t))
        return dict(tiles=t, cell=cell.value)

    def sim_set_robot_terrain(self, tile=None, origin=None):
        B = self.batch
        if tile is None:
            self._call("sim_set_robot_terrain", None, None); return
        t = _i32(np.broadcast_to(np.asarray(tile), (B,)), (B,))
        o = _f64(np.zeros((B, 2)) if origin is None else np.broadcast_to(np.asarray(origin, dtype=np.float64), (B, 2)), (B, 2))
        self._call("sim_set_robot_terrain", _p(t), _p(o))

    def sim_get_robot_terrain(self):
        t = np.zeros(self.batch, dtype=np.int32); o = np.zeros((self.batch, 2)); is_set = C.c_int32()
        self._call("sim_get_robot_terrain", _p(t), _p(o), C.byref(is_set))
        return dict(tile=t, origin=o) if is_set.value else None

    def sim_standing_state(self, xy_yaw):
        xy = _f64(xy_yaw).reshape(-1, 3); n = xy.shape[0]; q = np.zeros((n, 24)); v = np.zeros((n, 24))
        self._call("sim_standing_state", n, _p(xy), _p(q), _p(v))
        return q, v

    def sim_get_sensor_params(self):
        p = _lib.SensorParams(); self._call("sim_get_sensor_params", C.byref(p))
        return {n: getattr(p, n) for n, _ in _lib.SensorParams._fields_}

    def sim_set_sensor_params(self, **params):
        p = _lib.SensorParams(); self._call("sim_get_sensor_params", C.byref(p))
        names = [n for n, _ in _lib.SensorParams._fields_]
        for k, v in params.items():
            if k not in names:
                raise ValueError("sim_set_sensor_params: unknown parameter %r (one of %s)" % (k, ", ".join(names)))
            setattr(p, k, int(v) if k == "seed" else float(v))
        self._call("sim_set_sensor_params", C.byref(p))

    def sim_read_sensors(self, dt, sample, q, v, v_prev):
        B = self.batch; out = np.zeros((B, _lib.SENSORS)); q, v, v_prev = _f64(q, (B, 24)), _f64(v, (B, 24)), _f64(v_prev, (B, 24))
        self._call("sim_read_sensors", float(dt), int(sample), _p(q), _p(v), _p(v_prev), _p(out))
        return out

    def sim_read_sensors_dev(self, dt, sample, q, v, v_prev, sensors, stream=None):
        self._call("sim_read_sensors_dev", float(dt), int(sample), _p(q), _p(v), _p(v_prev), _p(sensors), stream)

    def state_est_get_params(self):
        p = _lib.StateEstParams(); self._call("state_est_get_params", C.byref(p))
        return {n: getattr(p, n) for n, _ in _lib.StateEstParams._fields_}

# ... 402 lines not shown
```

Measured before the change: 24.37.

## Pick Riccati serial warp by per-SM slot so it lands on distinct schedulers

The Riccati kernel now claims a per-SM slot (0-3) through atomics on a new device array. It reads each warp's hardware %warpid and picks as the serial Cholesky warp the one whose scheduler matches its slot. The aim is to spread the four co-resident CTAs' serial phases across different warp schedulers, so they stop contending on one scheduler as the old (k+b)&3 rotation could. This adds atomics at kernel start and end, a new persistent buffer that must be cleared correctly, and compile-time-disabled probe instrumentation.

```diff
diff --git a/include/qmb200.h b/include/qmb200.h
--- a/include/qmb200.h
+++ b/include/qmb200.h
@@ -341,6 +341,8 @@
 int qmb200_measure_fp64_peak(qmb200_handle* h, double* tflops);
 
 int qmb200_debug_get_step(qmb200_handle* h, double* dx , double* du , double* robot );
+#define QMB200_SM_SLOT_WORDS 256
+int qmb200_mpc_sm_slots(qmb200_handle* h, uint32_t* masks );
 #define QMB200_SOLVER_SQP 0
 #define QMB200_SOLVER_IPM 1
 #define QMB200_SOLVER_DDP 2
diff --git a/qm_control_b200/_lib.py b/qm_control_b200/_lib.py
--- a/qm_control_b200/_lib.py
+++ b/qm_control_b200/_lib.py
@@ -8,6 +8,7 @@
 
 NX, NU, RBD, CMD, TARGET, EMAX, KMAX = 30, 30, 55, 54, 37, 32, 4
 GAIT_CAP, GAIT_MAXM = 64, 16
+SM_SLOT_WORDS = 256
 TARGET_CMD_VEL, TARGET_EE_CMD_VEL, TARGET_EE_GOAL = 0, 1, 2
 
 dp = C.POINTER(C.c_double)
@@ -253,6 +254,7 @@
     "qmb200_get_flow_kernel_time": (I32, [P] * 2),
     "qmb200_measure_fp64_peak": (I32, [P] * 2),
     "qmb200_debug_get_step": (I32, [P] * 4),
+    "qmb200_mpc_sm_slots": (I32, [P] * 2),
     "qmb200_mpc_set_solver": (I32, [P, I32]),
     "qmb200_mpc_get_solver": (I32, [P] * 6),
     "qmb200_comm_get_unique_id": (I32, [P]),
diff --git a/qm_control_b200/csrc/capi_mpc.inc b/qm_control_b200/csrc/capi_mpc.inc
--- a/qm_control_b200/csrc/capi_mpc.inc
+++ b/qm_control_b200/csrc/capi_mpc.inc
@@ -245,5 +245,10 @@
   if (dx) QMB_CUDA(h, cudaMemcpy(dx, h->mpc.dx, Bn * NX * 8, cudaMemcpyDeviceToHost)); if (du) QMB_CUDA(h, cudaMemcpy(du, h->mpc.du, Bn * NU * 8, cudaMemcpyDeviceToHost));
   if (robot) QMB_CUDA(h, cudaMemcpy(robot, h->mpc.robot, (size_t)h->B * ROBOT_DBL * 8, cudaMemcpyDeviceToHost)); return 0;
 }
-
-}
+static_assert(QMB200_SM_SLOT_WORDS == RIC_SLOT_WORDS, "the header states the slot array's size");
+int qmb200_mpc_sm_slots(qmb200_handle* h, uint32_t* masks) {
+  if (!h || !masks) return -1; QMB_CUDA(h, cudaSetDevice(h->device)); QMB_CUDA(h, cudaDeviceSynchronize());
+  QMB_CUDA(h, cudaMemcpy(masks, h->mpc.sm_slots, RIC_SLOT_WORDS * sizeof(uint32_t), cudaMemcpyDeviceToHost)); return 0;
+}
+
+}
diff --git a/qm_control_b200/csrc/kernels/mpc_api.cuh b/qm_control_b200/csrc/kernels/mpc_api.cuh
--- a/qm_control_b200/csrc/kernels/mpc_api.cuh
+++ b/qm_control_b200/csrc/kernels/mpc_api.cuh
@@ -30,6 +30,7 @@
 static_assert(STAGE_DBL == 1484 && (ST_BR % 2 == 0) && (ST_Q % 2 == 0) && (ST_TAIL % 2 == 0) && (TAIL_DBL % 2 == 0), "16-byte aligned pieces");
 constexpr int GAIN_DBL = 18 * LDG;
 constexpr int ROBOT_DBL = 8;
+constexpr int RIC_SLOT_WORDS = 256;
 
 struct MpcSolutionDev { int32_t* n_nodes = nullptr; double* t = nullptr; int32_t* event = nullptr; double* x = nullptr; double* u = nullptr; };
 
@@ -42,6 +43,7 @@
   double *node_rec = nullptr;
   double *stage = nullptr, *gains = nullptr, *dx = nullptr, *du = nullptr, *robot = nullptr, *step_info = nullptr;
   int32_t *stage_i = nullptr, *status = nullptr;
+  uint32_t *sm_slots = nullptr;
 };
 bool mpc_alloc(MpcBuffers& m, int B, int nmax, std::string& err, std::vector<void*>& allocs, cudaStream_t stream);
 int mpc_configure_device();
diff --git a/qm_control_b200/csrc/kernels/mpc_kernels.cu b/qm_control_b200/csrc/kernels/mpc_kernels.cu
--- a/qm_control_b200/csrc/kernels/mpc_kernels.cu
+++ b/qm_control_b200/csrc/kernels/mpc_kernels.cu
@@ -440,7 +440,16 @@
 #ifndef QMB_TMA
 #define QMB_TMA 1
 #endif
+#ifndef QMB_RIC_PROBE
+#define QMB_RIC_PROBE 0
+#endif
 constexpr int RIC_THREADS = 128, RIC_NTYPE = 512;
+#if QMB_RIC_PROBE
+constexpr int RP_HDR = 12, RP_NODE = 5;
+__device__ unsigned* g_ric_probe = nullptr;
+__device__ unsigned g_ric_probe_launch = 0;
+__device__ __forceinline__ unsigned probe_clock(unsigned t0) { return (unsigned)clock64() - t0; }
+#endif
 struct RicSmem {
   double P[NX * LDX];
   double A[NX * LDX];
@@ -453,9 +462,14 @@
   double dx[32], dut[32], tmp[32];
   double red[RIC_THREADS / 32][4];
   alignas(8) unsigned long long bar[4];
-  int flag; int pad_;
+  int flag;
+  int sw, slot, slot_sm;
+  unsigned char wsp[4];
   signed char srow[MU + 2], sfirst[MU + 2];
   unsigned char ntype[RIC_NTYPE];
+#if QMB_RIC_PROBE
+  unsigned pr_t0, pr_j, pr_top, pr_p3s, pr_p3e, pr_help[4];
+#endif
 };
 static_assert(sizeof(RicSmem) <= 57344 - 64, "Riccati kernel must keep four CTAs per SM");
 
@@ -469,6 +483,8 @@
   asm volatile("cp.async.bulk.shared::cluster.global.mbarrier::complete_tx::bytes [%0], [%1], %2, [%3];\n" ::"r"(smem_u32(dst)), "l"(src), "r"(bytes), "r"(smem_u32(bar)) : "memory");
 }
 __device__ __forceinline__ int fresh_tid() { int t; asm volatile("mov.u32 %0, %%tid.x;" : "=r"(t)); return t; }
+__device__ __forceinline__ unsigned sm_id() { unsigned r; asm volatile("mov.u32 %0, %%smid;" : "=r"(r)); return r; }
+__device__ __forceinline__ unsigned warp_id() { unsigned r; asm volatile("mov.u32 %0, %%warpid;" : "=r"(r)); return r; }
 __device__ __forceinline__ void cp_async16(void* smem_dst, const void* gmem_src) { asm volatile("cp.async.cg.shared.global [%0], [%1], 16;\n" ::"r"(smem_u32(smem_dst)), "l"(gmem_src) : "memory"); }
 __device__ __forceinline__ void cp_async_wait_all() { asm volatile("cp.async.wait_all;\n" ::: "memory"); }
 struct CopyGroup {
@@ -519,16 +535,30 @@
 __device__ __forceinline__ int sup_pos(int j, int first) { return j < 6 ? j : ((j >= 9 && j < 12) ? j - 3 : (((unsigned)(j - 12 - first) < 3u) ? 9 + j - 12 - first : -1)); }
 
 __global__ void __launch_bounds__(RIC_THREADS, 4) mpc_riccati_kernel(const DevModel* __restrict__ mdl, int b0, int B, int nmax, MpcProblemDev p, MpcSolutionDev sol, const double* __restrict__ stage,
-                                                                  double* __restrict__ gains, double* __restrict__ dxo, double* __restrict__ duo, double* __restrict__ robot, int32_t* __restrict__ status) {
+                                                                  double* __restrict__ gains, double* __restrict__ dxo, double* __restrict__ duo, double* __restrict__ robot, int32_t* __restrict__ status,
+                                                                  unsigned* __restrict__ sm_slots) {
   extern __shared__ __align__(16) unsigned char smem_raw[];
   RicSmem& sm = *reinterpret_cast<RicSmem*>(smem_raw);
   const int tid = threadIdx.x, warp = tid >> 5, lane = tid & 31, ti = tid >> 2, jb = tid & 3; const int b = b0 + blockIdx.x;
   if (status[b] & MST_CONVERGED) return;
+#if QMB_RIC_PROBE
+  const unsigned long long pr_start = clock64();
+#endif
   const int n = sol.n_nodes[b]; const int N = n - 1;
   const double* sgb = stage + (size_t)b * nmax * STAGE_DBL; double* gb = gains + (size_t)b * nmax * GAIN_DBL;
   const int lfp = pack_leg_foot(mdl); const double imass = 1.0 / srbd_of(mdl, p.srbd, b)->m;
   for (int e = tid; e < (int)(sizeof(RicSmem) / 8); e += RIC_THREADS) reinterpret_cast<double*>(&sm)[e] = 0.0;
   __syncthreads();
+  if (tid == 0) { const unsigned smid = sm_id(); int slot = b & 3, word = -1;
+    if (smid < (unsigned)RIC_SLOT_WORDS) { unsigned taken = 0u;
+      for (int attempt = 0; attempt < 4; ++attempt) {
+        const unsigned free = ~taken & 0xFu; if (!free) break; const unsigned bit = free & (0u - free);
+        taken = atomicOr(sm_slots + smid, bit); if (!(taken & bit)) { slot = __ffs(bit) - 1; word = (int)smid; break; } } }
+    sm.slot = slot; sm.slot_sm = word; }
+  if (lane == 0) sm.wsp[warp] = (unsigned char)(warp_id() & 3u);
+#if QMB_RIC_PROBE
+  if (tid == 0) { sm.pr_t0 = (unsigned)pr_start; unsigned* pr = g_ric_probe + (size_t)b * (RP_HDR + RP_NODE * nmax); pr[0] = g_ric_probe_launch; pr[1] = sm_id(); pr[6] = (unsigned)pr_start; pr[7] = (unsigned)(pr_start >> 32); sm.pr_j = 0; }
+#endif
   if (tid < NX && (tid < 3 || tid >= 24)) sm.A[tid * LDX + tid] = 1.0;
   if (tid == 0) { for (int i = 0; i < 4; ++i) mbar_init(&sm.bar[i], 1); asm volatile("fence.mbarrier_init.release.cluster;\n" ::: "memory"); }
   asm volatile("fence.proxy.async.shared::cta;\n" ::: "memory");
@@ -568,6 +598,13 @@
   perf0 = warp_sum(perf0); perf1 = warp_sum(perf1); perf2 = warp_sum(perf2);
   if (lane == 0) { sm.red[warp][0] = perf0; sm.red[warp][1] = perf1; sm.red[warp][2] = perf2; }
   __syncthreads();
+  if (tid == 0) { const int slot = sm.slot; int sw = -1, hits = 0;
+    for (int w = 0; w < 4; ++w) if (sm.wsp[w] == slot) { sw = w; ++hits; }
+    sm.sw = hits == 1 ? sw : slot;
+#if QMB_RIC_PROBE
+    unsigned* pr = g_ric_probe + (size_t)b * (RP_HDR + RP_NODE * nmax); for (int w = 0; w < 4; ++w) pr[2 + w] = sm.wsp[w]; pr[10] = slot; pr[11] = sm.sw;
+#endif
+  }
   double perf[3]; for (int i = 0; i < 3; ++i) perf[i] = sm.red[0][i] + sm.red[1][i] + sm.red[2][i] + sm.red[3][i];
   if (N >= 1) { issue_tail(N - 1); if (node_type(N - 1) != 1) issue_ab(N - 1); gT.wait(); if (node_type(N - 1) != 1) expand(); }
   int st = 0;
@@ -583,6 +620,9 @@
       continue;
     }
     gAB.wait(); if (QMB_TMA) __syncthreads();
+#if QMB_RIC_PROBE
+    if (tid == 0) sm.pr_top = probe_clock(sm.pr_t0);
+#endif
     const double dtw_k = sm.tail[T_MISC]; const int acol0 = reinterpret_cast<const int32_t*>(sm.tail + T_INT)[SI_M] - 6;
     { const int i0 = 16 * (warp >> 1), j0 = 16 * (warp & 1);
       double c[2][2][2] = {};
@@ -629,10 +669,13 @@
     __syncthreads();
     issue_q(k);
     if (k > 0) issue_tail(k - 1);
-    const int sw = (k + b) & 3;
+    const int sw = sm.sw;
     if (!QMB_TMA) gQ.wait();
     if (warp == sw) {
       if (QMB_TMA) gQ.skip();
+#if QMB_RIC_PROBE
+      if (lane == 0) sm.pr_p3s = probe_clock(sm.pr_t0);
+#endif
       double hr[MU], y[MU]; double dinv = 0.0; bool ok = true; double* Yb = sm.PB;
 #pragma unroll
       for (int c = 0; c < MU; ++c) { hr[c] = (lane < MU) ? sm.H[c * LDH + lane] : 0.0; y[c] = sm.G[c * LDG + lane]; }
@@ -658,6 +701,9 @@
 #pragma unroll
         for (int c = 0; c < a; ++c) y[c] = fma(-sm.Lt[c * MU + a], y[a], y[c]);
       }
+#if QMB_RIC_PROBE
+      if (lane == 0) sm.pr_p3e = probe_clock(sm.pr_t0);
+#endif
     } else {
       if (QMB_TMA) gQ.wait();
       const int hi = (warp - sw - 1) & 3;
@@ -668,8 +714,16 @@
           if (ri >= 24 && ri < NX && cj <= NX) v += sm.W[ri * LDX + cj];
           c[0][0][e] = v; }
         warp_mma<24, 1, 1, false>(sm.A, LDX, i0, sm.W, LDX, j0, c, g, t); cfrag_store<1, 1>(sm.P, LDX, i0, j0, NX, c, g, t); }
+#if QMB_RIC_PROBE
+      if (lane == 0) sm.pr_help[warp] = probe_clock(sm.pr_t0);
+#endif
     }
     __syncthreads();
+#if QMB_RIC_PROBE
+    if (tid == 0) { unsigned hl = 0; for (int w = 0; w < 4; ++w) if (w != sw && sm.pr_help[w] > hl) hl = sm.pr_help[w];
+      unsigned* pr = g_ric_probe + (size_t)b * (RP_HDR + RP_NODE * nmax) + RP_HDR + RP_NODE * sm.pr_j;
+      pr[0] = sm.pr_top; pr[1] = sm.pr_p3s; pr[2] = sm.pr_p3e; pr[3] = hl; pr[4] = sm.wsp[sw]; ++sm.pr_j; }
+#endif
     if (sm.flag) { st |= MST_NOT_PD; if (k > 0) gT.wait(); break; }
     if (k > 0) { if (tnext != 1) issue_ab(k - 1); gT.wait(); if (tnext != 1) expand(); }
     { const double* Yb = sm.PB; const int i0 = 16 * (warp >> 1), j0 = 16 * (warp & 1);
@@ -732,7 +786,12 @@
   if (lane == 0) { sm.red[warp][0] = armijo; sm.red[warp][1] = dxn2; sm.red[warp][2] = dun2; }
   __syncthreads();
   if (tid == 0) { double a = 0, x2 = 0, u2 = 0; for (int w = 0; w < RIC_THREADS / 32; ++w) { a += sm.red[w][0]; x2 += sm.red[w][1]; u2 += sm.red[w][2]; }
-    double* rb = robot + (size_t)b * ROBOT_DBL; rb[0] = a; rb[1] = perf[0]; rb[2] = perf[1]; rb[3] = perf[2]; rb[4] = sqrt(x2); rb[5] = sqrt(u2); if (st) atomicOr(&status[b], st); }
+    double* rb = robot + (size_t)b * ROBOT_DBL; rb[0] = a; rb[1] = perf[0]; rb[2] = perf[1]; rb[3] = perf[2]; rb[4] = sqrt(x2); rb[5] = sqrt(u2); if (st) atomicOr(&status[b], st);
+    if (sm.slot_sm >= 0) atomicAnd(sm_slots + sm.slot_sm, ~(1u << sm.slot));
+#if QMB_RIC_PROBE
+    unsigned* pr = g_ric_probe + (size_t)b * (RP_HDR + RP_NODE * nmax); pr[8] = probe_clock(sm.pr_t0); pr[9] = sm.pr_j;
+#endif
+  }
 }
 
 __device__ __forceinline__ void fixup_inputs(MpcSolutionDev sol, int b, int nmax, int n, int tid, int nthreads) {
@@ -1017,6 +1076,7 @@
   bool ok = A(&m.t0, B) && A(&m.x0, (size_t)B * NX) && A(&m.n_events, B) && A(&m.event_times, (size_t)B * EMAX) && A(&m.modes, (size_t)B * (EMAX + 1)) && A(&m.n_target, B) && A(&m.target_times, (size_t)B * KMAX) && A(&m.target_states, (size_t)B * KMAX * TARGET_DIM);
   for (int s = 0; s < 2 && ok; ++s) ok = A(&m.sol[s].n_nodes, B) && A(&m.sol[s].t, Bn) && A(&m.sol[s].event, Bn) && A(&m.sol[s].x, Bn * NX) && A(&m.sol[s].u, Bn * NU);
   ok = ok && A(&m.stage, Bn * STAGE_DBL) && A(&m.gains, Bn * GAIN_DBL) && A(&m.dx, Bn * NX) && A(&m.du, Bn * NU) && A(&m.node_rec, Bn * ne::NODE_REC_DBL) && A(&m.ddp_trial, (size_t)B * RO_MAXTRIALS * 2) && A(&m.robot, (size_t)B * ROBOT_DBL) && A(&m.status, B) && A(&m.step_info, (size_t)B * 4);
+  ok = ok && A(&m.sm_slots, RIC_SLOT_WORDS);
   return ok;
 }
 
@@ -1031,6 +1091,15 @@
   return (int)e;
 }
 
+#if QMB_RIC_PROBE
+static unsigned* g_probe_buf = nullptr; static size_t g_probe_words = 0; static unsigned g_probe_launch = 0;
+static void ric_probe_arm(const MpcBuffers& m, cudaStream_t stream) {
+  const size_t words = (size_t)m.B * (RP_HDR + RP_NODE * m.nmax);
+  if (words > g_probe_words) { cudaStreamSynchronize(stream); cudaFree(g_probe_buf); cudaMalloc(&g_probe_buf, words * 4); cudaMemset(g_probe_buf, 0, words * 4); g_probe_words = words;
+    cudaMemcpyToSymbol(g_ric_probe, &g_probe_buf, sizeof(g_probe_buf)); }
+  static unsigned id; id = ++g_probe_launch; cudaMemcpyToSymbolAsync(g_ric_probe_launch, &id, sizeof(id), 0, cudaMemcpyHostToDevice, stream); cudaStreamSynchronize(stream);
+}
+#endif
 int mpc_solve_launch(const DevModel* mdl, const DevModel& hm, MpcBuffers& m, const MpcProblemDev& p, int b0, int b1, cudaStream_t stream, cudaEvent_t* ev) {
   const int nb = b1 - b0, nmax = m.nmax; if (nb <= 0) return 0;
   MpcSolutionDev prev = m.sol[m.cur], next = m.sol[1 - m.cur];
@@ -1047,7 +1116,10 @@
     if (ev && it == iters - 1) cudaEventRecord(ev[7], stream);
     (p.tuning ? mpc_lq_kernel<true> : mpc_lq_kernel<false>)<<<(unsigned)((nodes + LQ_WARPS - 1) / LQ_WARPS), 32 * LQ_WARPS, sizeof(LqSmem) * LQ_WARPS, stream>>>(mdl, b0, b1, nmax, p, next, m.node_rec, m.stage, m.status);
     if (ev && it == iters - 1) cudaEventRecord(ev[2], stream);
-    mpc_riccati_kernel<<<nb, RIC_THREADS, sizeof(RicSmem), stream>>>(mdl, b0, b1, nmax, p, next, m.stage, m.gains, m.dx, m.du, m.robot, m.status);
+#if QMB_RIC_PROBE
+    ric_probe_arm(m, stream);
+#endif
+    mpc_riccati_kernel<<<nb, RIC_THREADS, sizeof(RicSmem), stream>>>(mdl, b0, b1, nmax, p, next, m.stage, m.gains, m.dx, m.du, m.robot, m.status, m.sm_slots);
     if (ev && it == iters - 1) cudaEventRecord(ev[3], stream);
     if (ddp) { mpc_rollout_trials_kernel<<<(nb + ro_rpc - 1) / ro_rpc, ro_rpc * tr_pitch, (size_t)ro_rpc * GAIN_DBL * 8, stream>>>(mdl, b0, b1, nmax, p, next, m.stage, m.gains, m.ddp_trial, m.robot, m.status, n_trials, tr_pitch, ro_rpc);
       mpc_rollout_kernel<<<ro_grid, RO_THREADS, 0, stream>>>(mdl, b0, b1, nmax, p, next, m.stage, m.gains, m.ddp_trial, m.robot, m.status, m.step_info, 2, n_trials, tr_pitch, it); ++launched; }
@@ -1083,3 +1155,12 @@
 }
 
 }
+
+#if QMB_RIC_PROBE
+extern "C" long long qmb_ric_probe_copy(unsigned* out, long long words) {
+  if (cudaDeviceSynchronize() != cudaSuccess) return -1;
+  const size_t n = words < (long long)qmb::g_probe_words ? (size_t)words : qmb::g_probe_words;
+  if (out && n && cudaMemcpy(out, qmb::g_probe_buf, n * 4, cudaMemcpyDeviceToHost) != cudaSuccess) return -1;
+  return (long long)qmb::g_probe_words;
+}
+#endif
diff --git a/qm_control_b200/interface.py b/qm_control_b200/interface.py
--- a/qm_control_b200/interface.py
+++ b/qm_control_b200/interface.py
@@ -156,6 +156,11 @@
         self.lib.qmb200_mpc_get_solver(self.h, C.byref(s), C.byref(it), C.byref(dt), C.byref(gx), C.byref(gn))
         return dict(solver=s.value, iterations=it.value, delta_tol=dt.value, g_max=gx.value, g_min=gn.value)
 
+    def mpc_sm_slots(self):
+        out = np.zeros(_lib.SM_SLOT_WORDS, dtype=np.uint32)
+        self._call("mpc_sm_slots", _p(out))
+        return out
+
     def mpc_set_iterations(self, sqp_iterations=0, cost_tol=0.0):
         self._call("mpc_set_iterations", int(sqp_iterations), float(cost_tol))
 
```

After: 24.81, median of 6. 1.02x the previous value.
